# curtischong/arreau

Measured on AMD Instinct MI355X. Metric: denoising steps/sec (crystal-steps, whole node), higher is better.
Workload: dtype f32

## Files before the change

arreau_amd/_hip.py:

```python
import ctypes
import os
from ctypes import c_char_p, c_double, c_float, c_int32, c_int64, c_size_t, c_void_p, POINTER, Structure

import torch

_HERE = os.path.dirname(os.path.abspath(__file__))
LIB_PATH = os.environ.get("ARREAU_HIP_LIB") or os.path.join(_HERE, "csrc", "libarreau_hip.so")

EXPORTS = [
    "arreau_last_error", "arreau_version", "arreau_model_create", "arreau_model_destroy",
    "arreau_model_config", "arreau_workspace_bytes", "arreau_lattice_from_params", "arreau_frac_to_cart",
    "arreau_radius_graph_pbc", "arreau_compact_edges", "arreau_edges_to_slots", "arreau_predict_scores",
    "arreau_reverse_step", "arreau_profile_edge_kernel", "arreau_edge_kernel_time_ms", "arreau_conv_kernel_time_ms",
    "arreau_model_status", "arreau_model_set_variant", "arreau_ponita_forward",
    "arreau_diffusion_noise", "arreau_diffusion_losses", "arreau_sample_loop", "arreau_philox_fill",
    "arreau_train_forward", "arreau_train_backward", "arreau_train_conv_stats", "arreau_model_update_train_weights",
    "arreau_debug_sgemm", "arreau_optimizer_create", "arreau_optimizer_step", "arreau_optimizer_destroy",
    "arreau_model_train_weight_pointers", "arreau_model_refresh_derived_train_weights",
    "arreau_model_set_formats", "arreau_debug_set_pollution", "arreau_debug_leftover_fraction",
    "arreau_sample_loop_conditioned", "arreau_condition_initial_state",
    "arreau_sample_loop_scheduled", "arreau_reverse_step_to",
    "arreau_sample_loop_corrected", "arreau_corrector_step", "arreau_philox_fill_word",
    "arreau_sample_loop_resampled", "arreau_resample_jump", "arreau_optimizer_step_ema",
    "arreau_sample_loop_tied", "arreau_reverse_step_tied", "arreau_resample_jump_tied",
    "arreau_sample_loop_sym", "arreau_reverse_step_sym", "arreau_crystal_screen",
    "arreau_crystal_fingerprint", "arreau_fingerprint_match",
]

STATUS_NONFINITE, STATUS_BAD_TIMESTEP, STATUS_BAD_TYPE, STATUS_BAD_TIE, STATUS_BAD_SYMMETRY = 1, 2, 4, 8, 16
EDGE_KERNELS = {0: "fp32-mfma", 1: "fp32-mfma", 2: "fp32-mfma", 3: "bf16x6", 4: "fp16x3", 5: "general-fp32-gemm"}
MLP_KERNELS = {0: "fp32-mfma", 1: "bf16x6", 2: "fp16x3-32x32x16", 3: "fp16x3-16x16x32",
               5: "general-fp32-gemm"}
VARIANT_GENERAL = 5


class ArreauHipError(RuntimeError):
    pass


OPT_MAX_GROUPS = 4


class AdamArgs(Structure):
    _fields_ = [("step", c_int64), ("lr", c_double * OPT_MAX_GROUPS), ("weight_decay", c_double * OPT_MAX_GROUPS),
                ("beta1", c_double), ("beta2", c_double), ("eps", c_double), ("max_norm", c_double)]


class SampleConditionC(Structure):
    _fields_ = [("x0", c_void_p), ("pos_mask", c_void_p), ("a0", c_void_p), ("type_mask", c_void_p), ("l0", c_void_p),
                ("len_mask", c_void_p)]


class SampleScheduleC(Structure):
    _fields_ = [("d_next", c_void_p), ("lattice_clipmax", ctypes.c_float)]


class CorrectorC(Structure):
    _fields_ = [("steps", c_int32), ("snr", ctypes.c_float)]


class ResamplingC(Structure):
    _fields_ = [("passes", c_int32), ("jump_length", c_int32), ("timesteps", POINTER(c_int32)), ("n_timesteps", c_int32)]


class SymmetryC(Structure):
    _fields_ = [(name, c_void_p) for name in ("leader", "op", "orbit", "orbit_ptr", "orbit_atoms", "stab_ptr", "stab_ops", "rot",
                                                "rot_inv", "trans")] + [(name, c_int32) for name in ("n_orbits", "n_orbit_atoms",
                                                                                                     "n_stab_ops", "n_ops")]


class ScreenCriteriaC(Structure):
    _fields_ = [("min_distance", c_float), ("min_volume", c_float), ("search_radius", c_float), ("mask_type", c_int32),
                ("max_shells", c_int32)]


class ScreenResultC(Structure):
    _fields_ = [(name, c_void_p) for name in ("min_distance", "pair", "n_close", "volume", "number_density", "flags")]


class FingerprintParamsC(Structure):
    _fields_ = [("r_max", c_float), ("sigma", c_float), ("n_bins", c_int32), ("max_shells", c_int32)]


class FingerprintResultC(Structure):
    _fields_ = [(name, c_void_p) for name in ("fingerprint", "species", "counts", "flags")]


class MatchResultC(Structure):
    _fields_ = [(name, c_void_p) for name in ("duplicate_of", "distance", "nearest", "nearest_distance")]


class Config(Structure):
    _fields_ = [
        ("num_atomic_states", c_int32), ("hidden_dim", c_int32), ("basis_dim", c_int32),
        ("num_layers", c_int32), ("num_ori", c_int32), ("widening_factor", c_int32), ("degree", c_int32),
        ("max_neighbors", c_int32), ("num_timesteps", c_int32), ("radius", c_float),
        ("has_layer_scale", c_int32),
    ]


class Status(Structure):
    _fields_ = [("flags", c_int32), ("edge_kernel", c_int32), ("mlp_kernel", c_int32), ("conv_kernel", c_int32),
                ("basis_row_bytes", c_int32), ("conv_cross_fp8", c_int32), ("edge_activation_bound", c_float), ("node_activation_bound", c_float),
                ("basis_fp8_share", c_float), ("cross_fp8_share", c_float), ("readout_kernel", c_int32)]


_SD_FIELDS = [
    "basis_w1", "basis_b1", "basis_w2", "basis_b2", "fiber_w1", "fiber_b1", "fiber_w2", "fiber_b2",
    "x_embedder_w", "conv_kernel_w", "conv_fiber_w", "conv_bias", "norm_w", "norm_b", "linear1_w",
    "linear1_b", "linear2_w", "linear2_b", "layer_scale", "readout_w", "readout_b", "ori_grid", "t_emb_w",
    "ve_sigmas", "vp_alpha_bars", "vp_betas", "q_one_step_transposed", "q_mats",
]


class StateDict(Structure):
    _fields_ = [(name, c_void_p) for name in _SD_FIELDS]


def _prototypes():
    vp, i32, i64, u32, u64, f32, f64 = c_void_p, c_int32, c_int64, ctypes.c_uint32, ctypes.c_uint64, c_float, c_double
    cond, sched, corr, res, sym = (POINTER(t) for t in (SampleConditionC, SampleScheduleC, CorrectorC, ResamplingC, SymmetryC))
    loop = [vp] * 6 + [i32] * 4 + [u64] + [vp] * 4 + [c_size_t, i32]
    step_to = [vp] * 8 + [i32, i32] + [vp] * 7 + [f32]
    jump = [vp] * 8 + [i32, i32] + [vp] * 5 + [cond, vp]
    adam = [vp] * 4 + [POINTER(AdamArgs), vp]
    return {
        "arreau_last_error": [], "arreau_version": [],
        "arreau_model_create": [POINTER(Config), POINTER(StateDict), vp, POINTER(vp)],
        "arreau_model_destroy": [vp],
        "arreau_model_config": [vp, POINTER(Config)],
        "arreau_workspace_bytes": [POINTER(Config), i64, i64],
        "arreau_lattice_from_params": [vp, vp, i32, vp, vp],
        "arreau_frac_to_cart": [vp, vp, vp, i32, i32, vp, vp],
        "arreau_radius_graph_pbc": [vp, vp, vp, i32, i32, f32, i32] + [vp] * 6,
        "arreau_compact_edges": [vp] * 5 + [i32, i32] + [vp] * 6,
        "arreau_edges_to_slots": [vp, vp, vp, i64, i32, i32] + [vp] * 6,
        "arreau_predict_scores": [vp] * 7 + [i32, i32, i32] + [vp] * 7 + [vp, c_size_t, vp],
        "arreau_reverse_step": [vp] * 7 + [i32, i32] + [vp] * 8,
        "arreau_model_status": [vp, POINTER(Status), i32, vp],
        "arreau_model_set_variant": [vp, i32, i32],
        "arreau_model_set_formats": [vp, i32, i32],
        "arreau_ponita_forward": [vp] * 5 + [i32, i32] + [vp] * 7 + [vp, c_size_t, vp],
        "arreau_diffusion_noise": [vp] * 6 + [i32, i32] + [vp] * 11,
        "arreau_diffusion_losses": [vp] * 10 + [i32, i32] + [vp] * 6,
        "arreau_sample_loop": loop + [vp],
        "arreau_sample_loop_conditioned": loop + [cond, vp],
        "arreau_sample_loop_scheduled": loop + [cond, sched, vp],
        "arreau_sample_loop_corrected": loop + [cond, sched, corr, vp],
        "arreau_sample_loop_resampled": loop + [cond, sched, corr, res, vp],
        "arreau_sample_loop_tied": loop + [cond, sched, corr, res, vp, vp],
        "arreau_sample_loop_sym": loop + [cond, sched, corr, res, vp, sym, vp],
        "arreau_condition_initial_state": [vp] * 4 + [i32, i32, i32, u64, cond, vp],
        "arreau_reverse_step_to": step_to + [vp],
        "arreau_reverse_step_tied": step_to + [vp, vp],
        "arreau_reverse_step_sym": step_to + [vp, sym, vp],
        "arreau_corrector_step": [vp] * 4 + [i32, i32, vp, vp, f32, cond, vp],
        "arreau_resample_jump": jump + [vp],
        "arreau_resample_jump_tied": jump + [vp, vp],
        "arreau_philox_fill": [u64, i32, i32, i64, vp, vp, vp],
        "arreau_philox_fill_word": [u64, i32, i32, u32, i64, vp, vp, vp],
        "arreau_crystal_screen": [vp] * 4 + [i32, i32, POINTER(ScreenCriteriaC), POINTER(ScreenResultC), vp],
        "arreau_crystal_fingerprint": [vp] * 4 + [i32, i32, POINTER(FingerprintParamsC), POINTER(FingerprintResultC), vp],
        "arreau_fingerprint_match": [POINTER(FingerprintResultC), i32, POINTER(FingerprintResultC), i32, f32, POINTER(MatchResultC), vp],
        "arreau_train_forward": [vp] * 7 + [i32, i32] + [vp] * 4,
        "arreau_train_backward": [vp] * 4 + [POINTER(StateDict), vp],
        "arreau_train_conv_stats": [vp, vp, vp],
        "arreau_debug_sgemm": [i32, i32, i32, i32, vp, i64, i64, vp, i64, i64, vp, i32, f32, f32, vp],
        "arreau_model_update_train_weights": [vp, POINTER(StateDict), vp],
        "arreau_model_train_weight_pointers": [vp, POINTER(StateDict)],
        "arreau_model_refresh_derived_train_weights": [vp, vp, vp, vp],
        "arreau_optimizer_create": [i32, POINTER(vp), POINTER(vp), POINTER(i64), POINTER(i64), POINTER(i32), i32, i64, POINTER(vp)],
        "arreau_optimizer_step": adam + [vp],
        "arreau_optimizer_step_ema": adam + [f64, vp, vp],
        "arreau_optimizer_destroy": [vp],
        "arreau_debug_set_pollution": [u32],
        "arreau_debug_leftover_fraction": [u32, POINTER(f64), POINTER(f64), vp],
        "arreau_profile_edge_kernel": [i32],
        "arreau_edge_kernel_time_ms": [POINTER(f64), POINTER(i64)],
        "arreau_conv_kernel_time_ms": [POINTER(f64), POINTER(i64)],
    }


_RESTYPES = {"arreau_last_error": c_char_p, "arreau_version": c_char_p, "arreau_model_destroy": None,
             "arreau_workspace_bytes": c_size_t, "arreau_optimizer_destroy": None}

_lib = None


def lib():
    global _lib
    if _lib is not None:
        return _lib
    if not os.path.exists(LIB_PATH):
        raise ArreauHipError(
            f"{LIB_PATH} not found: build it with `python -m arreau_amd.build` (hipcc, gfx950). "
            "arreau_amd has no CPU fallback.")
    L = ctypes.CDLL(LIB_PATH)
    prototypes = _prototypes()
    for name in EXPORTS:
        if os.environ.get("ARREAU_HIP_LIB") and not hasattr(L, name):
            continue
        fn = getattr(L, name)
        fn.argtypes = prototypes[name]
        fn.restype = _RESTYPES.get(name, c_int32)
    _lib = L
    return L


def check(rc, what):
    if rc != 0:
        msg = lib().arreau_last_error().decode(errors="replace")
        raise ArreauHipError(f"{what} failed (code {rc}): {msg}")


def ptr(t):
    if t is None:
        return None
    assert t.is_contiguous(), "arreau_amd passes contiguous tensors only"
    return c_void_p(t.data_ptr())


def stream_ptr(device=None):
    return c_void_p(torch.cuda.current_stream(device).cuda_stream)


def require_gpu():
    if not torch.cuda.is_available():
        raise ArreauHipError("arreau_amd needs an AMD GPU (gfx950); there is no CPU fallback.")
```

arreau_amd/csrc/f16x3.h:

```cpp
#pragma once
#include <hip/hip_fp16.h>

#include "internal.h"

typedef _Float16 f16x8 __attribute__((ext_vector_type(8)));
typedef _Float16 f16x2 __attribute__((ext_vector_type(2)));
typedef unsigned int u32x4 __attribute__((ext_vector_type(4)));

#define F16X3_SCALE 2048.0f
#define F16X3_INV_SCALE (1.0f / 2048.0f)

#ifdef ARREAU_F32_PACKED
typedef float f32x2 __attribute__((ext_vector_type(2)));
__device__ __forceinline__ f32x2 fma2(f32x2 a, f32x2 b, f32x2 c) { return __builtin_elementwise_fma(a, b, c); }
__device__ __forceinline__ f16x2 cvt_f16x2(f32x2 v) { return __builtin_convertvector(v, f16x2); }
__device__ __forceinline__ f32x2 cvt_f32x2(f16x2 h) { return __builtin_convertvector(h, f32x2); }
#else
struct f32x2 { float x, y; };
__device__ __forceinline__ f32x2 operator*(f32x2 a, f32x2 b) { return f32x2{a.x * b.x, a.y * b.y}; }
__device__ __forceinline__ f32x2 operator-(f32x2 a, f32x2 b) { return f32x2{a.x - b.x, a.y - b.y}; }
__device__ __forceinline__ f32x2 operator+(f32x2 a, f32x2 b) { return f32x2{a.x + b.x, a.y + b.y}; }
__device__ __forceinline__ f32x2 fma2(f32x2 a, f32x2 b, f32x2 c) { return f32x2{fmaf(a.x, b.x, c.x), fmaf(a.y, b.y, c.y)}; }
__device__ __forceinline__ f16x2 cvt_f16x2(f32x2 v) {
    typedef float vf2 __attribute__((ext_vector_type(2)));
    return __builtin_convertvector(vf2{v.x, v.y}, f16x2);
}
__device__ __forceinline__ f32x2 cvt_f32x2(f16x2 h) { return f32x2{(float)h[0], (float)h[1]}; }
#endif
__device__ __forceinline__ f32x2 splat2(float v) { return f32x2{v, v}; }
#define F16X3_PAIR(v, i) (f32x2{(v)[2 * (i)], (v)[2 * (i) + 1]})

__device__ __forceinline__ f32x2 gelu_fast2(f32x2 x) {
    const float ax = fabsf(x.x), ay = fabsf(x.y);
    const f32x2 a = f32x2{__builtin_amdgcn_fmed3f(ax, -INFINITY, 12.0f), __builtin_amdgcn_fmed3f(ay, -INFINITY, 12.0f)};
    f32x2 q = fma2(splat2(3.3092788558903113e-05f), a, splat2(-7.6921945996487589e-04f));
    q = fma2(q, a, splat2(8.0807156986535972e-03f));
    q = fma2(q, a, splat2(-5.3412102790454205e-02f));
    q = fma2(q, a, splat2(-4.5877097453124149e-01f));
    q = fma2(q, a, splat2(-1.1512017015627947e+00f));
    q = fma2(q, a, splat2(-9.9999306107072172e-01f));
    f32x2 r;
    r.x = fmaf(-ax, __builtin_amdgcn_exp2f(q.x), __builtin_amdgcn_fmed3f(x.x, 0.0f, INFINITY));
    r.y = fmaf(-ay, __builtin_amdgcn_exp2f(q.y), __builtin_amdgcn_fmed3f(x.y, 0.0f, INFINITY));
    return r;
}
__device__ __forceinline__ float gelu_fast(float x) { return gelu_fast2(splat2(x)).x; }

struct Planes2 { u32x4 p[2][2]; };

template <bool CLAMP = true>
__device__ __forceinline__ void split_pair2(f32x2 v, unsigned& hi, unsigned& lo) {
    hi = __builtin_bit_cast(unsigned, cvt_f16x2(v));
    const f32x2 sc = v * splat2(F16X3_SCALE);
    const float neg_scale = -F16X3_SCALE;
    asm("v_fma_mixlo_f16 %0, %1, %2, %3 op_sel_hi:[1,0,0]" : "=v"(lo) : "v"(hi), "s"(neg_scale), "v"(sc.x));
    asm("v_fma_mixhi_f16 %0, %1, %2, %3 op_sel:[1,0,0] op_sel_hi:[1,0,0]" : "+v"(lo) : "v"(hi), "s"(neg_scale), "v"(sc.y));
}
template <bool OWNED = false>
__device__ __forceinline__ void split_pair_act(f32x2 v, unsigned& hi, unsigned& lo) {
    hi = __builtin_bit_cast(unsigned, cvt_f16x2(v));
    const float neg_one = -1.0f;
    if constexpr (OWNED) {
        lo = hi;
        asm("v_fma_mixlo_f16 %0, %1, %2, %3 op_sel_hi:[1,0,0]" : "+v"(lo) : "v"(hi), "s"(neg_one), "v"(v.x));
    } else
    asm("v_fma_mixlo_f16 %0, %1, %2, %3 op_sel_hi:[1,0,0]" : "=v"(lo) : "v"(hi), "s"(neg_one), "v"(v.x));
    asm("v_fma_mixhi_f16 %0, %1, %2, %3 op_sel:[1,0,0] op_sel_hi:[1,0,0]" : "+v"(lo) : "v"(hi), "s"(neg_one), "v"(v.y));
}
template <bool WORD>
__device__ __forceinline__ void split_pair_fp8(f32x2 v, unsigned& hi, unsigned& lo8) {
    typedef short s16x2 __attribute__((ext_vector_type(2)));
    hi = __builtin_bit_cast(unsigned, cvt_f16x2(v));
    float r0, r1;
    const float neg_one = -1.0f;
    asm("v_fma_mix_f32 %0, %1, %2, %3 op_sel_hi:[1,0,0]" : "=v"(r0) : "v"(hi), "s"(neg_one), "v"(v.x));
    asm("v_fma_mix_f32 %0, %1, %2, %3 op_sel:[1,0,0] op_sel_hi:[1,0,0]" : "=v"(r1) : "v"(hi), "s"(neg_one), "v"(v.y));
    lo8 = __builtin_bit_cast(unsigned, __builtin_amdgcn_cvt_scalef32_pk_fp8_f32(__builtin_bit_cast(s16x2, lo8), r0, r1, F16X3_INV_SCALE, WORD));
}
template <bool WORD>
__device__ __forceinline__ unsigned widen_lo8(unsigned lo8) {
    return __builtin_bit_cast(unsigned, __builtin_amdgcn_cvt_scalef32_pk_f16_fp8(lo8, 1.0f, WORD));
}

__device__ __forceinline__ Planes2 split_tile2(const f32x16& x) {
    Planes2 r;
#pragma unroll
    for (int s = 0; s < 2; ++s)
#pragma unroll
        for (int pp = 0; pp < 4; ++pp) {
            unsigned hi, lo;
            split_pair_act(F16X3_PAIR(x, 4 * s + pp), hi, lo);
            r.p[0][s][pp] = hi;
            r.p[1][s][pp] = lo;
        }
    return r;
}
__device__ __forceinline__ Planes2 gelu_split_folded2(const f32x16& v, float scale) {
    Planes2 r;
#pragma unroll
    for (int s = 0; s < 2; ++s)
#pragma unroll
        for (int pp = 0; pp < 4; ++pp) {
            unsigned hi, lo;
            split_pair_act(gelu_fast2(F16X3_PAIR(v, 4 * s + pp)) * splat2(scale), hi, lo);
            r.p[0][s][pp] = hi;
            r.p[1][s][pp] = lo;
        }
    return r;
}
__device__ __forceinline__ f32x16 fold_cross(const f32x16& mainacc, const f32x16& cross);
__device__ __forceinline__ Planes2 gelu_split_tile2(const f32x16& mainacc, const f32x16& cross, float scale) {
    return gelu_split_folded2(fold_cross(mainacc, cross), scale);
}

__device__ __forceinline__ f32x16 mfma_f16(const u32x4& a, const u32x4& b, const f32x16& c) {
    return __builtin_amdgcn_mfma_f32_32x32x16_f16(__builtin_bit_cast(f16x8, a), __builtin_bit_cast(f16x8, b), c, 0, 0, 0);
}

template <int NIN, int KS0, int KS1, int PF = 1>
__device__ __forceinline__ void mma_range2(f32x16& mainacc, f32x16& cross, const u32x4* __restrict__ buf,
                                           const Planes2 (&b)[NIN], int lane) {
    const u32x4* f = buf + lane;
    u32x4 c1[PF + 1], c2[PF + 1];
#pragma unroll
    for (int i = 0; i < PF; ++i)
        if (KS0 + i < KS1) {
            c1[i] = f[(size_t)(KS0 + i) * 128];
            c2[i] = f[(size_t)(KS0 + i) * 128 + 64];
        }
#pragma unroll
    for (int ks = KS0; ks < KS1; ++ks) {
        const int slot = (ks - KS0) % (PF + 1), nslot = (ks - KS0 + PF) % (PF + 1);
        if (ks + PF < KS1) {
            c1[nslot] = f[(size_t)(ks + PF) * 128];
            c2[nslot] = f[(size_t)(ks + PF) * 128 + 64];
        }
        const int t = ks >> 1, s = ks & 1;
        mainacc = mfma_f16(c1[slot], b[t].p[0][s], mainacc);
        cross = mfma_f16(c2[slot], b[t].p[0][s], cross);
        mainacc = mfma_f16(c1[slot], b[t].p[1][s], mainacc);
    }
    __builtin_amdgcn_sched_group_barrier(0x100, 2 * (PF < KS1 - KS0 ? PF : KS1 - KS0), 0);
#pragma unroll
    for (int ks = KS0; ks < KS1; ++ks) {
        if (ks + PF < KS1) __builtin_amdgcn_sched_group_barrier(0x100, 2, 0);
        __builtin_amdgcn_sched_group_barrier(0x008, 3, 0);
    }
}

template <int NIN, int NKS>
struct MmaStream2 {
    const u32x4* f;
    u32x4 c1[2], c2[2];
    __device__ __forceinline__ void start(const u32x4* __restrict__ buf, int lane) {
        f = buf + lane;
        c1[0] = f[0];
        c2[0] = f[64];
        __builtin_amdgcn_sched_group_barrier(0x100, 2, 0);
    }
    template <int KS0, int KS1>
    __device__ __forceinline__ void run(f32x16& mainacc, f32x16& cross, const Planes2 (&b)[NIN]) {
#pragma unroll
        for (int ks = KS0; ks < KS1; ++ks) {
            const int slot = ks & 1, nslot = slot ^ 1;
            if (ks + 1 < NKS) {
                c1[nslot] = f[(size_t)(ks + 1) * 128];
                c2[nslot] = f[(size_t)(ks + 1) * 128 + 64];
            }
            const int t = ks >> 1, s = ks & 1;
            mainacc = mfma_f16(c1[slot], b[t].p[0][s], mainacc);
            cross = mfma_f16(c2[slot], b[t].p[0][s], cross);
            mainacc = mfma_f16(c1[slot], b[t].p[1][s], mainacc);
        }
#pragma unroll
        for (int ks = KS0; ks < KS1; ++ks) {
            if (ks + 1 < NKS) __builtin_amdgcn_sched_group_barrier(0x100, 2, 0);
            __builtin_amdgcn_sched_group_barrier(0x008, 3, 0);
        }
    }
};

typedef float f32x4v __attribute__((ext_vector_type(4)));
__device__ __forceinline__ f32x4v mfma16_f16(const u32x4& a, const u32x4& b, const f32x4v& c) {
    return __builtin_amdgcn_mfma_f32_16x16x32_f16(__builtin_bit_cast(f16x8, a), __builtin_bit_cast(f16x8, b), c, 0, 0, 0);
}
struct Acc16 { f32x4v m[2][2], x[2][2]; };

template <int NKB, bool ACT = false >
struct MmaStream16 {
    const u32x4* f;
    u32x4 a1[2], a2[2];
    __device__ __forceinline__ void start(const u32x4* __restrict__ buf, int lane) {
        f = buf + lane;
        a1[0] = f[0];
        a2[0] = f[64];
        __builtin_amdgcn_sched_group_barrier(0x100, 2, 0);
    }
    template <int ST0, int ST1>
    __device__ __forceinline__ void run(Acc16& acc, const u32x4 (&b)[2][NKB][2]) {
        run<ST0, ST1>(acc.m, acc.x, b);
    }
    template <int ST0, int ST1>
    __device__ __forceinline__ void run(f32x4v (&am)[2][2], f32x4v (&ax)[2][2], const u32x4 (&b)[2][NKB][2]) {
#pragma unroll
        for (int st = ST0; st < ST1; ++st) {
            const int slot = st & 1, nslot = slot ^ 1;
            if (st + 1 < 2 * NKB) {
                a1[nslot] = f[(size_t)(st + 1) * 128];
                a2[nslot] = f[(size_t)(st + 1) * 128 + 64];
            }
            const int kb = st >> 1, mt = st & 1;
#pragma unroll
            for (int nb = 0; nb < 2; ++nb) {
                am[mt][nb] = mfma16_f16(a1[slot], b[nb][kb][0], am[mt][nb]);
                if constexpr (ACT) {
                    ax[mt][nb] = mfma16_f16(a2[slot], b[nb][kb][0], ax[mt][nb]);
                    am[mt][nb] = mfma16_f16(a1[slot], b[nb][kb][1], am[mt][nb]);
                } else {
                    ax[mt][nb] = mfma16_f16(a1[slot], b[nb][kb][1], ax[mt][nb]);
                    ax[mt][nb] = mfma16_f16(a2[slot], b[nb][kb][0], ax[mt][nb]);
                }
            }
        }
#pragma unroll
        for (int st = ST0; st < ST1; ++st) {
            if (st + 1 < 2 * NKB) __builtin_amdgcn_sched_group_barrier(0x100, 2, 0);
            __builtin_amdgcn_sched_group_barrier(0x008, 6, 0);
        }
    }
};

template <int NKB, int ST0, int ST1, int NB = 2>
__device__ __forceinline__ void mma16_range(f32x4v (&am)[2][NB], f32x4v (&ax)[2][NB], const u32x4* __restrict__ buf,
                                            const u32x4 (&b)[NB][NKB][2], int lane) {
    const u32x4* f = buf + lane;
    u32x4 a1[2], a2[2];
    auto frag = [&](u32x4& d, const u32x4& src) { d = src; };
    frag(a1[ST0 & 1], f[(size_t)ST0 * 128]);
    frag(a2[ST0 & 1], f[(size_t)ST0 * 128 + 64]);
#pragma unroll
    for (int st = ST0; st < ST1; ++st) {
        const int slot = st & 1, nslot = slot ^ 1;
        if (st + 1 < ST1) {
            frag(a1[nslot], f[(size_t)(st + 1) * 128]);
            frag(a2[nslot], f[(size_t)(st + 1) * 128 + 64]);
        }
        const int kb = st >> 1, mt = st & 1;
#pragma unroll
        for (int nb = 0; nb < NB; ++nb) {
            am[mt][nb] = mfma16_f16(a1[slot], b[nb][kb][0], am[mt][nb]);
            ax[mt][nb] = mfma16_f16(a2[slot], b[nb][kb][0], ax[mt][nb]);
            am[mt][nb] = mfma16_f16(a1[slot], b[nb][kb][1], am[mt][nb]);
        }
    }
    __builtin_amdgcn_sched_group_barrier(0x100, 2, 0);
#pragma unroll
    for (int st = ST0; st < ST1; ++st) {
        if (st + 1 < ST1) __builtin_amdgcn_sched_group_barrier(0x100, 2, 0);
        __builtin_amdgcn_sched_group_barrier(0x008, 3 * NB, 0);
    }
}

__device__ __forceinline__ f32x16 fold_cross(const f32x16& mainacc, const f32x16& cross) {
    f32x16 r;
#pragma unroll
    for (int i = 0; i < 8; ++i) {
        const f32x2 v = fma2(F16X3_PAIR(cross, i), splat2(F16X3_INV_SCALE), F16X3_PAIR(mainacc, i));
        r[2 * i] = v.x;
        r[2 * i + 1] = v.y;
    }
    return r;
}

__device__ __forceinline__ void glds16(const u32x4* gsrc, unsigned lds_dst) {
    unsigned keep;
    asm volatile("s_mov_b32 %0, m0\n\ts_mov_b32 m0, %2\n\ts_nop 0\n\tglobal_load_lds_dwordx4 %1, off\n\ts_mov_b32 m0, %0"
                 : "=&s"(keep) : "v"(gsrc), "s"(lds_dst) : "memory");
}
template <int NF, int NW>
__device__ __forceinline__ void dma_chunk(const u32x4* __restrict__ chunk, u32x4* slot, int wave, int lane) {
    constexpr int PER = (NF + NW - 1) / NW;
    const unsigned base = __builtin_amdgcn_readfirstlane((unsigned)(size_t)slot);
#pragma unroll
    for (int i = 0; i < PER; ++i) {
        int f = NW * i + wave;
        if (NF % NW != 0 && f >= NF) f -= NF % NW;
        glds16(chunk + (size_t)f * 64 + lane, base + (unsigned)f * 1024u);
    }
}
template <int NF, int NW>
__device__ __forceinline__ void dma_chunk_lean(const void* chunk_uniform, unsigned lane16, int wave,
                                               unsigned slot_plus_wave ) {
    static_assert(NF % NW == 0, "dma_chunk_lean: whole fragments per wave");
    const char* base = static_cast<const char*>(chunk_uniform) + 1024 * wave;
#pragma unroll
    for (int i = 0; i < NF / NW; ++i)
        asm volatile("s_add_u32 m0, %2, %3\n\ts_nop 0\n\tglobal_load_lds_dwordx4 %0, %1"
                     :
                     : "v"(lane16), "s"(base + 1024 * NW * i), "s"(slot_plus_wave), "n"(1024 * NW * i)
                     : "memory", "scc", "m0");
}
__device__ __forceinline__ void dma_wait() { asm volatile("s_waitcnt vmcnt(0)" ::: "memory"); }
template <int N>
__device__ __forceinline__ void dma_wait_but() {
#ifdef ARREAU_DEBUG_WAIT_ALL
    asm volatile("s_waitcnt vmcnt(0)" ::: "memory");
#else
    asm volatile("s_waitcnt vmcnt(%0)" ::"n"(N) : "memory");
#endif
}
```

arreau_amd/csrc/internal.h:

```cpp
#pragma once
#include <hip/hip_runtime.h>
#include <stdint.h>
#include <stdio.h>
#include <string>
#include <tuple>

#include "../../include/arreau_hip.h"

#define ARREAU_NUM_ATTR 6
#define ARREAU_NUM_MONO 83
#define ARREAU_MONO_PAD 96
#define ARREAU_POLY_COLS 258
#define ARREAU_ORI 16

struct arreau_train_ctx;
typedef float f32x16 __attribute__((ext_vector_type(16)));
typedef float f32x4 __attribute__((ext_vector_type(4)));

void arreau_set_error(const std::string& msg);

#define ARREAU_CHECK_HIP(expr)                                                              \
    do {                                                                                    \
        hipError_t _e = (expr);                                                             \
        if (_e != hipSuccess) {                                                             \
            arreau_set_error(std::string(#expr) + ": " + hipGetErrorString(_e));           \
            return ARREAU_EHIP;                                                             \
        }                                                                                   \
    } while (0)

#define ARREAU_REQUIRE(cond, msg)                                                           \
    do {                                                                                    \
        if (!(cond)) {                                                                      \
            arreau_set_error(std::string(msg));                                            \
            return ARREAU_EINVAL;                                                           \
        }                                                                                   \
    } while (0)

struct SampleConditionDev {
    const float* x0;
    const uint8_t* pos_mask;
    const int32_t* a0;
    const uint8_t* type_mask;
    const float* l0;
    const uint8_t* len_mask;
};

struct SampleState {
    float* frac;
    int32_t* types;
    float* lengths;
    const float* angles;
    const int32_t* offsets;
    int B, N;
    const int32_t* const_types;
    const float* fixed_lengths;
    float* lattice;
    bool operator==(const SampleState&) const = default;
};

inline bool operator==(const SampleConditionDev& a, const SampleConditionDev& b) {
    auto members = [](const SampleConditionDev& c) {
        const auto& [x0, pos_mask, a0, type_mask, l0, len_mask] = c;
        return std::tie(x0, pos_mask, a0, type_mask, l0, len_mask);
    };
    return members(a) == members(b);
}
inline bool operator==(const arreau_symmetry& a, const arreau_symmetry& b) {
    auto members = [](const arreau_symmetry& y) {
        const auto& [leader, op, orbit, orbit_ptr, orbit_atoms, stab_ptr, stab_ops, rot, rot_inv, trans, n_orbits, n_orbit_atoms,
                     n_stab_ops, n_ops] = y;
        return std::tie(leader, op, orbit, orbit_ptr, orbit_atoms, stab_ptr, stab_ops, rot, rot_inv, trans, n_orbits, n_orbit_atoms,
                        n_stab_ops, n_ops);
    };
    return members(a) == members(b);
}

struct SampleGraphKey {
    SampleState state;
    const void* workspace;
    uint64_t seed;
    SampleConditionDev cond;
    const int32_t* sched_next;
    const int32_t* length_tie;
    arreau_symmetry sym;
    int32_t edge_variant, mlp_variant, conv_variant, no_prep, basis_form, basis_fp8, cross_fp8, small_layer_fusion;
    int32_t scheduled;
    uint32_t clip_bits;
    int32_t corrector_steps;
    uint32_t snr_bits;
    int32_t resample_passes, resample_jump;
    bool operator==(const SampleGraphKey&) const = default;
};

struct arreau_model {
    arreau_config cfg;
    int S, C, D, L, O, W, H, k, T;
    float* blob;
    size_t blob_floats;
    const float* ori;
    const float* w1p;
    const float* b1;
    const float* w2p;
    const float* b2;
    const float* wkp;
    const float* edge_bf16;
    const float* edge_f16;
    int f16_ok;
    const float* conv_x8;
    int x8_ok;
    int x8_weights_ok;
    int fp8_ok;
    float calib_fp8, calib_x8;
    int train_full_range;
    int calibrating;
    float edge_act_bound, node_act_bound;
    int edge_variant, mlp_variant, conv_variant, readout_variant;
    mutable int ran_edge, ran_mlp, ran_conv, ran_x8, ran_readout;
    const float *t_w1f, *t_w2, *t_wk, *t_lin1, *t_lin2, *t_ro_w;
    struct arreau_train_ctx* train;
    int fused;
    int packed_stale;
    void* loop_stream;
    void* loop_event;
    SampleGraphKey graph_key;
    void* retired_graph;
    void* retired_stream;
    int32_t* status;
    float* fk;
    const float* conv_bias;
    const float* ln_w;
    const float* ln_b;
    const float* mlp;
    const float* mlp_bf16;
    const float* mlp_f16;
    const float* mlp_f16m;
    const float* mb1;
    const float* mb2;
    const float* ls;
    const float* embT;
    const float* ro_wT;
    const float* ro_b;
    const float* ro_pack;
    const float* ro_wv;
    float ro_bv_host[16];
    const float* t_emb_w;
    const float* ve_sigmas;
    const float* vp_alpha_bars;
    const float* vp_betas;
    const float* q1t;
    const float* qmats;
    int qmats_absorbing;
    const float* fiber_w1;
    const float* fiber_b1;
    const float* fiber_w2;
    const float* fiber_b2;
    const float* fiber_wk;
};

#define ARREAU_PACK_TILE_FLOATS 1024

__device__ __forceinline__ f32x16 arreau_mfma(float a, float b, f32x16 c) {
    return __builtin_amdgcn_mfma_f32_32x32x2f32(a, b, c, 0, 0, 0);
}

#define ARREAU_PF 8

template <int G, int NIN, int NCB>
__device__ __forceinline__ void arreau_stream_tile(f32x16 (&acc)[NCB], f32x4 (&ring)[ARREAU_PF],
                                                   const float* __restrict__ region, const int f0,
                                                   const f32x16 (&b)[NIN][NCB]) {
#pragma unroll
    for (int g = 0; g < G; ++g) {
        const int f = f0 + g;
        const f32x4 a = ring[f % ARREAU_PF];
        ring[f % ARREAU_PF] = *reinterpret_cast<const f32x4*>(region + (size_t)(f + ARREAU_PF) * 256);
#pragma unroll
        for (int m = 0; m < 4; ++m) {
#pragma unroll
            for (int cb = 0; cb < NCB; ++cb) acc[cb] = arreau_mfma(a[m], b[g >> 2][cb][4 * (g & 3) + m], acc[cb]);
        }
    }
#pragma unroll
    for (int g = 0; g < G; ++g) {
        __builtin_amdgcn_sched_group_barrier(0x020, 1, 0);
        __builtin_amdgcn_sched_group_barrier(0x008, 4 * NCB, 0);
    }
}

__device__ __forceinline__ f32x16 arreau_bias_tile(const float* __restrict__ bias, int u, int h) {
    f32x16 r;
#pragma unroll
    for (int q = 0; q < 4; ++q) {
        const f32x4 v = *reinterpret_cast<const f32x4*>(bias + 32 * u + 8 * q + 4 * h);
        r[4 * q] = v[0]; r[4 * q + 1] = v[1]; r[4 * q + 2] = v[2]; r[4 * q + 3] = v[3];
    }
    return r;
}

__device__ __forceinline__ float arreau_erf(float a) {
    const float t = fabsf(a);
    const float s = a * a;
    float r = fmaf(-1.72853470e-5f, t, 3.83197126e-4f);
    const float u = fmaf(-3.88396438e-3f, t, 2.42546219e-2f);
    r = fmaf(r, s, u);
    r = fmaf(r, t, -1.06777877e-1f);
    r = fmaf(r, t, -6.34846687e-1f);
    r = fmaf(r, t, -1.28717512e-1f);
    r = fmaf(r, t, -t);
    r = 1.0f - __builtin_amdgcn_exp2f(r * 1.44269504088896341f);
    r = copysignf(r, a);
    float p = -5.96761703e-4f;
    p = fmaf(p, s, 4.99119423e-3f);
    p = fmaf(p, s, -2.67681349e-2f);
    p = fmaf(p, s, 1.12819925e-1f);
    p = fmaf(p, s, -3.76125336e-1f);
    p = fmaf(p, s, 1.28379166e-1f);
    p = fmaf(p, a, a);
    return t > 0.927734375f ? r : p;
}

__device__ __forceinline__ float arreau_gelu(float x) {
    return 0.5f * x * (1.0f + arreau_erf(x * 0.70710678118654752440f));
}

struct StepNoiseSrc {
    const float* z_lattice;
    const float* z_frac;
    const float* u_types;
    uint64_t seed;
};

inline bool arreau_condition_empty(const SampleConditionDev* c) {
    return !c || !((c->x0 && c->pos_mask) || (c->a0 && c->type_mask) || (c->l0 && c->len_mask));
}
int arreau_condition_to_dev(const arreau_sample_condition* c, SampleConditionDev* out);
int arreau_symmetry_check(const arreau_symmetry* y, const char* who);

struct StepScheduleDev {
    const int32_t* next;
    const int32_t* s_of;
    float clipmax;
};

int arreau_corrector_check(int32_t steps, float snr, const char* who);
struct CorrectorDev {
    int steps;
    float snr;
};

struct StepOptions {
    const SampleConditionDev* cond = nullptr;
    const StepScheduleDev* sched = nullptr;
    CorrectorDev corr{};
    const int32_t* pass = nullptr;
    const int32_t* length_tie = nullptr;
    const arreau_symmetry* sym = nullptr;
};

int arreau_launch_corrector(const arreau_model* m, const SampleState& st, const int32_t* d_t, const float* d_eps, const float* d_z_frac,
                            uint64_t seed, uint32_t iter, const StepOptions& opt, hipStream_t s);

int arreau_resampling_check(int32_t passes, int32_t jump_length, const char* who);
struct JumpLoopDev {
    float* lattice_ws;
    float* cvec;
    int32_t* t_next;
    int32_t* t_cur;
    int32_t* pass;
};
int arreau_launch_resample_jump(const arreau_model* m, const SampleState& st, const int32_t* d_s, const int32_t* d_t, int s, int t,
                                const int32_t* d_batch, const StepNoiseSrc& noise , uint32_t pass,
                                const SampleConditionDev* cond, const JumpLoopDev* loop,
                                const int32_t* d_length_tie ,
                                hipStream_t stream);

void arreau_train_ctx_destroy(struct arreau_train_ctx* t);
#define ARREAU_VARIANT_GENERAL 5
inline bool arreau_general_path(const arreau_model* m) { return !m->fused || m->edge_variant == ARREAU_VARIANT_GENERAL; }
struct arreau_graph_view {
    const int32_t *batch, *deg, *src;
    const float *lattice, *dir, *dist;
};
int arreau_general_network(arreau_model* m, const arreau_graph_view& g, const int32_t* d_off, int B, int N, float* d_eps,
                           float* d_logits, float* d_len0, hipStream_t s);
float* arreau_general_x0(arreau_model* m, int N, int B, hipStream_t s);
void arreau_model_retire_graph(arreau_model* m, void* exec, void* stream);

inline int arreau_cu_count() {
    static const int n_cu = [] {
        int dev = 0;
        hipDeviceProp_t prop;
        if (hipGetDevice(&dev) == hipSuccess && hipGetDeviceProperties(&prop, dev) == hipSuccess && prop.multiProcessorCount > 0)
            return (int)prop.multiProcessorCount;
        return 256;
    }();
    return n_cu;
}

extern unsigned arreau_debug_pollution;
int arreau_debug_pollute(hipStream_t s);
#define ARREAU_LAUNCH(kernel, grid, block, smem, stream, ...)                      \
    do {                                                                           \
        if (arreau_debug_pollution) (void)arreau_debug_pollute(stream);            \
        hipLaunchKernelGGL(kernel, grid, block, smem, stream, __VA_ARGS__);        \
    } while (0)

int arreau_launch_fiber_precompute(arreau_model* m, hipStream_t s);
int arreau_launch_neighbor(const float* cart, const float* lattice, const int32_t* offsets, const int32_t* batch, int B, int N,
                           float radius, int k, int32_t* deg, int32_t* src, int32_t* cell, float* dir, float* dist,
                           hipStream_t s);
int arreau_launch_neighbor_embed(const arreau_model* m, const float* cart, const float* lattice, const int32_t* offsets,
                                 const int32_t* batch, int B, int N, int32_t* deg, int32_t* src, int32_t* cell, float* dir,
                                 float* dist, const float* frac, const int32_t* types, const float* cvec, float* x0, hipStream_t s,
                                 int32_t* tick = nullptr ,
                                 const int32_t* next_t = nullptr ,
                                 bool advance = true );
int arreau_launch_prep(const arreau_model* m, const float* frac, const float* lengths, const float* angles,
                       const int32_t* t, const int32_t* offsets, int B, int N, float* lattice, float* cart,
                       int32_t* batch, float* cvec, hipStream_t s, int32_t* t_next = nullptr, int32_t* t_cur = nullptr,
                       int t_offset = 0, const int32_t* next_t = nullptr );
struct ReverseInputs {
    const int32_t* t;
    const float *eps, *logits, *len0;
    StepNoiseSrc noise;
    const float* gs_atoms = nullptr;
    const int32_t* batch = nullptr;
    float* lattice_ws = nullptr;
    float* cvec_next = nullptr;
};
int arreau_launch_reverse(const arreau_model* m, const SampleState& st, const ReverseInputs& in, const StepOptions& opt, hipStream_t s);
int arreau_launch_edge(const arreau_model* m, const float* dir, const float* dist, const int32_t* deg,
                       const int32_t* batch, const float* lattice, int N, float* kbuf, hipStream_t s);
int arreau_launch_edge_bf16x6(const arreau_model* m, const float* dir, const float* dist, const int32_t* deg,
                              const int32_t* batch, const float* lattice, int N, float* kbuf, hipStream_t s);
int arreau_launch_edge_f16x3(const arreau_model* m, const float* dir, const float* dist, const int32_t* deg,
                             const int32_t* batch, const float* lattice, int N, float* kbuf, hipStream_t s);
int arreau_launch_embed(const arreau_model* m, const float* frac, const int32_t* types, const float* lattice,
                        const int32_t* batch, const float* cvec, int N, float* x0, hipStream_t s);
int arreau_launch_embed_general(const arreau_model* m, const float* x, const float* vec, int N, float* x0, hipStream_t s);
int arreau_launch_batch_index(const int32_t* offsets, int B, int N, int32_t* batch, hipStream_t s);
int arreau_launch_node_layer(const arreau_model* m, int layer, const float* kbuf, const int32_t* deg,
                             const int32_t* src, const float* x_in, float* x_conv, float* x_out, float* xbar,
                             float* vsum, int N, hipStream_t s);
typedef unsigned int u32x3_k __attribute__((ext_vector_type(3)));
__device__ __forceinline__ u32x3_k arreau_pack_k3(float v0, float v1, float v2, float v3) {
    const unsigned r0 = __float_as_uint(v0) + 0x80u, r1 = __float_as_uint(v1) + 0x80u;
    const unsigned r2 = __float_as_uint(v2) + 0x80u, r3 = __float_as_uint(v3) + 0x80u;
    u32x3_k d;
    d[0] = __builtin_amdgcn_perm(r1, r0, 0x05030201u);
    d[1] = __builtin_amdgcn_perm(r2, r1, 0x06050302u);
    d[2] = __builtin_amdgcn_perm(r3, r2, 0x07060503u);
    return d;
}
__device__ __forceinline__ void arreau_unpack_k3(unsigned d0, unsigned d1, unsigned d2, float (&v)[4]) {
    v[0] = __uint_as_float(d0 << 8);
    v[1] = __uint_as_float(__builtin_amdgcn_perm(d1, d0, 0x0504030cu));
    v[2] = __uint_as_float(__builtin_amdgcn_perm(d2, d1, 0x0403020cu));
    v[3] = __uint_as_float(d2 & 0xffffff00u);
}
bool arreau_k3(const arreau_model* m);
bool arreau_basis_form(const arreau_model* m, int receivers);
bool arreau_basis_fp8(const arreau_model* m);
bool arreau_cross_fp8(const arreau_model* m);
void arreau_prof_conv(int end, hipStream_t s);
int arreau_launch_conv_proj(const arreau_model* m, int layer, const float* basis, const int32_t* deg, const int32_t* src,
                            const float* x_in, float* x_conv, int N, hipStream_t s);

int arreau_launch_mlp_bf16x6(const arreau_model* m, int layer, const float* x_conv, const float* x_in, float* x_out,
                             float* xbar, float* vsum, int N, hipStream_t s);
bool arreau_mlp_train_forward_available(const arreau_model* m);
int arreau_launch_mlp_train_forward(const arreau_model* m, int layer, const float* x_conv, const float* x_in, float* x_out, float* xhat,
                                    float* rstd, float* xn, float* hpre, float* h, float* out, int N, hipStream_t s,
                                    const float* kl = nullptr, int kl_pitch = 0, const int32_t* deg = nullptr, const int32_t* src = nullptr,
                                    const float* fk = nullptr, float* x1 = nullptr);
int arreau_repack_mlp_f16x3_m16(arreau_model* m, hipStream_t s);
int arreau_launch_mlp_f16x3_m16(const arreau_model* m, int layer, const float* x_conv, const float* x_in, float* x_out,
                                float* xbar, float* vsum, int N, hipStream_t s);
bool arreau_small_layer_fusable(const arreau_model* m, int N);
int arreau_launch_small_layer(const arreau_model* m, int layer, const float* kbuf, const int32_t* deg, const int32_t* src,
                              const float* x_in, float* x_out, float* xbar, float* vsum, int Ntot, hipStream_t s);
int arreau_launch_mlp_f16x3_m16_split(const arreau_model* m, int layer, const float* x_conv, const float* x_in, float* x_out,
                                      float* xbar, float* vsum, int N, hipStream_t s);
int arreau_launch_readout(const arreau_model* m, const float* xbar, const float* vsum, const int32_t* offsets,
                          int B, int N, float* gs, float* eps, float* logits, float* len0, hipStream_t s);
```

arreau_amd/csrc/model.hip:

```cpp
#include <math.h>
#include <stdlib.h>
#include <string.h>

#include <algorithm>
#include <vector>

#include "internal.h"

static thread_local std::string g_last_error;
void arreau_set_error(const std::string& msg) { g_last_error = msg; }
extern "C" const char* arreau_last_error(void) { return g_last_error.c_str(); }
extern "C" const char* arreau_version(void) { return "arreau_hip 0.1 (gfx950)"; }

static void pack_linear(const float* W, int out_dim, int in_dim, int in_stride, int out_pad, int in_pad,
                        float* P) {
    const int U = out_pad / 32, Tn = in_pad / 32;
    for (int u = 0; u < U; ++u)
        for (int t = 0; t < Tn; ++t)
            for (int q = 0; q < 4; ++q)
                for (int lane = 0; lane < 64; ++lane)
                    for (int m = 0; m < 4; ++m) {
                        int out = 32 * u + (lane & 31);
                        int in = 32 * t + 8 * q + 4 * (lane >> 5) + m;
                        float v = (out < out_dim && in < in_dim) ? W[(size_t)out * in_stride + in] : 0.0f;
                        P[((((size_t)u * Tn + t) * 4 + q) * 64 + lane) * 4 + m] = v;
                    }
}

static inline uint16_t bf16_trunc_bits(float x) {
    uint32_t u;
    memcpy(&u, &x, 4);
    return (uint16_t)(u >> 16);
}
static inline float bf16_bits_to_float(uint16_t b) {
    uint32_t u = (uint32_t)b << 16;
    float x;
    memcpy(&x, &u, 4);
    return x;
}

static void pack_linear_bf16x3(const float* W, int out_dim, int in_dim, int in_stride, int out_pad, int in_pad,
                               uint16_t* Q) {
    const int U = out_pad / 32, Tn = in_pad / 32;
    for (int u = 0; u < U; ++u)
        for (int t = 0; t < Tn; ++t)
            for (int s = 0; s < 2; ++s)
                for (int lane = 0; lane < 64; ++lane)
                    for (int jj = 0; jj < 8; ++jj) {
                        const int out = 32 * u + (lane & 31);
                        const int in = 32 * t + 16 * s + 8 * (jj >> 2) + 4 * (lane >> 5) + (jj & 3);
                        const float w = (out < out_dim && in < in_dim) ? W[(size_t)out * in_stride + in] : 0.0f;
                        const uint16_t b1 = bf16_trunc_bits(w);
                        const float r1 = w - bf16_bits_to_float(b1);
                        const uint16_t b2 = bf16_trunc_bits(r1);
                        const float r2 = r1 - bf16_bits_to_float(b2);
                        const uint16_t b3 = bf16_trunc_bits(r2);
                        const uint16_t pl[3] = {b1, b2, b3};
                        for (int p = 0; p < 3; ++p)
                            Q[((((((size_t)u * Tn + t) * 2 + s) * 3 + p) * 64) + lane) * 8 + jj] = pl[p];
                    }
}

static inline uint16_t f32_to_f16_rne(float x) {
    uint32_t u;
    memcpy(&u, &x, 4);
    const uint32_t sign = (u >> 16) & 0x8000u;
    const int32_t exp = (int32_t)((u >> 23) & 0xff) - 127 + 15;
    uint32_t man = u & 0x7fffffu;
    if (((u >> 23) & 0xff) == 0xff) return (uint16_t)(sign | 0x7c00u | (man ? 0x200u : 0));
    if (exp >= 31) return (uint16_t)(sign | 0x7c00u);
    if (exp <= 0) {
        if (exp < -10) return (uint16_t)sign;
        man |= 0x800000u;
        const int shift = 14 - exp;
        uint32_t half = man >> shift;
        const uint32_t rem = man & ((1u << shift) - 1), mid = 1u << (shift - 1);
        if (rem > mid || (rem == mid && (half & 1))) ++half;
        return (uint16_t)(sign | half);
    }
    uint32_t half = ((uint32_t)exp << 10) | (man >> 13);
    const uint32_t rem = man & 0x1fffu;
    if (rem > 0x1000u || (rem == 0x1000u && (half & 1))) ++half;
    return (uint16_t)(sign | half);
}
static inline float f16_to_f32(uint16_t hbits) {
    const uint32_t sign = (uint32_t)(hbits & 0x8000u) << 16;
    const uint32_t exp = (hbits >> 10) & 0x1f, man = hbits & 0x3ffu;
    uint32_t u;
    if (exp == 0) {
        if (man == 0) u = sign;
        else {
            int e = -1;
            uint32_t m = man;
            do { ++e; m <<= 1; } while (!(m & 0x400u));
            u = sign | ((uint32_t)(127 - 15 - e) << 23) | ((m & 0x3ffu) << 13);
        }
    } else if (exp == 31) u = sign | 0x7f800000u | (man << 13);
    else u = sign | ((exp - 15 + 127) << 23) | (man << 13);
    float x;
    memcpy(&x, &u, 4);
    return x;
}

static float pack_linear_f16x3(const float* W, int out_dim, int in_dim, int in_stride, int out_pad, int in_pad,
                               uint16_t* Q) {
    const int U = out_pad / 32, Tn = in_pad / 32;
    float wmax = 0.f;
    for (int u = 0; u < U; ++u)
        for (int t = 0; t < Tn; ++t)
            for (int s = 0; s < 2; ++s)
                for (int lane = 0; lane < 64; ++lane)
                    for (int jj = 0; jj < 8; ++jj) {
                        const int out = 32 * u + (lane & 31);
                        const int in = 32 * t + 16 * s + 8 * (jj >> 2) + 4 * (lane >> 5) + (jj & 3);
                        const float w = (out < out_dim && in < in_dim) ? W[(size_t)out * in_stride + in] : 0.0f;
                        wmax = fabsf(w) > wmax ? fabsf(w) : wmax;
                        const uint16_t h1 = f32_to_f16_rne(w);
                        const uint16_t h2 = f32_to_f16_rne((w - f16_to_f32(h1)) * 2048.0f);
                        const size_t base = ((((size_t)u * Tn + t) * 2 + s) * 2) * 512 + (size_t)lane * 8 + jj;
                        Q[base] = h1;
                        Q[base + 512] = h2;
                    }
    return wmax;
}

static float pack_linear_f16x3_m16(const float* W, int out_dim, int in_dim, int in_stride, uint16_t* Q, bool native = false) {
    const int U = out_dim / 32, KB = in_dim / 32;
    float wmax = 0.f;
    for (int u = 0; u < U; ++u)
        for (int kb = 0; kb < KB; ++kb)
            for (int mt = 0; mt < 2; ++mt)
                for (int lane = 0; lane < 64; ++lane)
                    for (int e = 0; e < 8; ++e) {
                        const int g = lane >> 4;
                        const int out = 32 * u + 16 * mt + (lane & 15);
                        const int in = native ? 32 * kb + 16 * (e >> 2) + 4 * g + (e & 3)
                                              : 32 * kb + 16 * (g & 1) + 8 * (e >> 2) + 4 * (g >> 1) + (e & 3);
                        const float w = W[(size_t)out * in_stride + in];
                        wmax = fabsf(w) > wmax ? fabsf(w) : wmax;
                        const uint16_t h1 = f32_to_f16_rne(w);
                        const uint16_t h2 = f32_to_f16_rne((w - f16_to_f32(h1)) * 2048.0f);
                        const size_t base = (((size_t)u * KB + kb) * 2 + mt) * 2 * 512 + (size_t)lane * 8 + e;
                        Q[base] = h1;
                        Q[base + 512] = h2;
                    }
    return wmax;
}

static inline uint8_t f32_to_e4m3_rne_sat(float x) {
    const uint8_t sign = signbit(x) ? 0x80 : 0;
    const float a = fabsf(x);
    if (!(a == a)) return 0x7f;
    if (a >= 448.0f) return sign | 0x7e;
    int e;
    const float f = frexpf(a, &e);
    const int E = e - 1;
    if (a == 0.0f) return sign;
    if (E < -6) return sign | (uint8_t)nearbyintf(ldexpf(a, 9));
    int mant = (int)nearbyintf((2.0f * f - 1.0f) * 8.0f), ex = E + 7;
    if (mant == 8) { mant = 0; ++ex; }
    const int code = (ex << 3) | mant;
    return sign | (uint8_t)(code > 0x7e ? 0x7e : code);
}

static float pack_conv_cross_fp8(const float* W , int C, int D, uint8_t* Q) {
    float amax = 0.f;
    for (int T = 0; T < C / 16; ++T)
        for (int kp = 0; kp < D / 64; ++kp)
            for (int h = 0; h < 2; ++h)
                for (int lane = 0; lane < 64; ++lane)
                    for (int e = 0; e < 8; ++e) {
                        const int g = lane >> 4, kb = 2 * kp + h;
                        const int out = 16 * T + (lane & 15);
                        const int in = 32 * kb + 16 * (e >> 2) + 4 * g + (e & 3);
                        const float w = W[(size_t)out * D + in];
                        const float a1 = f16_to_f32(f32_to_f16_rne(w));
                        const float a2 = f16_to_f32(f32_to_f16_rne((w - a1) * 2048.0f));
                        amax = fmaxf(amax, fabsf(64.0f * a1));
                        const size_t plane0 = ((((size_t)T * (D / 64) + kp) * 2 + 0) * 64 + lane) * 16, plane1 = plane0 + 64 * 16;
                        Q[plane0 + 8 * h + e] = f32_to_e4m3_rne_sat(64.0f * a1);
                        Q[plane1 + 8 * h + e] = f32_to_e4m3_rne_sat(64.0f * a2);
                    }
    return amax;
}

struct Mono { int n; int idx[3]; };
static std::vector<Mono> monomials() {
    std::vector<Mono> v;
    for (int i = 0; i < 6; ++i) v.push_back({1, {i, 0, 0}});
    for (int i = 0; i < 6; ++i)
        for (int j = i; j < 6; ++j) v.push_back({2, {i, j, 0}});
    for (int i = 0; i < 6; ++i)
        for (int j = i; j < 6; ++j)
            for (int k = j; k < 6; ++k) v.push_back({3, {i, j, k}});
    return v;
}

static void fold_poly_weight(const float* W, int C, std::vector<float>& Wf ) {
    auto mons = monomials();
    Wf.assign((size_t)C * ARREAU_MONO_PAD, 0.0f);
    for (int c = 0; c < C; ++c) {
        const float* row = W + (size_t)c * ARREAU_POLY_COLS;
        for (size_t mi = 0; mi < mons.size(); ++mi) {
            const Mono& mo = mons[mi];
            double acc = 0.0;
            if (mo.n == 1) {
                acc = row[mo.idx[0]];
            } else if (mo.n == 2) {
                int i = mo.idx[0], j = mo.idx[1];
                acc = row[6 + 6 * i + j];
                if (i != j) acc += row[6 + 6 * j + i];
            } else {
                int a[3] = {mo.idx[0], mo.idx[1], mo.idx[2]};
                int perms[6][3] = {{0, 1, 2}, {0, 2, 1}, {1, 0, 2}, {1, 2, 0}, {2, 0, 1}, {2, 1, 0}};
                int seen[6][3];
                int ns = 0;
                for (auto& p : perms) {
                    int t3[3] = {a[p[0]], a[p[1]], a[p[2]]};
                    bool dup = false;
                    for (int s = 0; s < ns; ++s)
                        if (seen[s][0] == t3[0] && seen[s][1] == t3[1] && seen[s][2] == t3[2]) dup = true;
                    if (dup) continue;
                    seen[ns][0] = t3[0]; seen[ns][1] = t3[1]; seen[ns][2] = t3[2];
                    ++ns;
                    acc += row[42 + 36 * t3[0] + 6 * t3[1] + t3[2]];
                }
            }
            Wf[(size_t)c * ARREAU_MONO_PAD + mi] = (float)acc;
        }
    }
}

struct BlobBuilder {
    std::vector<float> data;
    size_t reserve(size_t n) {
        size_t off = (data.size() + 63) / 64 * 64;
        data.resize(off + n, 0.0f);
        return off;
    }
    size_t put(const float* src, size_t n) {
        size_t off = reserve(n);
        memcpy(data.data() + off, src, n * sizeof(float));
        return off;
    }
};

#define ARREAU_CALIB_SHARE 0.1f
static int calibrate_message_formats(arreau_model* m, hipStream_t s) {
    const char* off = getenv("ARREAU_CALIBRATE");
    if ((off && atoi(off) == 0) || !m->fused || !m->f16_ok || m->edge_variant != 4 || m->conv_variant != 2 || m->k != 8 || m->L < 2 ||
        (m->mlp_variant != 3 && m->mlp_variant != 4))
        return ARREAU_OK;
    const int B = 16, n = 20, N = B * n, S = m->S;
    uint64_t rng = 0x9e3779b97f4a7c15ull;
    auto uni = [&]() {
        rng ^= rng >> 12; rng ^= rng << 25; rng ^= rng >> 27;
        return (float)((double)((rng * 0x2545f4914f6cdd1dull) >> 11) / 9007199254740992.0);
    };
    std::vector<float> frac((size_t)N * 3), lengths((size_t)B * 3), angles((size_t)B * 3);
    std::vector<int32_t> types(N), tt(B, m->T / 2), offs(B + 1);
    for (auto& v : frac) v = uni();
    for (auto& v : lengths) v = 4.0f + 4.0f * uni();
    for (auto& v : angles) v = (70.0f + 40.0f * uni()) * 0.017453292519943295f;
    for (int i = 0; i < N; ++i) types[i] = i % 3 == 0 ? S - 1 : (int)(uni() * (float)S) % S;
    for (int b = 0; b <= B; ++b) offs[b] = b * n;
    const size_t ws_bytes = arreau_workspace_bytes(&m->cfg, N, B);
    const size_t f_in = (size_t)N * 3 + 6 * (size_t)B, out1 = (size_t)N * 3 + (size_t)N * S + 3 * (size_t)B;
    const size_t i_in = (size_t)N + 2 * (size_t)B + 1;
    char* dev = nullptr;
    const size_t bytes = ws_bytes + (f_in + 3 * out1 + i_in) * 4 + 4096;
    if (hipMalloc((void**)&dev, bytes) != hipSuccess) { (void)hipGetLastError(); return ARREAU_OK; }
    float* d_frac = (float*)dev; float* d_len = d_frac + (size_t)N * 3; float* d_ang = d_len + 3 * B;
    float* d_out = d_ang + 3 * B;
    int32_t* d_types = (int32_t*)(d_out + 3 * out1); int32_t* d_t = d_types + N; int32_t* d_off = d_t + B;
    char* d_ws = (char*)(((uintptr_t)(d_off + B + 1) + 255) & ~(uintptr_t)255);
    hipError_t e = hipMemcpyAsync(d_frac, frac.data(), frac.size() * 4, hipMemcpyHostToDevice, s);
    if (e == hipSuccess) e = hipMemcpyAsync(d_len, lengths.data(), lengths.size() * 4, hipMemcpyHostToDevice, s);
    if (e == hipSuccess) e = hipMemcpyAsync(d_ang, angles.data(), angles.size() * 4, hipMemcpyHostToDevice, s);
    if (e == hipSuccess) e = hipMemcpyAsync(d_types, types.data(), types.size() * 4, hipMemcpyHostToDevice, s);
    if (e == hipSuccess) e = hipMemcpyAsync(d_t, tt.data(), tt.size() * 4, hipMemcpyHostToDevice, s);
    if (e == hipSuccess) e = hipMemcpyAsync(d_off, offs.data(), offs.size() * 4, hipMemcpyHostToDevice, s);
    int rc = e == hipSuccess ? ARREAU_OK : ARREAU_EHIP;
    const int x8_weights = m->x8_ok;
    m->calibrating = 1;
    const int modes[3][2] = {{0, 0}, {1, 0}, {1, 1}};
    for (int v = 0; v < 3 && rc == ARREAU_OK; ++v) {
        if (modes[v][1] && !x8_weights) break;
        m->fp8_ok = modes[v][0]; m->x8_ok = modes[v][1];
        float* o = d_out + (size_t)v * out1;
        rc = arreau_predict_scores(m, d_frac, d_types, d_len, d_ang, d_t, d_off, B, N, 0, nullptr, nullptr, nullptr, nullptr, o,
                                   o + (size_t)N * 3, o + (size_t)N * 3 + (size_t)N * S, d_ws, ws_bytes, (void*)s);
    }
    m->calibrating = 0;
    m->fp8_ok = 1; m->x8_ok = x8_weights;
    std::vector<float> h(3 * out1);
    int32_t flags = 0;
    if (rc == ARREAU_OK) {
        e = hipMemcpyAsync(h.data(), d_out, h.size() * 4, hipMemcpyDeviceToHost, s);
        if (e == hipSuccess) e = hipMemcpyAsync(&flags, m->status, 4, hipMemcpyDeviceToHost, s);
        if (e == hipSuccess) e = hipMemsetAsync(m->status, 0, 4, s);
        if (e == hipSuccess) e = hipStreamSynchronize(s);
        if (e != hipSuccess) rc = ARREAU_EHIP;
    }
    (void)hipStreamSynchronize(s);
    (void)hipFree(dev);
    m->ran_edge = m->ran_mlp = m->ran_conv = m->ran_readout = -1;
    m->ran_x8 = 0;
    if (rc != ARREAU_OK) { arreau_set_error(std::string("format calibration: ") + arreau_last_error()); return rc; }
    (void)flags;
    auto finite = [&](int v) {
        const float* q = h.data() + (size_t)v * out1;
        for (size_t i = 0; i < (size_t)N * 3 + (size_t)N * S; ++i)
            if (!(fabsf(q[i]) < INFINITY)) return false;
        return true;
    };
    if (!finite(0)) return ARREAU_OK;
    auto share = [&](int v) {
        if (!finite(v)) return 1e9;
        const float* r = h.data();
        const float* q = h.data() + (size_t)v * out1;
        double me = 0.0, ml = 0.0, de = 0.0, dl = 0.0;
        for (size_t i = 0; i < (size_t)N * 3; ++i) { me = fmax(me, fabs((double)r[i])); de = fmax(de, fabs((double)q[i] - r[i])); }
        for (size_t i = (size_t)N * 3; i < (size_t)N * 3 + (size_t)N * S; ++i) { ml = fmax(ml, fabs((double)r[i])); dl = fmax(dl, fabs((double)q[i] - r[i])); }
        return fmax(de / (1e-5 * fmax(1.0, me)), dl / (1e-5 * fmax(1.0, ml / 8.0)));
    };
    m->calib_fp8 = (float)fmin(share(1), 1e9);
    m->fp8_ok = m->calib_fp8 <= ARREAU_CALIB_SHARE ? 1 : 0;
    if (x8_weights) {
        m->calib_x8 = (float)fmin(share(2), 1e9);
        m->x8_ok = m->fp8_ok && m->calib_x8 <= ARREAU_CALIB_SHARE ? 1 : 0;
    }
    if (getenv("ARREAU_VERBOSE_CALIBRATION"))
        fprintf(stderr, "[arreau_hip] message-path formats: share of the parity bounds used up on the calibration batch -- fp8 residual plane %.3f, "
                "+ fp8 cross products %.3f (limit %.2f): basis fp8 %d, fp8 cross %d\n", m->calib_fp8, m->calib_x8, ARREAU_CALIB_SHARE, m->fp8_ok, m->x8_ok);
    return ARREAU_OK;
}

extern "C" int arreau_model_create(const arreau_config* cfg, const arreau_state_dict* sd, void* stream,
                                   arreau_model** out_model) {
    ARREAU_REQUIRE(cfg && sd && out_model, "arreau_model_create: null argument");
    const int S = cfg->num_atomic_states, C = cfg->hidden_dim, D = cfg->basis_dim, L = cfg->num_layers;
    const int O = cfg->num_ori, W = cfg->widening_factor, T = cfg->num_timesteps, k = cfg->max_neighbors;
    const int H = W * C;
    ARREAU_REQUIRE(O == ARREAU_ORI, "unsupported num_ori (this build handles num_ori = 16)");
    ARREAU_REQUIRE(cfg->degree == 3, "unsupported polynomial degree (this build handles degree = 3)");
    ARREAU_REQUIRE(C >= 4 && C % 4 == 0 && C <= 1024, "hidden_dim must be a multiple of 4 in 4..1024");
    ARREAU_REQUIRE(D >= 4 && D % 4 == 0 && D <= 1024, "basis_dim must be a multiple of 4 in 4..1024");
    ARREAU_REQUIRE(W >= 1 && H <= 1024, "widening_factor * hidden_dim must be at most 1024");
    const bool fused = C == 128 && D == 256 && W == 4;
    ARREAU_REQUIRE(k >= 1 && k <= ARREAU_MAX_K, "max_neighbors must be in 1..8");
    ARREAU_REQUIRE(S >= 2 && S <= 124, "num_atomic_states must be in 2..124");
    ARREAU_REQUIRE(L >= 1 && L <= 8 && T >= 2, "bad num_layers (1..8) / num_timesteps");
    const float* need[] = {sd->basis_w1, sd->basis_b1, sd->basis_w2, sd->basis_b2, sd->fiber_w1, sd->fiber_b1,
                           sd->fiber_w2, sd->fiber_b2, sd->x_embedder_w, sd->conv_kernel_w, sd->conv_fiber_w,
                           sd->conv_bias, sd->norm_w, sd->norm_b, sd->linear1_w, sd->linear1_b, sd->linear2_w,
                           sd->linear2_b, sd->readout_w, sd->readout_b, sd->ori_grid, sd->t_emb_w, sd->ve_sigmas,
                           sd->vp_alpha_bars, sd->vp_betas, sd->q_one_step_transposed, sd->q_mats};
    for (const float* p : need) ARREAU_REQUIRE(p != nullptr, "arreau_model_create: missing state_dict entry");

    float edge_bound = 0.f, node_bound = 0.f;
    {
        std::vector<float> w1f_b;
        fold_poly_weight(sd->basis_w1, C, w1f_b);
        auto mons = monomials();
        const double R = cfg->radius > 1.0f ? cfg->radius : 1.0f;
        double mono_max = 0.0, h1_max = 0.0, basis_max = 0.0;
        std::vector<double> mb(mons.size());
        for (size_t mi = 0; mi < mons.size(); ++mi) {
            double b = 1.0;
            for (int q = 0; q < mons[mi].n; ++q) b *= mons[mi].idx[q] == 2 ? R : 1.0;
            mb[mi] = b;
            mono_max = std::max(mono_max, b);
        }
        for (int j = 0; j < C; ++j) {
            double a = fabs((double)sd->basis_b1[j]);
            for (size_t mi = 0; mi < mons.size(); ++mi) a += fabs((double)w1f_b[(size_t)j * ARREAU_MONO_PAD + mi]) * mb[mi];
            h1_max = std::max(h1_max, a);
        }
        for (int j = 0; j < D; ++j) {
            double a = fabs((double)sd->basis_b2[j]);
            for (int i = 0; i < C; ++i) a += fabs((double)sd->basis_w2[(size_t)j * C + i]) * h1_max;
            basis_max = std::max(basis_max, a);
        }
        edge_bound = (float)std::max(mono_max, std::max(h1_max, basis_max));
        double nb = 0.0;
        for (int l = 0; l < L; ++l) {
            const float* g = sd->norm_w + (size_t)l * C;
            const float* be = sd->norm_b + (size_t)l * C;
            for (int i = 0; i < C; ++i) nb = std::max(nb, sqrt((double)C - 1.0) * fabs((double)g[i]) + fabs((double)be[i]));
            for (int j = 0; j < H; ++j) {
                const float* w = sd->linear1_w + ((size_t)l * H + j) * C;
                double n2 = 0.0, dot = 0.0;
                for (int i = 0; i < C; ++i) { n2 += (double)w[i] * g[i] * (double)w[i] * g[i]; dot += (double)w[i] * be[i]; }
                nb = std::max(nb, sqrt((double)C) * sqrt(n2) + fabs(dot) + fabs((double)sd->linear1_b[(size_t)l * H + j]));
            }
        }
        node_bound = (float)nb;
    }

    BlobBuilder bb;
    std::vector<float> tmp;
    const size_t off_ori = bb.put(sd->ori_grid, (size_t)O * 3);

    std::vector<float> w1f;
    fold_poly_weight(sd->basis_w1, C, w1f);
    const size_t n_w1 = (size_t)(C / 32) * (ARREAU_MONO_PAD / 32) * ARREAU_PACK_TILE_FLOATS;
    const size_t n_w2 = (size_t)(D / 32) * (C / 32) * ARREAU_PACK_TILE_FLOATS;
    const size_t wk_tile = (size_t)(C / 32) * (D / 32) * ARREAU_PACK_TILE_FLOATS;
    const size_t stream_pad = 16 * 256;
    const size_t off_w1p = bb.reserve(fused ? n_w1 + n_w2 + wk_tile * L + stream_pad : 0);
    const size_t off_w2p = off_w1p + n_w1;
    const size_t off_wkp = off_w2p + n_w2;
    if (fused) {
        pack_linear(w1f.data(), C, ARREAU_MONO_PAD, ARREAU_MONO_PAD, C, ARREAU_MONO_PAD, bb.data.data() + off_w1p);
        pack_linear(sd->basis_w2, D, C, C, D, C, bb.data.data() + off_w2p);
        for (int l = 0; l < L; ++l)
            pack_linear(sd->conv_kernel_w + (size_t)l * C * D, C, D, D, C, D, bb.data.data() + off_wkp + l * wk_tile);
    }
    const size_t off_b1 = bb.put(sd->basis_b1, C);
    const size_t off_b2 = bb.put(sd->basis_b2, D);
    const size_t h_w1 = (size_t)(C / 32) * (ARREAU_MONO_PAD / 32) * 6 * 512;
    const size_t h_w2 = (size_t)(D / 32) * (C / 32) * 6 * 512;
    const size_t h_wk = (size_t)(C / 32) * (D / 32) * 6 * 512;
    const size_t off_es16 = bb.reserve(fused ? (h_w1 + h_w2 + h_wk * L) / 2 + 64 : 0);
    if (fused) {
        uint16_t* q = reinterpret_cast<uint16_t*>(bb.data.data() + off_es16);
        pack_linear_bf16x3(w1f.data(), C, ARREAU_MONO_PAD, ARREAU_MONO_PAD, C, ARREAU_MONO_PAD, q);
        pack_linear_bf16x3(sd->basis_w2, D, C, C, D, C, q + h_w1);
        for (int l = 0; l < L; ++l)
            pack_linear_bf16x3(sd->conv_kernel_w + (size_t)l * C * D, C, D, D, C, D, q + h_w1 + h_w2 + l * h_wk);
    }

    const size_t f_w1 = (size_t)(C / 32) * (ARREAU_MONO_PAD / 32) * 4 * 512;
    const size_t f_w2 = (size_t)(D / 32) * (C / 32) * 4 * 512;
    const size_t f_wk = (size_t)(C / 32) * (D / 32) * 4 * 512;
    const size_t off_ef16 = bb.reserve(fused ? (f_w1 + f_w2 + f_wk * L) / 2 + 64 : 0);
    float wmax16 = 0.f;
    if (fused) {
        uint16_t* q = reinterpret_cast<uint16_t*>(bb.data.data() + off_ef16);
        wmax16 = fmaxf(wmax16, pack_linear_f16x3(w1f.data(), C, ARREAU_MONO_PAD, ARREAU_MONO_PAD, C, ARREAU_MONO_PAD, q));
        wmax16 = fmaxf(wmax16, pack_linear_f16x3_m16(sd->basis_w2, D, C, C, q + f_w1));
        for (int l = 0; l < L; ++l)
            wmax16 = fmaxf(wmax16, pack_linear_f16x3_m16(sd->conv_kernel_w + (size_t)l * C * D, C, D, D,
                                                         q + f_w1 + f_w2 + l * f_wk, true));
    }
    const size_t x8_layer_floats = (size_t)(C / 16) * (D / 64) * 2 * 64 * 16 / 4;
    const size_t off_x8 = bb.reserve(fused ? x8_layer_floats * L : 0);
    float x8_amax = 0.f;
    if (fused)
        for (int l = 0; l < L; ++l)
            x8_amax = fmaxf(x8_amax, pack_conv_cross_fp8(sd->conv_kernel_w + (size_t)l * C * D, C, D,
                                                         reinterpret_cast<uint8_t*>(bb.data.data() + off_x8 + l * x8_layer_floats)));
    const size_t off_fk = bb.reserve((size_t)L * O * O * C);
    const size_t off_conv_bias = bb.put(sd->conv_bias, (size_t)L * C);
    const size_t off_ln_w = bb.put(sd->norm_w, (size_t)L * C);
    const size_t off_ln_b = bb.put(sd->norm_b, (size_t)L * C);

    const int HQ = H / 4;
    const size_t q1 = (size_t)(HQ / 32) * (C / 32) * ARREAU_PACK_TILE_FLOATS;
    const size_t q2 = (size_t)(C / 32) * (HQ / 32) * ARREAU_PACK_TILE_FLOATS;
    const size_t off_mlp = bb.reserve(fused ? (q1 + q2) * 4 * L + stream_pad : 0);
    for (int l = 0; l < L && fused; ++l)
        for (int w = 0; w < 4; ++w) {
            float* dst = bb.data.data() + off_mlp + ((size_t)l * 4 + w) * (q1 + q2);
            pack_linear(sd->linear1_w + ((size_t)l * H + (size_t)w * HQ) * C, HQ, C, C, HQ, C, dst);
            pack_linear(sd->linear2_w + (size_t)l * C * H + (size_t)w * HQ, C, HQ, H, C, HQ, dst + q1);
        }
    const size_t hq1 = (size_t)(HQ / 32) * (C / 32) * 6 * 512;
    const size_t hq2 = (size_t)(C / 32) * (HQ / 32) * 6 * 512;
    const size_t off_mlp16 = bb.reserve(fused ? (hq1 + hq2) * 4 * L / 2 + 64 : 0);
    for (int l = 0; l < L && fused; ++l)
        for (int w = 0; w < 4; ++w) {
            uint16_t* dst = reinterpret_cast<uint16_t*>(bb.data.data() + off_mlp16) + ((size_t)l * 4 + w) * (hq1 + hq2);
            pack_linear_bf16x3(sd->linear1_w + ((size_t)l * H + (size_t)w * HQ) * C, HQ, C, C, HQ, C, dst);
            pack_linear_bf16x3(sd->linear2_w + (size_t)l * C * H + (size_t)w * HQ, C, HQ, H, C, HQ, dst + hq1);
        }
    const size_t fq1 = (size_t)(HQ / 32) * (C / 32) * 4 * 512;
    const size_t fq2 = (size_t)(C / 32) * (HQ / 32) * 4 * 512;
    const size_t off_mlpf16 = bb.reserve(fused ? (fq1 + fq2) * 4 * L / 2 + 64 : 0);
    for (int l = 0; l < L && fused; ++l)
        for (int w = 0; w < 4; ++w) {
            uint16_t* dst = reinterpret_cast<uint16_t*>(bb.data.data() + off_mlpf16) + ((size_t)l * 4 + w) * (fq1 + fq2);
            wmax16 = fmaxf(wmax16, pack_linear_f16x3(sd->linear1_w + ((size_t)l * H + (size_t)w * HQ) * C, HQ, C, C, HQ, C, dst));
            wmax16 = fmaxf(wmax16, pack_linear_f16x3(sd->linear2_w + (size_t)l * C * H + (size_t)w * HQ, C, HQ, H, C, HQ, dst + fq1));
        }
    const size_t off_mlpf16m = bb.reserve(fused ? (fq1 + fq2) * 4 * L / 2 + 64 : 0);
    for (int l = 0; l < L && fused; ++l)
        for (int w = 0; w < 4; ++w) {
            uint16_t* dst = reinterpret_cast<uint16_t*>(bb.data.data() + off_mlpf16m) + ((size_t)l * 4 + w) * (fq1 + fq2);
            pack_linear_f16x3_m16(sd->linear1_w + ((size_t)l * H + (size_t)w * HQ) * C, HQ, C, C, dst, true);
            pack_linear_f16x3_m16(sd->linear2_w + (size_t)l * C * H + (size_t)w * HQ, C, HQ, H, dst + fq1, true);
        }
    const size_t off_mb1 = bb.put(sd->linear1_b, (size_t)L * H);
    const size_t off_mb2 = bb.put(sd->linear2_b, (size_t)L * C);

    tmp.assign((size_t)L * C, 1.0f);
    if (cfg->has_layer_scale && sd->layer_scale) memcpy(tmp.data(), sd->layer_scale, tmp.size() * sizeof(float));
    const size_t off_ls = bb.put(tmp.data(), tmp.size());

    const int IN = S + 78;
    tmp.assign((size_t)IN * C, 0.f);
    for (int c = 0; c < C; ++c)
        for (int i = 0; i < IN; ++i) tmp[(size_t)i * C + c] = sd->x_embedder_w[(size_t)c * IN + i];
    const size_t off_embT = bb.put(tmp.data(), tmp.size());

    const int RO = S + 4;
    tmp.assign((size_t)L * C * RO, 0.f);
    for (int l = 0; l < L; ++l)
        for (int s = 0; s < RO; ++s)
            for (int c = 0; c < C; ++c)
                tmp[((size_t)l * C + c) * RO + s] = sd->readout_w[((size_t)l * RO + s) * C + c];
    const size_t off_ro_wT = bb.put(tmp.data(), tmp.size());
    const size_t off_ro_b = bb.put(sd->readout_b, (size_t)L * RO);
    const int RO_PAD = RO <= 96 ? 96 : ((RO + 31) / 32) * 32;
    const size_t ro_layer = (size_t)(RO_PAD / 32) * (C / 32) * ARREAU_PACK_TILE_FLOATS;
    tmp.assign(fused ? (size_t)L * ro_layer + (size_t)ARREAU_PF * 256 : 0, 0.f);
    for (int l = 0; l < L && fused; ++l) pack_linear(sd->readout_w + (size_t)l * RO * C, RO, C, C, RO_PAD, C, tmp.data() + (size_t)l * ro_layer);
    const size_t off_ro_pack = bb.put(tmp.data(), tmp.size());
    tmp.assign((size_t)L * C, 0.f);
    for (int l = 0; l < L; ++l)
        for (int c = 0; c < C; ++c) tmp[(size_t)l * C + c] = sd->readout_w[((size_t)l * RO + S) * C + c];
    const size_t off_ro_wv = bb.put(tmp.data(), tmp.size());

    const size_t off_temb = bb.put(sd->t_emb_w, ARREAU_T_EMB_DIM / 2);
    const size_t off_ve = bb.put(sd->ve_sigmas, (size_t)T + 1);
    const size_t off_ab = bb.put(sd->vp_alpha_bars, (size_t)T + 1);
    const size_t off_be = bb.put(sd->vp_betas, (size_t)T + 1);
    const size_t off_q1t = bb.put(sd->q_one_step_transposed, (size_t)T * S * S);
    const size_t off_qm = bb.put(sd->q_mats, (size_t)T * S * S);

    const size_t off_fw1 = bb.put(sd->fiber_w1, (size_t)C * 3);
    const size_t off_fb1 = bb.put(sd->fiber_b1, C);
    const size_t off_fw2 = bb.put(sd->fiber_w2, (size_t)D * C);
    const size_t off_fb2 = bb.put(sd->fiber_b2, D);
    const size_t off_fwk = bb.put(sd->conv_fiber_w, (size_t)L * C * D);
    const size_t off_t_w1f = bb.put(w1f.data(), (size_t)C * ARREAU_MONO_PAD);
    const size_t off_t_w2 = bb.put(sd->basis_w2, (size_t)D * C);
    const size_t off_t_wk = bb.put(sd->conv_kernel_w, (size_t)L * C * D);
    const size_t off_t_lin1 = bb.put(sd->linear1_w, (size_t)L * H * C);
    const size_t off_t_lin2 = bb.put(sd->linear2_w, (size_t)L * C * H);
    const size_t off_t_ro_w = bb.reserve((size_t)L * RO * C + (size_t)4 * C);
    memcpy(bb.data.data() + off_t_ro_w, sd->readout_w, (size_t)L * RO * C * sizeof(float));
    const size_t off_status = bb.reserve(64);

    arreau_model* m = new arreau_model();
    memset(m, 0, sizeof(*m));
    m->cfg = *cfg;
    m->S = S; m->C = C; m->D = D; m->L = L; m->O = O; m->W = W; m->H = H; m->k = k; m->T = T;
    m->blob_floats = bb.data.size();
    hipError_t e = hipMalloc((void**)&m->blob, m->blob_floats * sizeof(float));
    if (e != hipSuccess) {
        delete m;
        arreau_set_error(std::string("hipMalloc(model blob): ") + hipGetErrorString(e));
        return ARREAU_EHIP;
    }
    hipStream_t s = (hipStream_t)stream;
    e = hipMemcpyAsync(m->blob, bb.data.data(), m->blob_floats * sizeof(float), hipMemcpyHostToDevice, s);
    if (e == hipSuccess) e = hipStreamSynchronize(s);
    if (e != hipSuccess) {
        (void)hipFree(m->blob);
        delete m;
        arreau_set_error(std::string("model upload: ") + hipGetErrorString(e));
        return ARREAU_EHIP;
    }
    float* b = m->blob;
    m->ori = b + off_ori; m->w1p = b + off_w1p; m->b1 = b + off_b1; m->w2p = b + off_w2p; m->b2 = b + off_b2;
    m->wkp = b + off_wkp; m->edge_bf16 = b + off_es16; m->edge_f16 = b + off_ef16; m->f16_ok = fused && wmax16 < 60000.0f ? 1 : 0; m->conv_x8 = b + off_x8; m->x8_ok = m->x8_weights_ok = fused && x8_amax <= 448.0f ? 1 : 0; m->fp8_ok = fused ? 1 : 0; m->calib_fp8 = m->calib_x8 = -1.0f; m->fk = b + off_fk; m->conv_bias = b + off_conv_bias; m->ln_w = b + off_ln_w;
    m->ln_b = b + off_ln_b; m->mlp = b + off_mlp; m->mlp_bf16 = b + off_mlp16; m->mlp_f16 = b + off_mlpf16; m->mlp_f16m = b + off_mlpf16m; m->mb1 = b + off_mb1; m->mb2 = b + off_mb2;
    m->ls = b + off_ls; m->embT = b + off_embT; m->ro_wT = b + off_ro_wT; m->ro_b = b + off_ro_b; m->ro_pack = b + off_ro_pack; m->ro_wv = b + off_ro_wv;
    for (int l = 0; l < L; ++l) m->ro_bv_host[l] = sd->readout_b[(size_t)l * RO + S];
    m->t_emb_w = b + off_temb; m->ve_sigmas = b + off_ve; m->vp_alpha_bars = b + off_ab; m->vp_betas = b + off_be;
    m->q1t = b + off_q1t; m->qmats = b + off_qm;
    {
        int absorbing = 1;
        const float* q = sd->q_mats;
        for (size_t t = 0; t < (size_t)T && absorbing; ++t)
            for (int c = 0; c < S && absorbing; ++c)
                for (int s2 = 0; s2 < S - 1; ++s2)
                    if (s2 != c && q[(t * S + c) * S + s2] != 0.0f) { absorbing = 0; break; }
        if (getenv("ARREAU_D3PM_DENSE")) absorbing = 0;
        m->qmats_absorbing = absorbing;
    }
    m->fiber_w1 = b + off_fw1; m->fiber_b1 = b + off_fb1; m->fiber_w2 = b + off_fw2; m->fiber_b2 = b + off_fb2;
    m->fiber_wk = b + off_fwk;
    m->status = reinterpret_cast<int32_t*>(b + off_status);
    m->t_w1f = b + off_t_w1f; m->t_w2 = b + off_t_w2; m->t_wk = b + off_t_wk; m->t_lin1 = b + off_t_lin1;
    m->t_lin2 = b + off_t_lin2; m->t_ro_w = b + off_t_ro_w;
    auto env_int = [](const char* name, int dflt) { const char* e = getenv(name); return e ? atoi(e) : dflt; };
    m->edge_act_bound = edge_bound;
    m->node_act_bound = node_bound;
    const float f16_slack = 64.0f * 65504.0f;
    m->edge_variant = env_int("ARREAU_EDGE_VARIANT", edge_bound <= f16_slack ? 4 : 3);
    m->mlp_variant = env_int("ARREAU_MLP_VARIANT", node_bound <= f16_slack ? 3 : 1);
    m->train_full_range = edge_bound > f16_slack || node_bound > f16_slack ? 1 : 0;
    m->conv_variant = env_int("ARREAU_CONV_VARIANT", 2);
    m->readout_variant = env_int("ARREAU_READOUT_VARIANT", 1);
    m->ran_edge = m->ran_mlp = m->ran_conv = m->ran_readout = -1;
    m->ran_x8 = 0;
    m->fused = fused ? 1 : 0;
    if (!fused || getenv("ARREAU_GENERAL_PATH")) m->edge_variant = ARREAU_VARIANT_GENERAL;

    int rc = arreau_launch_fiber_precompute(m, s);
    if (rc == ARREAU_OK) {
        e = hipStreamSynchronize(s);
        if (e != hipSuccess) {
            arreau_set_error(std::string("fiber precompute: ") + hipGetErrorString(e));
            rc = ARREAU_EHIP;
        }
    }
    if (rc == ARREAU_OK) rc = calibrate_message_formats(m, s);
    if (rc != ARREAU_OK) {
        if (m->train) arreau_train_ctx_destroy(m->train);
        (void)hipFree(m->blob);
        delete m;
        return rc;
    }
    *out_model = m;
    return ARREAU_OK;
}

void arreau_model_retire_graph(arreau_model* m, void* exec, void* stream) {
    if (m->retired_graph) {
        (void)hipStreamSynchronize((hipStream_t)m->retired_stream);
        (void)hipGraphExecDestroy((hipGraphExec_t)m->retired_graph);
    }
    m->retired_graph = exec;
    m->retired_stream = stream;
}

extern "C" void arreau_model_destroy(arreau_model* model) {
    if (!model) return;
    arreau_model_retire_graph(model, nullptr, nullptr);
    if (model->train) {
        (void)hipDeviceSynchronize();
        arreau_train_ctx_destroy(model->train);
    }
    if (model->loop_stream) {
        (void)hipStreamSynchronize((hipStream_t)model->loop_stream);
        (void)hipStreamDestroy((hipStream_t)model->loop_stream);
        (void)hipEventDestroy((hipEvent_t)model->loop_event);
    }
    if (model->blob) (void)hipFree(model->blob);
    delete model;
}

extern "C" int arreau_model_config(const arreau_model* model, arreau_config* out_cfg) {
    ARREAU_REQUIRE(model && out_cfg, "arreau_model_config: null argument");
    *out_cfg = model->cfg;
    return ARREAU_OK;
}

extern "C" int arreau_model_set_variant(arreau_model* model, int32_t edge_variant, int32_t mlp_variant) {
    ARREAU_REQUIRE(model, "arreau_model_set_variant: null model");
    ARREAU_REQUIRE(edge_variant >= -1 && edge_variant <= ARREAU_VARIANT_GENERAL && mlp_variant >= -1 && mlp_variant <= 4,
                   "arreau_model_set_variant: edge variant must be in 0..5, mlp variant in 0..4 (-1 keeps)");
    ARREAU_REQUIRE(model->fused || edge_variant < 0 || edge_variant == ARREAU_VARIANT_GENERAL,
                   "arreau_model_set_variant: this model's shape (hidden_dim, basis_dim, widening_factor) has no fused kernels; "
                   "only the general path (edge variant 5) is available");
    if (edge_variant >= 0) model->edge_variant = edge_variant;
    if (mlp_variant == 1) model->train_full_range = 1;
    else if (mlp_variant == 3) model->train_full_range = 0;
    if (mlp_variant >= 0) model->mlp_variant = mlp_variant;
    return ARREAU_OK;
}

extern "C" int arreau_model_set_formats(arreau_model* model, int32_t basis_fp8, int32_t cross_fp8) {
    ARREAU_REQUIRE(model, "arreau_model_set_formats: null model");
    if (basis_fp8 >= 0) model->fp8_ok = basis_fp8 != 0 && model->fused ? 1 : 0;
    if (cross_fp8 >= 0) model->x8_ok = cross_fp8 != 0 && model->x8_weights_ok ? 1 : 0;
    if (!model->fp8_ok) model->x8_ok = 0;
    return ARREAU_OK;
}

extern "C" int arreau_model_status(const arreau_model* model, arreau_status* out, int32_t reset, void* stream) {
    ARREAU_REQUIRE(model && out, "arreau_model_status: null argument");
    hipStream_t s = (hipStream_t)stream;
    int32_t flags = 0;
    ARREAU_CHECK_HIP(hipMemcpyAsync(&flags, model->status, sizeof(flags), hipMemcpyDeviceToHost, s));
    if (reset) ARREAU_CHECK_HIP(hipMemsetAsync(model->status, 0, sizeof(int32_t), s));
    ARREAU_CHECK_HIP(hipStreamSynchronize(s));
    out->flags = flags;
    out->edge_kernel = model->ran_edge;
    out->mlp_kernel = model->ran_mlp;
    out->conv_kernel = model->ran_conv;
    out->readout_kernel = model->ran_readout;
    out->basis_row_bytes = model->ran_conv == 2 ? (arreau_basis_fp8(model) ? 768 : 1024) : 0;
    out->conv_cross_fp8 = model->ran_conv == 2 ? model->ran_x8 : 0;
    out->edge_activation_bound = model->edge_act_bound;
    out->node_activation_bound = model->node_act_bound;
    out->basis_fp8_share = model->calib_fp8;
    out->cross_fp8_share = model->calib_x8;
    return ARREAU_OK;
}

__global__ void fiber_precompute_kernel(const float* __restrict__ ori, const float* __restrict__ w1,
                                        const float* __restrict__ b1, const float* __restrict__ w2,
                                        const float* __restrict__ b2, const float* __restrict__ wk,
                                        float* __restrict__ fk, int C, int D, int L, int O) {
    extern __shared__ float sm[];
    float* h1 = sm;
    float* basis = sm + C;
    const int o = blockIdx.x / O, p = blockIdx.x % O;
    const float a = ori[o * 3 + 0] * ori[p * 3 + 0] + ori[o * 3 + 1] * ori[p * 3 + 1] + ori[o * 3 + 2] * ori[p * 3 + 2];
    const float poly[3] = {a, a * a, (a * a) * a};
    for (int c = threadIdx.x; c < C; c += blockDim.x) {
        float v = b1[c];
        for (int i = 0; i < 3; ++i) v += w1[c * 3 + i] * poly[i];
        h1[c] = arreau_gelu(v);
    }
    __syncthreads();
    for (int d = threadIdx.x; d < D; d += blockDim.x) {
        float v = b2[d];
        for (int c = 0; c < C; ++c) v += w2[(size_t)d * C + c] * h1[c];
        basis[d] = arreau_gelu(v);
    }
    __syncthreads();
    for (int idx = threadIdx.x; idx < L * C; idx += blockDim.x) {
        const int l = idx / C, c = idx % C;
        const float* wrow = wk + ((size_t)l * C + c) * D;
        float v = 0.f;
        for (int d = 0; d < D; ++d) v += wrow[d] * basis[d];
        fk[(((size_t)l * O + o) * O + p) * C + c] = v / (float)O;
    }
}

int arreau_launch_fiber_precompute(arreau_model* m, hipStream_t s) {
    const size_t smem = (size_t)(m->C + m->D) * sizeof(float);
    hipLaunchKernelGGL(fiber_precompute_kernel, dim3(m->O * m->O), dim3(256), smem, s, m->ori, m->fiber_w1,
                       m->fiber_b1, m->fiber_w2, m->fiber_b2, m->fiber_wk, m->fk, m->C, m->D, m->L, m->O);
    ARREAU_CHECK_HIP(hipGetLastError());
    return ARREAU_OK;
}
```

arreau_amd/csrc/node_f16m.hip:

```cpp
#include <stdlib.h>
#include <utility>

#include "f16x3.h"
#include "internal.h"

namespace {
__device__ __forceinline__ float row16_sum_m(float v) {
    auto dpp = [](float x, auto ctrl) {
        return __builtin_bit_cast(float, __builtin_amdgcn_update_dpp(0, __builtin_bit_cast(int, x), decltype(ctrl)::value, 0xf, 0xf, false));
    };
    v += dpp(v, std::integral_constant<int, 0xB1>{});
    v += dpp(v, std::integral_constant<int, 0x4E>{});
    v += dpp(v, std::integral_constant<int, 0x141>{});
    v += dpp(v, std::integral_constant<int, 0x140>{});
    return v;
}
__device__ __forceinline__ float group4_sum(float v) {
    v += __shfl_xor(v, 16, 64);
    v += __shfl_xor(v, 32, 64);
    return v;
}
template <bool CLAMP, bool OWNED = false>
__device__ __forceinline__ void split8(const float (&v)[8], u32x4& hi, u32x4& lo) {
#pragma unroll
    for (int pp = 0; pp < 4; ++pp) {
        unsigned a, b;
        split_pair_act<OWNED>(f32x2{v[2 * pp], v[2 * pp + 1]}, a, b);
        hi[pp] = a;
        lo[pp] = b;
    }
}
}

template <int C, int H, int NW, int NB, int NSLOT>
__global__ __launch_bounds__(64 * NW, 2) void mlp_kernel_f16x3_m16(
    const float* __restrict__ x_conv,
    const float* __restrict__ x_in, float* __restrict__ x_out,
    const float* __restrict__ ln_w, const float* __restrict__ ln_b,
    const u32x4* __restrict__ stream,
    const float* __restrict__ mb1, const float* __restrict__ mb2, const float* __restrict__ ls,
    const float* __restrict__ wv,
    float bv, int n0, int N , int first_layer,
    float* __restrict__ xbar,
    float* __restrict__ vsum)
{
    static_assert(C == 128 && H == 512, "chunking below assumes C = 128, H = 512");
    constexpr int KC = C / 32;
    constexpr int HQ = H / 4, KH = HQ / 32;
    constexpr int NF = KC * 4;
    static_assert(KH == KC, "W1 and W2 quarter chunks have the same size");
    static_assert(NSLOT == 3 || NSLOT == 4, "ring depth");
    constexpr int P = NSLOT - 1;
    constexpr int PER = NF / NW;
    __shared__ u32x4 lds[NSLOT][NF * 64];
    __shared__ __attribute__((aligned(16))) float bias_s[H];
    __shared__ __attribute__((aligned(16))) float ep_s[3][C];

    const int wave = __builtin_amdgcn_readfirstlane(threadIdx.x >> 6), lane = threadIdx.x & 63;
    const int cp = lane & 15, gp = lane >> 4;
    const int tile = (int)blockIdx.x * NW + wave;
    const bool active = n0 + NB * tile < N;
    int nrow[NB];
    bool valid[NB];
#pragma unroll
    for (int nb = 0; nb < NB; ++nb) {
        const int n_i = n0 + NB * tile + nb;
        valid[nb] = n_i < N;
        nrow[nb] = valid[nb] ? n_i : N - 1;
    }

    const u32x4* dma_src = stream;
    dma_chunk<NF, NW>(dma_src, lds[0], wave, lane);
    dma_src += (size_t)NF * 64;
    dma_chunk<NF, NW>(dma_src, lds[1], wave, lane);
    dma_src += (size_t)NF * 64;
    if constexpr (P == 3) {
        dma_chunk<NF, NW>(dma_src, lds[2], wave, lane);
        dma_src += (size_t)NF * 64;
    }
    for (int i = threadIdx.x; i < H; i += 64 * NW) bias_s[i] = mb1[i];
    for (int i = threadIdx.x; i < C; i += 64 * NW) {
        ep_s[0][i] = mb2[i];
        ep_s[1][i] = ls[i];
        ep_s[2][i] = wv[i];
    }

    u32x4 xn[NB][KC][2];
#pragma unroll
    for (int nb = 0; nb < NB; ++nb) {
        const float* rowp = x_conv + ((size_t)nrow[nb] * 16 + cp) * C + 4 * gp;
        float x[KC][8];
        float sum = 0.f;
#pragma unroll
        for (int kb = 0; kb < KC; ++kb)
#pragma unroll
            for (int hf = 0; hf < 2; ++hf) {
                const f32x4 v = *reinterpret_cast<const f32x4*>(rowp + 32 * kb + 16 * hf);
#pragma unroll
                for (int r = 0; r < 4; ++r) x[kb][4 * hf + r] = v[r];
                sum += (v[0] + v[1]) + (v[2] + v[3]);
            }
        const float mean = group4_sum(sum) * (1.0f / C);
        float sq = 0.f;
#pragma unroll
        for (int kb = 0; kb < KC; ++kb)
#pragma unroll
            for (int e = 0; e < 8; ++e) {
                const float dlt = x[kb][e] - mean;
                x[kb][e] = dlt;
                sq += dlt * dlt;
            }
        const float rstd = 1.0f / sqrtf(group4_sum(sq) * (1.0f / C) + 1e-5f);
#pragma unroll
        for (int kb = 0; kb < KC; ++kb) {
#pragma unroll
            for (int hf = 0; hf < 2; ++hf) {
                const f32x4 gw = *reinterpret_cast<const f32x4*>(ln_w + 32 * kb + 16 * hf + 4 * gp);
                const f32x4 gb = *reinterpret_cast<const f32x4*>(ln_b + 32 * kb + 16 * hf + 4 * gp);
#pragma unroll
                for (int r = 0; r < 4; ++r) x[kb][4 * hf + r] = x[kb][4 * hf + r] * rstd * gw[r] + gb[r];
            }
            split8<true>(x[kb], xn[nb][kb][0], xn[nb][kb][1]);
        }
    }
    dma_wait();
    __syncthreads();

    f32x4v acc_o[KC][2][NB];
#pragma unroll
    for (int u = 0; u < KC; ++u)
#pragma unroll
        for (int mt = 0; mt < 2; ++mt)
#pragma unroll
            for (int nb = 0; nb < NB; ++nb) acc_o[u][mt][nb] = f32x4v{0.f, 0.f, 0.f, 0.f};

    int sl = 0;
    const unsigned lane16 = 16u * lane;
    const unsigned lds0 = __builtin_amdgcn_readfirstlane((unsigned)(size_t)&lds[0][0]) + 1024u * wave;
    int q = 0;
    constexpr int NCHUNK = 8 * 4;
    auto sync = [&]() {
        const int younger = min(max(NCHUNK - 2 - q, 0), P - 2);
        if (P == 3 && younger == 1) dma_wait_but<PER>();
        else dma_wait();
        __syncthreads();
        if (q + P < NCHUNK) dma_chunk_lean<NF, NW>(dma_src, lane16, wave, lds0 + (unsigned)(sl == 0 ? NSLOT - 1 : sl - 1) * (NF * 1024u));
        dma_src += (size_t)NF * 64;
        ++q;
    };
    constexpr int ST = KC;
#pragma unroll 1
    for (int w = 0; w < 4; ++w) {
        u32x4 hid[NB][KH][2];
#pragma unroll
        for (int u = 0; u < KH; ++u) {
            struct { f32x4v m[2][NB], x[2][NB]; } acc;
#pragma unroll
            for (int mt = 0; mt < 2; ++mt) {
                const f32x4 b = *reinterpret_cast<const f32x4*>(bias_s + w * HQ + 32 * u + 16 * mt + 4 * gp);
#pragma unroll
                for (int nb = 0; nb < NB; ++nb) {
                    acc.m[mt][nb] = f32x4v{b[0], b[1], b[2], b[3]};
                    acc.x[mt][nb] = f32x4v{0.f, 0.f, 0.f, 0.f};
                }
            }
            if (active) mma16_range<KC, 0, ST, NB>(acc.m, acc.x, lds[sl], xn, lane);
            sync();
            if (active) {
                mma16_range<KC, ST, 2 * KC, NB>(acc.m, acc.x, lds[sl], xn, lane);
#pragma unroll
                for (int nb = 0; nb < NB; ++nb) {
                    float v[8];
#pragma unroll
                    for (int mt = 0; mt < 2; ++mt)
#pragma unroll
                        for (int pr = 0; pr < 2; ++pr) {
                            const f32x2 pre = fma2(f32x2{acc.x[mt][nb][2 * pr], acc.x[mt][nb][2 * pr + 1]}, splat2(F16X3_INV_SCALE),
                                                   f32x2{acc.m[mt][nb][2 * pr], acc.m[mt][nb][2 * pr + 1]});
                            const f32x2 act = gelu_fast2(pre);
                            v[4 * mt + 2 * pr] = act.x;
                            v[4 * mt + 2 * pr + 1] = act.y;
                        }
                    split8<false>(v, hid[nb][u][0], hid[nb][u][1]);
                }
            }
            sl = sl == NSLOT - 1 ? 0 : sl + 1;
        }
#pragma unroll
        for (int u = 0; u < KC; ++u) {
            f32x4v cross[2][NB];
#pragma unroll
            for (int mt = 0; mt < 2; ++mt)
#pragma unroll
                for (int nb = 0; nb < NB; ++nb) cross[mt][nb] = f32x4v{0.f, 0.f, 0.f, 0.f};
            if (active) mma16_range<KH, 0, ST, NB>(acc_o[u], cross, lds[sl], hid, lane);
            sync();
            if (active) {
                mma16_range<KH, ST, 2 * KH, NB>(acc_o[u], cross, lds[sl], hid, lane);
#pragma unroll
                for (int mt = 0; mt < 2; ++mt)
#pragma unroll
                    for (int nb = 0; nb < NB; ++nb)
#pragma unroll
                        for (int r = 0; r < 4; ++r) acc_o[u][mt][nb][r] = fmaf(cross[mt][nb][r], F16X3_INV_SCALE, acc_o[u][mt][nb][r]);
            }
            sl = sl == NSLOT - 1 ? 0 : sl + 1;
        }
    }
    dma_wait();
    if (!active) return;

    int lane_e = lane;
    asm volatile("" : "+v"(lane_e));
    const int c = lane_e & 15, g = lane_e >> 4;
    const float inv16 = 1.0f / 16.0f;
    float vdot[NB];
#pragma unroll
    for (int nb = 0; nb < NB; ++nb) vdot[nb] = 0.f;
#pragma unroll
    for (int u = 0; u < KC; ++u)
#pragma unroll
        for (int mt = 0; mt < 2; ++mt) {
            const int c0 = 32 * u + 16 * mt + 4 * g;
            const f32x4 b2v = *reinterpret_cast<const f32x4*>(&ep_s[0][c0]);
            const f32x4 lsv = *reinterpret_cast<const f32x4*>(&ep_s[1][c0]);
            const f32x4 wvv = *reinterpret_cast<const f32x4*>(&ep_s[2][c0]);
#pragma unroll
            for (int nb = 0; nb < NB; ++nb) {
                const size_t off = ((size_t)nrow[nb] * 16 + c) * C + c0;
                const f32x4 xi = *reinterpret_cast<const f32x4*>(x_in + off);
                f32x4 xo;
#pragma unroll
                for (int r = 0; r < 4; ++r) xo[r] = (acc_o[u][mt][nb][r] + b2v[r]) * lsv[r] + xi[r];
                if (valid[nb]) *reinterpret_cast<f32x4*>(x_out + off) = xo;
#pragma unroll
                for (int r = 0; r < 4; ++r) vdot[nb] += xo[r] * wvv[r];
                f32x4 sum;
#pragma unroll
                for (int r = 0; r < 4; ++r) sum[r] = row16_sum_m(xo[r]);
                if (valid[nb] && c == 0) {
                    const f32x4 mean = {sum[0] * inv16, sum[1] * inv16, sum[2] * inv16, sum[3] * inv16};
                    *reinterpret_cast<f32x4*>(xbar + (size_t)nrow[nb] * C + c0) = mean;
                }
            }
        }
#pragma unroll
    for (int nb = 0; nb < NB; ++nb) {
        const float tot = group4_sum(vdot[nb]);
        if (valid[nb] && g == 0) {
            const size_t o = (size_t)nrow[nb] * 16 + c;
            vsum[o] = (first_layer ? 0.0f : vsum[o]) + (tot + bv);
        }
    }
}

namespace {
template <int NST>
__device__ __forceinline__ void load_steps(u32x4 (&w)[2 * NST], const u32x4* __restrict__ chunk, int st0, int lane) {
#pragma unroll
    for (int i = 0; i < NST; ++i) {
        w[2 * i] = chunk[(size_t)(st0 + i) * 128 + lane];
        w[2 * i + 1] = chunk[(size_t)(st0 + i) * 128 + 64 + lane];
    }
}
}

struct MlpTrainSave {
    float *xhat, *rstd, *xn, *hpre, *h, *out;
    float* x1 = nullptr;
    int kl_pitch = 0;
};
template <int C, int H, bool FUSE = false, bool TRAIN = false>
__global__ __launch_bounds__(512) void mlp_kernel_f16x3_m16_split(
    const float* __restrict__ x_conv, const float* __restrict__ x_in, float* __restrict__ x_out,
    const float* __restrict__ ln_w, const float* __restrict__ ln_b, const u32x4* __restrict__ stream,
    const float* __restrict__ mb1, const float* __restrict__ mb2, const float* __restrict__ ls,
    const float* __restrict__ wv, float bv, int n0, int first_layer, float* __restrict__ xbar, float* __restrict__ vsum,
    const float* __restrict__ kl , const int32_t* __restrict__ deg,
    const int32_t* __restrict__ src, const float* __restrict__ fk , const float* __restrict__ conv_bias,
    MlpTrainSave save) {
    static_assert(C == 128 && H == 512, "chunking below assumes C = 128, H = 512");
    constexpr int KC = C / 32, HQ = H / 4;
    constexpr int TS = 132;
    __shared__ u32x4 hidx[16][2][64];
    __shared__ f32x4 xo_s[8][64];
    __shared__ __attribute__((aligned(16))) float ctile[FUSE ? 16 * TS : 4];
    __shared__ __attribute__((aligned(16))) float xc_s[FUSE ? 16 * TS : 4];

    const int wave = __builtin_amdgcn_readfirstlane(threadIdx.x >> 6), lane = threadIdx.x & 63;
    const int q = wave >> 1, e = wave & 1;
    const int cp = lane & 15, gp = lane >> 4;
    const int n = n0 + blockIdx.x;
    const u32x4* qs = stream + (size_t)q * 8 * 1024;

    u32x4 wa[16], wb[16];
    load_steps<8>(wa, qs + (size_t)(2 * e) * 1024, 0, lane);
    load_steps<8>(wb, qs + (size_t)(2 * e + 1) * 1024, 0, lane);
    const int ou = wave >> 1, omt = wave & 1;
    const int ep_c0 = 32 * ou + 16 * omt + 4 * gp;
    const size_t ep_off = ((size_t)n * 16 + cp) * C + ep_c0;
    const f32x4 ep_b2 = *reinterpret_cast<const f32x4*>(mb2 + ep_c0);
    const f32x4 ep_ls = *reinterpret_cast<const f32x4*>(ls + ep_c0);
    const f32x4 ep_xi = *reinterpret_cast<const f32x4*>(x_in + ep_off);

    if constexpr (FUSE) {
        const int tid = threadIdx.x;
        const int c = tid & 127, pq = tid >> 7;
        const int c4 = tid & 31, o_row = tid >> 5;
        constexpr int K = 8;
        const int nd = min(deg[n], K);
        const int32_t* srow = src + (size_t)n * K;
        const size_t kp = TRAIN ? (size_t)save.kl_pitch : (size_t)C;
        const size_t kbase = ((size_t)n * K * 16 + o_row) * kp + 4 * c4;
        f32x4 kv[K], xv[K];
#pragma unroll
        for (int s_ = 0; s_ < K; ++s_) {
            const int sn = max(srow[s_], 0);
            kv[s_] = *reinterpret_cast<const f32x4*>(kl + kbase + (size_t)s_ * 16 * kp);
            xv[s_] = *reinterpret_cast<const f32x4*>(x_in + ((size_t)sn * 16 + o_row) * C + 4 * c4);
        }
        float fkr[16][4];
#pragma unroll
        for (int o = 0; o < 16; ++o)
#pragma unroll
            for (int p = 0; p < 4; ++p) fkr[o][p] = fk[((size_t)o * 16 + (4 * pq + p)) * C + c];
        const float cbias = conv_bias[c];
        f32x4 acc = {0.f, 0.f, 0.f, 0.f};
#pragma unroll
        for (int s_ = 0; s_ < K; ++s_) {
            const bool on = s_ < nd;
            acc[0] = on ? __fadd_rn(acc[0], __fmul_rn(kv[s_][0], xv[s_][0])) : acc[0];
            acc[1] = on ? __fadd_rn(acc[1], __fmul_rn(kv[s_][1], xv[s_][1])) : acc[1];
            acc[2] = on ? __fadd_rn(acc[2], __fmul_rn(kv[s_][2], xv[s_][2])) : acc[2];
            acc[3] = on ? __fadd_rn(acc[3], __fmul_rn(kv[s_][3], xv[s_][3])) : acc[3];
        }
        *reinterpret_cast<f32x4*>(&ctile[o_row * TS + 4 * c4]) = acc;
        if constexpr (TRAIN) *reinterpret_cast<f32x4*>(save.x1 + ((size_t)n * 16 + o_row) * C + 4 * c4) = acc;
        __syncthreads();
        float out[4] = {0.f, 0.f, 0.f, 0.f};
#pragma unroll
        for (int o = 0; o < 16; ++o) {
            const float xo = ctile[o * TS + c];
#pragma unroll
            for (int p = 0; p < 4; ++p) out[p] += xo * fkr[o][p];
        }
#pragma unroll
        for (int p = 0; p < 4; ++p) xc_s[(4 * pq + p) * TS + c] = TRAIN ? out[p] * (1.0f / 16.0f) + cbias : out[p] + cbias;
        __syncthreads();
    }

    u32x4 xn[KC][2];
    {
        const float* rowp = FUSE ? xc_s + cp * TS + 4 * gp : x_conv + ((size_t)n * 16 + cp) * C + 4 * gp;
        float x[KC][8];
        float sum = 0.f;
#pragma unroll
        for (int kb = 0; kb < KC; ++kb)
#pragma unroll
            for (int hf = 0; hf < 2; ++hf) {
                const f32x4 v = *reinterpret_cast<const f32x4*>(rowp + 32 * kb + 16 * hf);
#pragma unroll
                for (int r = 0; r < 4; ++r) x[kb][4 * hf + r] = v[r];
                sum += (v[0] + v[1]) + (v[2] + v[3]);
            }
        const float mean = group4_sum(sum) * (1.0f / C);
        float sq = 0.f;
#pragma unroll
        for (int kb = 0; kb < KC; ++kb)
#pragma unroll
            for (int i = 0; i < 8; ++i) {
                const float dlt = x[kb][i] - mean;
                x[kb][i] = dlt;
                sq += dlt * dlt;
            }
        const float rstd = 1.0f / sqrtf(group4_sum(sq) * (1.0f / C) + 1e-5f);
        if constexpr (TRAIN) {
            if (wave == 0 && gp == 0) save.rstd[(size_t)n * 16 + cp] = rstd;
        }
#pragma unroll
        for (int kb = 0; kb < KC; ++kb) {
#pragma unroll
            for (int hf = 0; hf < 2; ++hf) {
                const f32x4 gw = *reinterpret_cast<const f32x4*>(ln_w + 32 * kb + 16 * hf + 4 * gp);
                const f32x4 gb = *reinterpret_cast<const f32x4*>(ln_b + 32 * kb + 16 * hf + 4 * gp);
                if constexpr (TRAIN) {
                    if (wave == 0) {
                        const size_t o = ((size_t)n * 16 + cp) * C + 32 * kb + 16 * hf + 4 * gp;
                        f32x4 xh, xo;
#pragma unroll
                        for (int r = 0; r < 4; ++r) {
                            xh[r] = x[kb][4 * hf + r] * rstd;
                            xo[r] = x[kb][4 * hf + r] * rstd * gw[r] + gb[r];
                        }
                        *reinterpret_cast<f32x4*>(save.xhat + o) = xh;
                        *reinterpret_cast<f32x4*>(save.xn + o) = xo;
                    }
                }
#pragma unroll
                for (int r = 0; r < 4; ++r) x[kb][4 * hf + r] = x[kb][4 * hf + r] * rstd * gw[r] + gb[r];
            }
            split8<true, FUSE && TRAIN>(x[kb], xn[kb][0], xn[kb][1]);
        }
    }

    auto hidden_chunk = [&](const u32x4 (&w)[16], int j) {
        const int u = 2 * e + j;
        f32x4v am[2], ax[2];
#pragma unroll
        for (int mt = 0; mt < 2; ++mt) {
            const f32x4 b = *reinterpret_cast<const f32x4*>(mb1 + q * HQ + 32 * u + 16 * mt + 4 * gp);
            am[mt] = f32x4v{b[0], b[1], b[2], b[3]};
            ax[mt] = f32x4v{0.f, 0.f, 0.f, 0.f};
        }
#pragma unroll
        for (int st = 0; st < 2 * KC; ++st) {
            const int kb = st >> 1, mt = st & 1;
            am[mt] = mfma16_f16(w[2 * st], xn[kb][0], am[mt]);
            ax[mt] = mfma16_f16(w[2 * st + 1], xn[kb][0], ax[mt]);
            am[mt] = mfma16_f16(w[2 * st], xn[kb][1], am[mt]);
        }
        float v[8];
#pragma unroll
        for (int mt = 0; mt < 2; ++mt)
#pragma unroll
            for (int pr = 0; pr < 2; ++pr) {
                const f32x2 pre = fma2(f32x2{ax[mt][2 * pr], ax[mt][2 * pr + 1]}, splat2(F16X3_INV_SCALE),
                                       f32x2{am[mt][2 * pr], am[mt][2 * pr + 1]});
                const f32x2 act = gelu_fast2(pre);
                v[4 * mt + 2 * pr] = act.x;
                v[4 * mt + 2 * pr + 1] = act.y;
                if constexpr (TRAIN) {
                    const size_t o = ((size_t)n * 16 + cp) * H + q * HQ + 32 * u + 16 * mt + 4 * gp + 2 * pr;
                    typedef float f2v __attribute__((ext_vector_type(2)));
                    *reinterpret_cast<f2v*>(save.hpre + o) = f2v{pre.x, pre.y};
                    *reinterpret_cast<f2v*>(save.h + o) = f2v{act.x, act.y};
                }
            }
        u32x4 hi, lo;
        split8<false, FUSE && TRAIN>(v, hi, lo);
        hidx[4 * q + u][0][lane] = hi;
        hidx[4 * q + u][1][lane] = lo;
    };
    auto load_out = [&](u32x4 (&w)[16], int w0, int w2) {
        const u32x4* chunk = stream + ((size_t)w2 * 8 + 4 + ou) * 1024 + lane;
#pragma unroll
        for (int kb = 0; kb < 4; ++kb) {
            w[w0 + 2 * kb] = chunk[(size_t)(2 * kb + omt) * 128];
            w[w0 + 2 * kb + 1] = chunk[(size_t)(2 * kb + omt) * 128 + 64];
        }
    };
    hidden_chunk(wa, 0);
    load_out(wa, 0, 0);
    load_out(wa, 8, 1);
    hidden_chunk(wb, 1);
    load_out(wb, 0, 2);
    load_out(wb, 8, 3);
    __syncthreads();

    f32x4v acc = f32x4v{0.f, 0.f, 0.f, 0.f};
    auto quarter = [&](const u32x4 (&w)[16], auto w0c, int w2) {
        constexpr int w0 = decltype(w0c)::value;
        f32x4v cross = f32x4v{0.f, 0.f, 0.f, 0.f};
#pragma unroll
        for (int kb = 0; kb < 4; ++kb) {
            const u32x4 bh = hidx[4 * w2 + kb][0][lane], bl = hidx[4 * w2 + kb][1][lane];
            acc = mfma16_f16(w[w0 + 2 * kb], bh, acc);
            cross = mfma16_f16(w[w0 + 2 * kb + 1], bh, cross);
            acc = mfma16_f16(w[w0 + 2 * kb], bl, acc);
        }
#pragma unroll
        for (int r = 0; r < 4; ++r) acc[r] = fmaf(cross[r], F16X3_INV_SCALE, acc[r]);
    };
    quarter(wa, std::integral_constant<int, 0>{}, 0);
    quarter(wa, std::integral_constant<int, 8>{}, 1);
    quarter(wb, std::integral_constant<int, 0>{}, 2);
    quarter(wb, std::integral_constant<int, 8>{}, 3);

    {
        f32x4 xo;
#pragma unroll
        for (int r = 0; r < 4; ++r) xo[r] = (acc[r] + ep_b2[r]) * ep_ls[r] + ep_xi[r];
        *reinterpret_cast<f32x4*>(x_out + ep_off) = xo;
        if constexpr (TRAIN) {
            *reinterpret_cast<f32x4*>(save.out + ep_off) = f32x4{acc[0] + ep_b2[0], acc[1] + ep_b2[1], acc[2] + ep_b2[2], acc[3] + ep_b2[3]};
            return;
        }
        f32x4 sum;
#pragma unroll
        for (int r = 0; r < 4; ++r) sum[r] = row16_sum_m(xo[r]);
        if (cp == 0) {
            const float inv16 = 1.0f / 16.0f;
            const f32x4 mean = {sum[0] * inv16, sum[1] * inv16, sum[2] * inv16, sum[3] * inv16};
            *reinterpret_cast<f32x4*>(xbar + (size_t)n * C + ep_c0) = mean;
        }
        xo_s[wave][lane] = xo;
    }
    __syncthreads();
    if (wave != 0) return;
    float vdot = 0.f;
#pragma unroll
    for (int u = 0; u < KC; ++u)
#pragma unroll
        for (int mt = 0; mt < 2; ++mt) {
            const f32x4 xo = xo_s[2 * u + mt][lane];
            const f32x4 wvv = *reinterpret_cast<const f32x4*>(wv + 32 * u + 16 * mt + 4 * gp);
#pragma unroll
            for (int r = 0; r < 4; ++r) vdot += xo[r] * wvv[r];
        }
    const float tot = group4_sum(vdot);
    if (gp == 0) {
        const size_t o = (size_t)n * 16 + cp;
        vsum[o] = (first_layer ? 0.0f : vsum[o]) + (tot + bv);
    }
}

#define ARREAU_MLP_SPLIT_MAX_NODES 512
int arreau_launch_mlp_f16x3_m16_split(const arreau_model* m, int layer, const float* x_conv, const float* x_in, float* x_out,
                                      float* xbar, float* vsum, int N, hipStream_t s) {
    if (N <= 0) return ARREAU_OK;
    const int C = m->C, H = m->H;
    if (!(C == 128 && H == 512)) {
        arreau_set_error("mlp kernel (fp16x3, hidden split): unsupported (hidden_dim, widening_factor)");
        return ARREAU_EINVAL;
    }
    const size_t layer_u32x4 = (size_t)2 * H * C * 2 * 2 / 16;
    const u32x4* stream = reinterpret_cast<const u32x4*>(m->mlp_f16m) + (size_t)layer * layer_u32x4;
    ARREAU_LAUNCH((mlp_kernel_f16x3_m16_split<128, 512>), dim3((unsigned)N), dim3(512), 0, s, x_conv, x_in, x_out,
                       m->ln_w + (size_t)layer * C, m->ln_b + (size_t)layer * C, stream, m->mb1 + (size_t)layer * H,
                       m->mb2 + (size_t)layer * C, m->ls + (size_t)layer * C, m->ro_wv + (size_t)layer * C, m->ro_bv_host[layer],
                       0, layer == 0 ? 1 : 0, xbar + (size_t)layer * N * C, vsum, (const float*)nullptr, (const int32_t*)nullptr,
                       (const int32_t*)nullptr, (const float*)nullptr, (const float*)nullptr, MlpTrainSave{});
    ARREAU_CHECK_HIP(hipGetLastError());
    return ARREAU_OK;
}

bool arreau_small_layer_fusable(const arreau_model* m, int N) {
    const char* e = getenv("ARREAU_FUSE_SMALL");
    static const int split_env = [] { const char* v = getenv("ARREAU_MLP_SPLIT"); return v ? atoi(v) : -1; }();
    return (e == nullptr || atoi(e) != 0) && split_env < 0 && N <= ARREAU_MLP_SPLIT_MAX_NODES && m->mlp_variant == 3 &&
           m->f16_ok && m->k == 8 && m->C == 128 && m->H == 512 && (m->conv_variant == 1 || m->conv_variant == 2) && !arreau_k3(m) &&
           !arreau_basis_form(m, N);
}
int arreau_launch_small_layer(const arreau_model* m, int layer, const float* kbuf, const int32_t* deg, const int32_t* src,
                              const float* x_in, float* x_out, float* xbar, float* vsum, int Ntot, hipStream_t s) {
    if (Ntot <= 0) return ARREAU_OK;
    const int C = m->C, H = m->H;
    const size_t layer_u32x4 = (size_t)2 * H * C * 2 * 2 / 16;
    const u32x4* stream = reinterpret_cast<const u32x4*>(m->mlp_f16m) + (size_t)layer * layer_u32x4;
    const size_t layer_stride = (size_t)Ntot * m->k * 16 * C;
    ARREAU_LAUNCH((mlp_kernel_f16x3_m16_split<128, 512, true>), dim3((unsigned)Ntot), dim3(512), 0, s, (const float*)nullptr, x_in, x_out,
                       m->ln_w + (size_t)layer * C, m->ln_b + (size_t)layer * C, stream, m->mb1 + (size_t)layer * H,
                       m->mb2 + (size_t)layer * C, m->ls + (size_t)layer * C, m->ro_wv + (size_t)layer * C, m->ro_bv_host[layer],
                       0, layer == 0 ? 1 : 0, xbar + (size_t)layer * Ntot * C, vsum, kbuf + layer_stride * layer, deg, src,
                       m->fk + (size_t)layer * 16 * 16 * C, m->conv_bias + (size_t)layer * C, MlpTrainSave{});
    ARREAU_CHECK_HIP(hipGetLastError());
    return ARREAU_OK;
}

bool arreau_mlp_train_forward_available(const arreau_model* m) {
    const char* e = getenv("ARREAU_TRAIN_FUSED_MLP");
    return (!e || atoi(e) != 0) && m->C == 128 && m->H == 512 && m->mlp_f16m != nullptr;
}
int arreau_launch_mlp_train_forward(const arreau_model* m, int layer, const float* x_conv, const float* x_in, float* x_out, float* xhat,
                                    float* rstd, float* xn, float* hpre, float* h, float* out, int N, hipStream_t s,
                                    const float* kl, int kl_pitch, const int32_t* deg, const int32_t* src, const float* fk, float* x1) {
    if (N <= 0) return ARREAU_OK;
    const int C = m->C, H = m->H;
    const size_t layer_u32x4 = (size_t)2 * H * C * 2 * 2 / 16;
    const u32x4* stream = reinterpret_cast<const u32x4*>(m->mlp_f16m) + (size_t)layer * layer_u32x4;
    if (kl != nullptr) {
        ARREAU_REQUIRE(m->k == 8 && kl_pitch % 4 == 0 && deg && src && fk && x1, "fused training conv: k = 8 and 16-byte kernel rows");
        MlpTrainSave sv{xhat, rstd, xn, hpre, h, out};
        sv.x1 = x1; sv.kl_pitch = kl_pitch;
        ARREAU_LAUNCH((mlp_kernel_f16x3_m16_split<128, 512, true, true>), dim3((unsigned)N), dim3(512), 0, s, (const float*)nullptr, x_in, x_out,
                      m->ln_w + (size_t)layer * C, m->ln_b + (size_t)layer * C, stream, m->mb1 + (size_t)layer * H, m->mb2 + (size_t)layer * C,
                      m->ls + (size_t)layer * C, (const float*)nullptr, 0.0f, 0, 0, (float*)nullptr, (float*)nullptr, kl, deg, src, fk,
                      m->conv_bias + (size_t)layer * C, sv);
        ARREAU_CHECK_HIP(hipGetLastError());
        return ARREAU_OK;
    }
    ARREAU_LAUNCH((mlp_kernel_f16x3_m16_split<128, 512, false, true>), dim3((unsigned)N), dim3(512), 0, s, x_conv, x_in, x_out,
                  m->ln_w + (size_t)layer * C, m->ln_b + (size_t)layer * C, stream, m->mb1 + (size_t)layer * H, m->mb2 + (size_t)layer * C,
                  m->ls + (size_t)layer * C, (const float*)nullptr, 0.0f, 0, 0, (float*)nullptr, (float*)nullptr, (const float*)nullptr,
                  (const int32_t*)nullptr, (const int32_t*)nullptr, (const float*)nullptr, (const float*)nullptr,
                  MlpTrainSave{xhat, rstd, xn, hpre, h, out});
    ARREAU_CHECK_HIP(hipGetLastError());
    return ARREAU_OK;
}

namespace {
__global__ __launch_bounds__(256) void repack_mlp_f16x3_m16_kernel(const float* __restrict__ lin1 , const float* __restrict__ lin2 ,
                                                                    int L, unsigned short* __restrict__ q) {
    constexpr int C = 128, H = 512, HQ = 128;
    const long i = (long)blockIdx.x * 256 + threadIdx.x;
    const long per_mat = 4L * 4 * 2 * 64 * 8;
    if (i >= (long)L * 4 * 2 * per_mat) return;
    const int e = (int)(i & 7), lane = (int)((i >> 3) & 63), mt = (int)((i >> 9) & 1), kb = (int)((i >> 10) & 3), u = (int)((i >> 12) & 3);
    const int mat = (int)((i >> 14) & 1), w = (int)((i >> 15) & 3), l = (int)(i >> 17);
    const int g = lane >> 4;
    const int o = 32 * u + 16 * mt + (lane & 15);
    const int k = 32 * kb + 16 * (e >> 2) + 4 * g + (e & 3);
    const float v = mat == 0 ? lin1[((size_t)l * H + (size_t)w * HQ + o) * C + k] : lin2[((size_t)l * C + o) * H + (size_t)w * HQ + k];
    const _Float16 h1 = (_Float16)v;
    const _Float16 h2 = (_Float16)((v - (float)h1) * 2048.0f);
    const size_t base = (((size_t)l * 4 + w) * 2 + mat) * (size_t)(2 * per_mat) + (((size_t)u * 4 + kb) * 2 + mt) * 2 * 512 + (size_t)lane * 8 + e;
    q[base] = __builtin_bit_cast(unsigned short, h1);
    q[base + 512] = __builtin_bit_cast(unsigned short, h2);
}
}
int arreau_repack_mlp_f16x3_m16(arreau_model* m, hipStream_t s) {
    if (!(m->C == 128 && m->H == 512 && m->mlp_f16m)) return ARREAU_OK;
    const long n = (long)m->L * 4 * 2 * 16384;
    ARREAU_LAUNCH(repack_mlp_f16x3_m16_kernel, dim3((unsigned)((n + 255) / 256)), dim3(256), 0, s, m->t_lin1, m->t_lin2, m->L,
                  reinterpret_cast<unsigned short*>(const_cast<float*>(m->mlp_f16m)));
    ARREAU_CHECK_HIP(hipGetLastError());
    return ARREAU_OK;
}

int arreau_launch_mlp_f16x3_m16(const arreau_model* m, int layer, const float* x_conv, const float* x_in, float* x_out,
                                float* xbar, float* vsum, int N, hipStream_t s) {
    if (N <= 0) return ARREAU_OK;
    const int C = m->C, H = m->H;
    if (!(C == 128 && H == 512)) {
        arreau_set_error("mlp kernel (fp16x3, 16x16x32): unsupported (hidden_dim, widening_factor)");
        return ARREAU_EINVAL;
    }
    constexpr int NW = 4;
    const size_t layer_u32x4 = (size_t)2 * H * C * 2 * 2 / 16;
    static const int split_env = [] { const char* e = getenv("ARREAU_MLP_SPLIT"); return e ? atoi(e) : -1; }();
    if (split_env >= 0 ? split_env != 0 : N <= ARREAU_MLP_SPLIT_MAX_NODES)
        return arreau_launch_mlp_f16x3_m16_split(m, layer, x_conv, x_in, x_out, xbar, vsum, N, s);
    static const int nb_env = [] { const char* e = getenv("ARREAU_MLP_NB"); return e ? atoi(e) : 0; }();
    const int wave_slots = 8 * arreau_cu_count();
    const long long rounds1 = ((long long)N + wave_slots - 1) / wave_slots;
    const long long rounds2 = (((long long)N + 1) / 2 + wave_slots - 1) / wave_slots;
    const int nb = nb_env == 1 || nb_env == 2 ? nb_env : (6 * rounds1 < 10 * rounds2 ? 1 : 2);
    const long long tiles = ((long long)N + nb - 1) / nb;
    const dim3 grid((unsigned)((tiles + NW - 1) / NW)), block(64 * NW);
    const float* lnw = m->ln_w + (size_t)layer * C;
    const float* lnb = m->ln_b + (size_t)layer * C;
    const u32x4* stream = reinterpret_cast<const u32x4*>(m->mlp_f16m) + (size_t)layer * layer_u32x4;
    static const int slots = [] { const char* e = getenv("ARREAU_MLP_SLOTS"); return e && atoi(e) == 4 ? 4 : 3; }();
    auto launch = [&](auto kernel) {
        ARREAU_LAUNCH(kernel, grid, block, 0, s, x_conv, x_in, x_out, lnw, lnb, stream, m->mb1 + (size_t)layer * H,
                           m->mb2 + (size_t)layer * C, m->ls + (size_t)layer * C, m->ro_wv + (size_t)layer * C,
                           m->ro_bv_host[layer], 0, N, layer == 0 ? 1 : 0, xbar + (size_t)layer * N * C, vsum);
    };
    if (nb == 1 && slots == 4) launch(mlp_kernel_f16x3_m16<128, 512, NW, 1, 4>);
    else if (nb == 1) launch(mlp_kernel_f16x3_m16<128, 512, NW, 1, 3>);
    else if (slots == 4) launch(mlp_kernel_f16x3_m16<128, 512, NW, 2, 4>);
    else launch(mlp_kernel_f16x3_m16<128, 512, NW, 2, 3>);
    ARREAU_CHECK_HIP(hipGetLastError());
    return ARREAU_OK;
}
```

arreau_amd/engine.py:

```python
import ctypes
import math
import os

import torch

from . import _hip


def _f32(t):
    return t.detach().to("cpu", torch.float32).contiguous()


def _byref(struct):
    return ctypes.byref(struct) if struct is not None else None


def screen(frac, lattice, offsets, types=None, criteria=None):
    from .diffusion import screening
    return screening.screen(frac, lattice, offsets, types, criteria)


def pack_state(module):
    net = module.model
    sd = module.state_dict()
    L = net.num_layers
    S = module.num_atomic_states
    cfg = _hip.Config(
        num_atomic_states=S, hidden_dim=net.hidden_dim, basis_dim=net.basis_dim, num_layers=L,
        num_ori=net.num_ori, widening_factor=net.widening_factor, degree=net.degree,
        max_neighbors=int(module.diffusion_loss.max_neighbors), num_timesteps=int(module.diffusion_loss.T),
        radius=float(module.diffusion_loss.cutoff),
        has_layer_scale=int(f"model.interaction_layers.0.layer_scale" in sd and
                            sd["model.interaction_layers.0.layer_scale"] is not None))
    il = "model.interaction_layers.{}."
    stack = lambda fmt: torch.stack([_f32(sd[fmt.format(i)]) for i in range(L)], 0).contiguous()
    host = {
        "basis_w1": _f32(sd["model.basis_fn.1.weight"]), "basis_b1": _f32(sd["model.basis_fn.1.bias"]),
        "basis_w2": _f32(sd["model.basis_fn.3.weight"]), "basis_b2": _f32(sd["model.basis_fn.3.bias"]),
        "fiber_w1": _f32(sd["model.fiber_basis_fn.1.weight"]), "fiber_b1": _f32(sd["model.fiber_basis_fn.1.bias"]),
        "fiber_w2": _f32(sd["model.fiber_basis_fn.3.weight"]), "fiber_b2": _f32(sd["model.fiber_basis_fn.3.bias"]),
        "x_embedder_w": _f32(sd["model.x_embedder.weight"]),
        "conv_kernel_w": stack(il + "conv.kernel.weight"), "conv_fiber_w": stack(il + "conv.fiber_kernel.weight"),
        "conv_bias": stack(il + "conv.bias"), "norm_w": stack(il + "norm.weight"), "norm_b": stack(il + "norm.bias"),
        "linear1_w": stack(il + "linear_1.weight"), "linear1_b": stack(il + "linear_1.bias"),
        "linear2_w": stack(il + "linear_2.weight"), "linear2_b": stack(il + "linear_2.bias"),
        "readout_w": stack("model.read_out_layers.{}.weight"), "readout_b": stack("model.read_out_layers.{}.bias"),
        "ori_grid": _f32(net.ori_grid), "t_emb_w": _f32(sd["t_emb.gaussian_fourier_proj_w"]),
        "ve_sigmas": _f32(sd["diffusion_loss.pos_diffusion.sigmas"]),
        "vp_alpha_bars": _f32(sd["diffusion_loss.lattice_diffusion.alpha_bars"]),
        "vp_betas": _f32(sd["diffusion_loss.lattice_diffusion.betas"]),
        "q_one_step_transposed": _f32(sd["diffusion_loss.d3pm.q_one_step_transposed"]),
        "q_mats": _f32(sd["diffusion_loss.d3pm.q_mats"]),
    }
    if cfg.has_layer_scale:
        host["layer_scale"] = stack(il + "layer_scale")
    expect = {"basis_w1": (net.hidden_dim, 258), "x_embedder_w": (net.hidden_dim, S + 78),
              "readout_w": (L, S + 4, net.hidden_dim), "ori_grid": (net.num_ori, 3),
              "q_mats": (cfg.num_timesteps, S, S), "ve_sigmas": (cfg.num_timesteps + 1,)}
    for k, shp in expect.items():
        if tuple(host[k].shape) != shp:
            raise ValueError(f"state_dict entry for {k} has shape {tuple(host[k].shape)}, expected {shp}")
    csd = _hip.StateDict()
    for name in _hip._SD_FIELDS:
        t = host.get(name)
        setattr(csd, name, t.data_ptr() if t is not None else None)
    return cfg, host, csd, S, L


class HipEngine:
    def __init__(self, module, device):
        _hip.require_gpu()
        self.device = torch.device(device)
        cfg, host, csd, S, L = pack_state(module)
        self.cfg = cfg
        self._handle = ctypes.c_void_p()
        with torch.cuda.device(self.device):
            _hip.check(_hip.lib().arreau_model_create(ctypes.byref(cfg), ctypes.byref(csd),
                                                      _hip.stream_ptr(self.device), ctypes.byref(self._handle)),
                       "arreau_model_create")
        self._host_keepalive = host
        self._ws = None
        self._ws_cap = (0, 0)
        self.S, self.k = S, cfg.max_neighbors
        self.stale_for_sampling = False
        self.fused_shape = (cfg.hidden_dim, cfg.basis_dim, cfg.widening_factor) == (128, 256, 4)
        self._general = not self.fused_shape or bool(os.environ.get("ARREAU_GENERAL_PATH"))

    def close(self):
        if getattr(self, "_handle", None) is not None and self._handle.value:
            _hip.lib().arreau_model_destroy(self._handle)
            self._handle = ctypes.c_void_p()

    def __del__(self):
        try:
            self.close()
        except Exception:
            pass

    def status(self, reset=False):
        st = _hip.Status()
        _hip.check(_hip.lib().arreau_model_status(self._handle, ctypes.byref(st), int(bool(reset)),
                                                   _hip.stream_ptr(self.device)), "arreau_model_status")
        return {"flags": int(st.flags), "edge_kernel": _hip.EDGE_KERNELS.get(st.edge_kernel, "none"),
                "mlp_kernel": _hip.MLP_KERNELS.get(st.mlp_kernel, "none"), "edge_variant": int(st.edge_kernel),
                "mlp_variant": int(st.mlp_kernel), "conv_variant": int(st.conv_kernel),
                "basis_row_bytes": int(st.basis_row_bytes), "conv_cross_fp8": int(st.conv_cross_fp8), "edge_activation_bound": float(st.edge_activation_bound),
                "node_activation_bound": float(st.node_activation_bound),
                "basis_fp8_share": float(st.basis_fp8_share), "cross_fp8_share": float(st.cross_fp8_share),
                "readout_kernel": int(st.readout_kernel)}

    def check_status(self, reset=True):
        st = self.status(reset=reset)
        f = st["flags"]
        if f:
            why = []
            if f & _hip.STATUS_NONFINITE:
                why.append("a network output is inf/NaN (an activation left the fp16 range of the fp16x3 kernels, "
                           "or the inputs/weights are non-finite); ARREAU_EDGE_VARIANT=3 ARREAU_MLP_VARIANT=1 selects the "
                           "full-range bf16x6 kernels")
            if f & _hip.STATUS_BAD_TIMESTEP:
                why.append("a timestep index was outside the schedule")
            if f & _hip.STATUS_BAD_TYPE:
                why.append("an atom-type index was outside [0, num_atomic_states)")
            if f & _hip.STATUS_BAD_TIE:
                why.append("a lattice-system tie code was outside 0..2")
            if f & _hip.STATUS_BAD_SYMMETRY:
                why.append("a space-group symmetry table entry was out of range or inconsistent")
            raise _hip.ArreauHipError("arreau_hip status flags %d: %s" % (f, "; ".join(why)))
        return st

    def set_formats(self, basis_fp8=-1, cross_fp8=-1):
        _hip.check(_hip.lib().arreau_model_set_formats(self._handle, int(basis_fp8), int(cross_fp8)), "arreau_model_set_formats")

    def fp8_formats_in_use(self, st=None):
        st = self.status(reset=False) if st is None else st
        return st["conv_variant"] == 2 and (st["basis_row_bytes"] == 768 or st["conv_cross_fp8"] == 1)

    def checked(self, fn):
        out = fn()
        st = self.status(reset=False)
        if st["flags"] == _hip.STATUS_NONFINITE and self.fp8_formats_in_use(st):
            import warnings
            warnings.warn("arreau_amd: non-finite outputs with fp8 operand planes in use (a basis value beyond e4m3's range?); this "
                          "engine keeps two fp16 planes and three fp16 products from now on and the evaluation is repeated with them")
            self.set_formats(0, 0)
            self.status(reset=True)
            out = fn()
        self.check_status()
        return out

    def set_batch_layout(self, num_atoms, groups=0):
        if int(groups) > 1:
            raise ValueError(f"set_batch_layout: groups={int(groups)} is not supported; the library runs one stream over "
                             "the whole batch")

    def set_variant(self, edge=-1, mlp=-1):
        _hip.check(_hip.lib().arreau_model_set_variant(self._handle, int(edge), int(mlp)), "arreau_model_set_variant")
        if int(edge) >= 0:
            self._general = int(edge) == _hip.VARIANT_GENERAL

    def ponita_forward(self, x, vec, lattice, offsets, edges):
        dev = self.device
        N, B = x.shape[0], lattice.shape[0]
        if x.shape[1] != self.S + 74 or tuple(vec.shape) != (N, 4, 3):
            raise ValueError(f"x must be [N,{self.S + 74}] and vec [N,4,3]; got {tuple(x.shape)}, {tuple(vec.shape)}")
        logits = torch.empty((N, self.S), device=dev, dtype=torch.float32)
        vec_out = torch.empty((N, 1, 3), device=dev, dtype=torch.float32)
        gscalar = torch.empty((B, 3), device=dev, dtype=torch.float32)
        ws = self.workspace(N, B)
        deg, src, direction, dist = edges
        _hip.check(_hip.lib().arreau_ponita_forward(
            self._handle, _hip.ptr(x), _hip.ptr(vec), _hip.ptr(lattice), _hip.ptr(offsets), B, N, _hip.ptr(deg),
            _hip.ptr(src), _hip.ptr(direction), _hip.ptr(dist), _hip.ptr(logits), _hip.ptr(vec_out), _hip.ptr(gscalar),
            _hip.ptr(ws), ws.numel(), _hip.stream_ptr(dev)), "arreau_ponita_forward")
        return logits, vec_out, gscalar

    def sample_loop(self, frac, types, lengths, angles, offsets, t_start, n_steps, seed, const_types, lattice_out,
                    use_graph=False, fixed_lengths=None, condition=None, next_table=None, lattice_clipmax=0.999, corrector=None,
                    resampling=None, length_tie=None, symmetry=None):
        res = None
        if resampling is not None:
            from .diffusion.resampling import check_resampling
            passes, jump = check_resampling(*resampling[:2])
            ts = list(resampling[2]) if len(resampling) > 2 and resampling[2] is not None else None
            if passes > 1:
                if next_table is not None and ts is None:
                    raise ValueError("resampling on a respaced loop needs the host list of its timesteps")
                ts_arr = (ctypes.c_int32 * len(ts))(*ts) if ts else None
                res = _hip.ResamplingC(passes, jump, ctypes.cast(ts_arr, ctypes.POINTER(ctypes.c_int32)) if ts else None,
                                       len(ts) if ts else 0)
        if corrector is not None:
            from .diffusion.corrector import check_corrector
            corrector = check_corrector(*corrector)
        N, B = frac.shape[0], lengths.shape[0]
        ws = self.workspace(N, B)
        args = (self._handle, _hip.ptr(frac), _hip.ptr(types), _hip.ptr(lengths), _hip.ptr(angles), _hip.ptr(offsets), B, N,
                int(t_start), int(n_steps), int(seed) & (2 ** 64 - 1), _hip.ptr(const_types), _hip.ptr(fixed_lengths),
                _hip.ptr(lattice_out), _hip.ptr(ws), ws.numel(), int(bool(use_graph)))
        sched = None
        if next_table is not None:
            T = int(self.cfg.num_timesteps)
            if (tuple(next_table.shape) != (T + 1,) or next_table.dtype != torch.int32 or next_table.device != self.device
                    or not next_table.is_contiguous()):
                raise ValueError(f"next_table must be a contiguous int32 tensor of shape ({T + 1},) on {self.device}")
            sched = _hip.SampleScheduleC(_hip.ptr(next_table).value, float(lattice_clipmax))
        cond = self._condition_struct(condition, N, B) if condition is not None else None
        corr = _hip.CorrectorC(corrector[0], corrector[1]) if corrector is not None else None
        if length_tie is not None:
            self._check_tie(length_tie, B)
        opts = (_byref(cond), _byref(sched), _byref(corr), _byref(res))
        if symmetry is not None:
            name, opts = "arreau_sample_loop_sym", opts + (_hip.ptr(length_tie), _byref(self._symmetry_struct(symmetry, N)))
        elif length_tie is not None:
            name, opts = "arreau_sample_loop_tied", opts + (_hip.ptr(length_tie),)
        elif any(o is not None for o in opts):
            name = "arreau_sample_loop_resampled"
        else:
            name, opts = "arreau_sample_loop", ()
        _hip.check(getattr(_hip.lib(), name)(*args, *opts, _hip.stream_ptr(self.device)), name)

    def _check_tie(self, length_tie, B):
        if (tuple(length_tie.shape) != (B,) or length_tie.dtype != torch.int32 or length_tie.device != self.device
                or not length_tie.is_contiguous()):
            raise ValueError(f"length_tie must be a contiguous int32 tensor of shape ({B},) on {self.device}")

    def _symmetry_struct(self, tables, N):
        names = ("leader", "op", "orbit", "orbit_ptr", "orbit_atoms", "stab_ptr", "stab_ops", "rot", "rot_inv", "trans")
        missing = [n for n in names if tables.get(n) is None]
        if missing or set(tables) - set(names):
            raise ValueError(f"symmetry tables: expected exactly {names}")
        for n in names:
            t = tables[n]
            want = torch.float32 if n in ("rot", "rot_inv", "trans") else torch.int32
            if t.dtype != want or t.device != self.device or not t.is_contiguous() or t.numel() == 0:
                raise ValueError(f"symmetry tables: {n} must be a non-empty contiguous {want} tensor on {self.device}")
        for n in ("leader", "op", "orbit"):
            if tuple(tables[n].shape) != (N,):
                raise ValueError(f"symmetry tables: {n} must have shape ({N},)")
        n_orb = tables["orbit_ptr"].numel() - 1
        if tables["stab_ptr"].numel() != n_orb + 1 or n_orb < 1:
            raise ValueError("symmetry tables: orbit_ptr and stab_ptr must both hold n_orbits + 1 >= 2 entries")
        n_ops = tables["rot"].numel() // 9
        if tuple(tables["rot"].shape) != (n_ops, 9) or tuple(tables["rot_inv"].shape) != (n_ops, 9) or \
                tuple(tables["trans"].shape) != (n_ops, 3):
            raise ValueError("symmetry tables: rot / rot_inv must be [n_ops, 9] and trans [n_ops, 3]")
        return _hip.SymmetryC(*[_hip.ptr(tables[n]).value for n in names], n_orb, tables["orbit_atoms"].numel(),
                              tables["stab_ops"].numel(), n_ops)

    def condition_initial_state(self, frac, types, lengths, t_start, seed, condition):
        N, B = frac.shape[0], lengths.shape[0]
        cond = self._condition_struct(condition, N, B)
        _hip.check(_hip.lib().arreau_condition_initial_state(
            self._handle, _hip.ptr(frac), _hip.ptr(types), _hip.ptr(lengths), B, N, int(t_start), int(seed) & (2 ** 64 - 1),
            ctypes.byref(cond), _hip.stream_ptr(self.device)), "arreau_condition_initial_state")

    def _condition_struct(self, condition, N, B):
        spec = {"x0": ((N, 3), torch.float32), "pos_mask": ((N,), torch.uint8), "a0": ((N,), torch.int32),
                "type_mask": ((N,), torch.uint8), "l0": ((B, 3), torch.float32), "len_mask": ((B,), torch.uint8)}
        unknown = set(condition) - set(spec)
        if unknown:
            raise ValueError(f"condition: unknown entries {sorted(unknown)}")
        c = _hip.SampleConditionC()
        for name, (shape, dtype) in spec.items():
            t = condition.get(name)
            if t is None:
                continue
            if tuple(t.shape) != shape or t.dtype != dtype or t.device != self.device or not t.is_contiguous():
                raise ValueError(f"condition: {name} must be a contiguous {dtype} tensor of shape {shape} on {self.device}")
            setattr(c, name, _hip.ptr(t))
        return c

    def philox_fill(self, seed, timestep, kind, n, raw=False):
        out = torch.empty(n, device=self.device, dtype=torch.float32)
        words = torch.empty((n, 4), device=self.device, dtype=torch.int32) if raw else None
        _hip.check(_hip.lib().arreau_philox_fill(int(seed) & (2 ** 64 - 1), int(timestep), int(kind), int(n), _hip.ptr(out),
                                                 _hip.ptr(words), _hip.stream_ptr(self.device)), "arreau_philox_fill")
        return (out, words) if raw else out

    def philox_fill_word(self, seed, timestep, kind, word3, n, raw=False):
        out = torch.empty(n, device=self.device, dtype=torch.float32)
        words = torch.empty((n, 4), device=self.device, dtype=torch.int32) if raw else None
        _hip.check(_hip.lib().arreau_philox_fill_word(int(seed) & (2 ** 64 - 1), int(timestep), int(kind), int(word3) & (2 ** 32 - 1),
                                                      int(n), _hip.ptr(out), _hip.ptr(words), _hip.stream_ptr(self.device)),
                   "arreau_philox_fill_word")
        return (out, words) if raw else out

    def corrector_step(self, frac, t_crystal, offsets, eps, z_frac, snr, condition=None):
        from .diffusion.corrector import check_corrector
        _, snr = check_corrector(1, snr)
        N, B = frac.shape[0], t_crystal.shape[0]
        cond = self._condition_struct(condition, N, B) if condition is not None else None
        _hip.check(_hip.lib().arreau_corrector_step(
            self._handle, _hip.ptr(frac), _hip.ptr(t_crystal), _hip.ptr(offsets), B, N, _hip.ptr(eps), _hip.ptr(z_frac), snr,
            _byref(cond), _hip.stream_ptr(self.device)), "arreau_corrector_step")

    def diffusion_noise(self, frac0, types0, lattice0, t_crystal, offsets, z_frac, u_types, z_lengths):
        dev = self.device
        N, B = frac0.shape[0], lattice0.shape[0]
        f32 = dict(device=dev, dtype=torch.float32)
        out = dict(noisy_frac=torch.empty((N, 3), **f32), target_eps=torch.empty((N, 3), **f32),
                   noisy_types=torch.empty(N, device=dev, dtype=torch.int32), noisy_lengths=torch.empty((B, 3), **f32),
                   lengths=torch.empty((B, 3), **f32), angles=torch.empty((B, 3), **f32))
        inv = torch.empty((B, 3, 3), **f32)
        _hip.check(_hip.lib().arreau_diffusion_noise(
            self._handle, _hip.ptr(frac0), _hip.ptr(types0), _hip.ptr(lattice0), _hip.ptr(t_crystal), _hip.ptr(offsets),
            B, N, _hip.ptr(z_frac), _hip.ptr(u_types), _hip.ptr(z_lengths), _hip.ptr(out["noisy_frac"]),
            _hip.ptr(out["target_eps"]), _hip.ptr(out["noisy_types"]), _hip.ptr(out["noisy_lengths"]),
            _hip.ptr(out["lengths"]), _hip.ptr(out["angles"]), _hip.ptr(inv), _hip.stream_ptr(dev)),
            "arreau_diffusion_noise")
        return out

    def diffusion_losses(self, pred_eps, target_eps, logits, types0, noisy_types, t_crystal, pred_lengths, lengths,
                         offsets, with_grads=False):
        dev = self.device
        N, B = pred_eps.shape[0], pred_lengths.shape[0]
        f32 = dict(device=dev, dtype=torch.float32)
        terms = torch.empty((N, 3), **f32)
        losses = torch.empty(6, **f32)
        g = (torch.empty((N, 3), **f32), torch.empty((N, self.S), **f32), torch.empty((B, 3), **f32)) if with_grads \
            else (None, None, None)
        _hip.check(_hip.lib().arreau_diffusion_losses(
            self._handle, _hip.ptr(pred_eps), _hip.ptr(target_eps), _hip.ptr(logits), _hip.ptr(types0),
            _hip.ptr(noisy_types), _hip.ptr(t_crystal), _hip.ptr(pred_lengths), _hip.ptr(lengths), _hip.ptr(offsets), B, N,
            _hip.ptr(terms), _hip.ptr(losses), _hip.ptr(g[0]), _hip.ptr(g[1]), _hip.ptr(g[2]), _hip.stream_ptr(dev)),
            "arreau_diffusion_losses")
        return (losses, g) if with_grads else losses

    def train_forward(self, frac, types, lengths, angles, t_crystal, offsets):
        dev = self.device
        N, B = frac.shape[0], lengths.shape[0]
        eps = torch.empty((N, 3), device=dev, dtype=torch.float32)
        logits = torch.empty((N, self.S), device=dev, dtype=torch.float32)
        len0 = torch.empty((B, 3), device=dev, dtype=torch.float32)
        _hip.check(_hip.lib().arreau_train_forward(
            self._handle, _hip.ptr(frac), _hip.ptr(types), _hip.ptr(lengths), _hip.ptr(angles), _hip.ptr(t_crystal),
            _hip.ptr(offsets), B, N, _hip.ptr(eps), _hip.ptr(logits), _hip.ptr(len0), _hip.stream_ptr(dev)),
            "arreau_train_forward")
        return eps, logits, len0

    def train_backward(self, grad_eps, grad_logits, grad_len0):
        dev = self.device
        cfg = self.cfg
        S, C, D, L, W = self.S, cfg.hidden_dim, cfg.basis_dim, cfg.num_layers, cfg.widening_factor
        H = W * C
        shapes = {"basis_w1": (C, 258), "basis_b1": (C,), "basis_w2": (D, C), "basis_b2": (D,), "fiber_w1": (C, 3),
                  "fiber_b1": (C,), "fiber_w2": (D, C), "fiber_b2": (D,), "x_embedder_w": (C, S + 78),
                  "conv_kernel_w": (L, C, D), "conv_fiber_w": (L, C, D), "conv_bias": (L, C), "norm_w": (L, C),
                  "norm_b": (L, C), "linear1_w": (L, H, C), "linear1_b": (L, H), "linear2_w": (L, C, H),
                  "linear2_b": (L, C), "layer_scale": (L, C), "readout_w": (L, S + 4, C), "readout_b": (L, S + 4)}
        sizes = {k: -(-math.prod(v) // 4) * 4 for k, v in shapes.items()}
        flat = torch.zeros(sum(sizes.values()), device=dev, dtype=torch.float32)
        g, o = {}, 0
        for k, shp in shapes.items():
            g[k] = flat[o:o + math.prod(shp)].view(shp)
            o += sizes[k]
        csd = _hip.StateDict()
        for name in _hip._SD_FIELDS:
            t = g.get(name)
            setattr(csd, name, t.data_ptr() if t is not None else None)
        _hip.check(_hip.lib().arreau_train_backward(self._handle, _hip.ptr(grad_eps), _hip.ptr(grad_logits),
                                                    _hip.ptr(grad_len0), ctypes.byref(csd), _hip.stream_ptr(dev)),
                   "arreau_train_backward")
        self.last_grad_flat = flat
        return {name: (g[field] if l is None else g[field][l]) for name, field, l in self._state_names()}

    def _state_names(self):
        names = getattr(self, "_state_names_cache", None)
        if names is None:
            cfg = self.cfg
            names = [("model.basis_fn.1.weight", "basis_w1", None), ("model.basis_fn.1.bias", "basis_b1", None),
                     ("model.basis_fn.3.weight", "basis_w2", None), ("model.basis_fn.3.bias", "basis_b2", None),
                     ("model.fiber_basis_fn.1.weight", "fiber_w1", None), ("model.fiber_basis_fn.1.bias", "fiber_b1", None),
                     ("model.fiber_basis_fn.3.weight", "fiber_w2", None), ("model.fiber_basis_fn.3.bias", "fiber_b2", None),
                     ("model.x_embedder.weight", "x_embedder_w", None)]
            il = "model.interaction_layers.{}."
            per_layer = {"conv.kernel.weight": "conv_kernel_w", "conv.fiber_kernel.weight": "conv_fiber_w", "conv.bias": "conv_bias",
                         "norm.weight": "norm_w", "norm.bias": "norm_b", "linear_1.weight": "linear1_w",
                         "linear_1.bias": "linear1_b", "linear_2.weight": "linear2_w", "linear_2.bias": "linear2_b"}
            if cfg.has_layer_scale:
                per_layer["layer_scale"] = "layer_scale"
            for l in range(cfg.num_layers):
                for key, field in per_layer.items():
                    names.append((il.format(l) + key, field, l))
                names.append((f"model.read_out_layers.{l}.weight", "readout_w", l))
                names.append((f"model.read_out_layers.{l}.bias", "readout_b", l))
            self._state_names_cache = names
        return names

    def update_train_weights(self, module):
        dev = self.device
        plan = getattr(self, "_train_weight_plan", None)
        params = getattr(module, "_named_parameter_cache", None)
        if params is None:
            params = dict(module.named_parameters())
        if plan is None or plan["module"] is not module or any(p.data_ptr() != q for p, q in zip(plan["src"], plan["ptrs"])):
            L = self.cfg.num_layers
            bufs, dst, src = {}, [], []
            for name, field, l in self._state_names():
                p = params[name]
                if field not in bufs:
                    bufs[field] = torch.empty(((L,) if l is not None else ()) + tuple(p.shape), device=dev, dtype=torch.float32)
                dst.append(bufs[field] if l is None else bufs[field][l])
                src.append(p)
            csd = _hip.StateDict()
            for name in _hip._SD_FIELDS:
                t = bufs.get(name)
                setattr(csd, name, t.data_ptr() if t is not None else None)
            plan = {"module": module, "bufs": bufs, "dst": dst, "src": src, "ptrs": [p.data_ptr() for p in src], "csd": csd}
            self._train_weight_plan = plan
        with torch.no_grad():
            torch._foreach_copy_(plan["dst"], [p.detach() for p in plan["src"]])
        _hip.check(_hip.lib().arreau_model_update_train_weights(self._handle, ctypes.byref(plan["csd"]), _hip.stream_ptr(dev)),
                   "arreau_model_update_train_weights")
        self.stale_for_sampling = not self._general

    def train_weight_mirrors(self, module):
        cached = getattr(self, "_mirror_cache", None)
        params = getattr(module, "_named_parameter_cache", None)
        if params is None:
            params = dict(module.named_parameters())
        if cached is not None and cached[0] is module and all(p.data_ptr() == q for p, q in cached[2]):
            return cached[1]
        csd = _hip.StateDict()
        _hip.check(_hip.lib().arreau_model_train_weight_pointers(self._handle, ctypes.byref(csd)), "arreau_model_train_weight_pointers")
        mirrors = {}
        for name, field, l in self._state_names():
            base = getattr(csd, field)
            p = params[name]
            if base:
                mirrors[p] = int(base) + 4 * p.numel() * (l or 0)
        self._mirror_cache = (module, mirrors, [(p, p.data_ptr()) for p in mirrors])
        return mirrors

    def refresh_derived_train_weights(self, module):
        params = getattr(module, "_named_parameter_cache", None)
        if params is None:
            params = dict(module.named_parameters())
        _hip.check(_hip.lib().arreau_model_refresh_derived_train_weights(
            self._handle, _hip.ptr(params["model.basis_fn.1.weight"].detach()), _hip.ptr(params["model.x_embedder.weight"].detach()),
            _hip.stream_ptr(self.device)), "arreau_model_refresh_derived_train_weights")
        self.stale_for_sampling = not self._general

    def conv_stats(self):
        st = torch.empty((self.cfg.num_layers, 3), device=self.device, dtype=torch.float32)
        _hip.check(_hip.lib().arreau_train_conv_stats(self._handle, _hip.ptr(st), _hip.stream_ptr(self.device)),
                   "arreau_train_conv_stats")
        return st

    def workspace(self, N, B):
        if self._ws is None or N > self._ws_cap[0] or B > self._ws_cap[1]:
            capN, capB = max(N, self._ws_cap[0]), max(B, self._ws_cap[1])
            nbytes = _hip.lib().arreau_workspace_bytes(ctypes.byref(self.cfg), capN, capB)
            self._ws = None
            self._ws = torch.empty(nbytes, dtype=torch.uint8, device=self.device)
            self._ws_cap = (capN, capB)
        return self._ws

    def predict_scores(self, frac, types, lengths, angles, t_crystal, offsets, edges=None, return_edges=False):
        dev = self.device
        N, B = frac.shape[0], lengths.shape[0]
        eps = torch.empty((N, 3), device=dev, dtype=torch.float32)
        logits = torch.empty((N, self.S), device=dev, dtype=torch.float32)
        len0 = torch.empty((B, 3), device=dev, dtype=torch.float32)
        ws = self.workspace(N, B)
        if edges is not None:
            deg, src, direction, dist = edges
            given = 1
        elif return_edges:
            k = self.k
            deg = torch.empty(N, device=dev, dtype=torch.int32)
            src = torch.empty((N, k), device=dev, dtype=torch.int32)
            direction = torch.empty((N, k, 3), device=dev, dtype=torch.float32)
            dist = torch.empty((N, k), device=dev, dtype=torch.float32)
            given = 0
        else:
            deg = src = direction = dist = None
            given = 0
        _hip.check(_hip.lib().arreau_predict_scores(
            self._handle, _hip.ptr(frac), _hip.ptr(types), _hip.ptr(lengths), _hip.ptr(angles), _hip.ptr(t_crystal),
            _hip.ptr(offsets), B, N, given, _hip.ptr(deg), _hip.ptr(src), _hip.ptr(direction), _hip.ptr(dist),
            _hip.ptr(eps), _hip.ptr(logits), _hip.ptr(len0), _hip.ptr(ws), ws.numel(), _hip.stream_ptr(dev)),
            "arreau_predict_scores")
        if return_edges:
            return eps, logits, len0, (deg, src, direction, dist)
        return eps, logits, len0

    def reverse_step(self, frac, types, lengths, angles, t_crystal, offsets, eps, logits, len0, z_lattice, z_frac,
                     u_types, lattice_out):
        B, N = lengths.shape[0], frac.shape[0]
        _hip.check(_hip.lib().arreau_reverse_step(
            self._handle, _hip.ptr(frac), _hip.ptr(types), _hip.ptr(lengths), _hip.ptr(angles), _hip.ptr(t_crystal),
            _hip.ptr(offsets), B, N, _hip.ptr(eps), _hip.ptr(logits), _hip.ptr(len0), _hip.ptr(z_lattice),
            _hip.ptr(z_frac), _hip.ptr(u_types), _hip.ptr(lattice_out), _hip.stream_ptr(self.device)),
            "arreau_reverse_step")

    def _reverse_step_to(self, name, frac, types, lengths, angles, t_crystal, s_crystal, offsets, eps, logits, len0, z_lattice, z_frac,
                         u_types, lattice_out, lattice_clipmax, *options):
        B, N = lengths.shape[0], frac.shape[0]
        _hip.check(getattr(_hip.lib(), name)(
            self._handle, _hip.ptr(frac), _hip.ptr(types), _hip.ptr(lengths), _hip.ptr(angles), _hip.ptr(t_crystal),
            _hip.ptr(s_crystal), _hip.ptr(offsets), B, N, _hip.ptr(eps), _hip.ptr(logits), _hip.ptr(len0), _hip.ptr(z_lattice),
            _hip.ptr(z_frac), _hip.ptr(u_types), _hip.ptr(lattice_out), float(lattice_clipmax), *options,
            _hip.stream_ptr(self.device)), name)

    def reverse_step_to(self, frac, types, lengths, angles, t_crystal, s_crystal, offsets, eps, logits, len0, z_lattice, z_frac,
                        u_types, lattice_out, lattice_clipmax=0.999):
        self._reverse_step_to("arreau_reverse_step_to", frac, types, lengths, angles, t_crystal, s_crystal, offsets, eps, logits, len0,
                              z_lattice, z_frac, u_types, lattice_out, lattice_clipmax)

    def reverse_step_tied(self, frac, types, lengths, angles, t_crystal, s_crystal, offsets, eps, logits, len0, z_lattice, z_frac,
                          u_types, lattice_out, length_tie, lattice_clipmax=0.999):
        self._check_tie(length_tie, lengths.shape[0])
        self._reverse_step_to("arreau_reverse_step_tied", frac, types, lengths, angles, t_crystal, s_crystal, offsets, eps, logits, len0,
                              z_lattice, z_frac, u_types, lattice_out, lattice_clipmax, _hip.ptr(length_tie))

    def reverse_step_sym(self, frac, types, lengths, angles, t_crystal, s_crystal, offsets, eps, logits, len0, z_lattice, z_frac,
                         u_types, lattice_out, length_tie, symmetry, lattice_clipmax=0.999):
        if length_tie is not None:
            self._check_tie(length_tie, lengths.shape[0])
        sym = self._symmetry_struct(symmetry, frac.shape[0]) if symmetry is not None else None
        self._reverse_step_to("arreau_reverse_step_sym", frac, types, lengths, angles, t_crystal, s_crystal, offsets, eps, logits, len0,
                              z_lattice, z_frac, u_types, lattice_out, lattice_clipmax, _hip.ptr(length_tie), _byref(sym))

    def resample_jump(self, frac, types, lengths, angles, s_crystal, t_crystal, offsets, z_frac, z_lengths, u_types, lattice_out,
                      const_types=None, fixed_lengths=None, condition=None, length_tie=None):
        B, N = lengths.shape[0], frac.shape[0]
        cond = self._condition_struct(condition, N, B) if condition is not None else None
        name, tie = "arreau_resample_jump", ()
        if length_tie is not None:
            self._check_tie(length_tie, B)
            name, tie = "arreau_resample_jump_tied", (_hip.ptr(length_tie),)
        _hip.check(getattr(_hip.lib(), name)(
            self._handle, _hip.ptr(frac), _hip.ptr(types), _hip.ptr(lengths), _hip.ptr(angles), _hip.ptr(s_crystal),
            _hip.ptr(t_crystal), _hip.ptr(offsets), B, N, _hip.ptr(z_frac), _hip.ptr(z_lengths), _hip.ptr(u_types),
            _hip.ptr(const_types), _hip.ptr(fixed_lengths), _byref(cond), _hip.ptr(lattice_out), *tie,
            _hip.stream_ptr(self.device)), name)

    def screen(self, frac, lattice, offsets, types=None, criteria=None):
        from .diffusion import screening
        if frac.device != self.device:
            raise ValueError(f"screen: the state must be on {self.device}")
        return screening.screen(frac, lattice, offsets, types, criteria)

    def edges_to_slots(self, edge_index, dists, direction, N):
        dev, k = self.device, self.k
        ei = edge_index.to(device=dev, dtype=torch.int64).contiguous()
        E = ei.shape[1]
        d = dists.to(device=dev, dtype=torch.float32).contiguous()
        dr = direction.to(device=dev, dtype=torch.float32).contiguous()
        deg = torch.empty(N, device=dev, dtype=torch.int32)
        src = torch.empty((N, k), device=dev, dtype=torch.int32)
        sdir = torch.empty((N, k, 3), device=dev, dtype=torch.float32)
        sdist = torch.empty((N, k), device=dev, dtype=torch.float32)
        status = torch.zeros(1, device=dev, dtype=torch.int32)
        _hip.check(_hip.lib().arreau_edges_to_slots(_hip.ptr(ei), _hip.ptr(d), _hip.ptr(dr), E, N, k, _hip.ptr(deg),
                                                     _hip.ptr(src), _hip.ptr(sdir), _hip.ptr(sdist), _hip.ptr(status),
                                                     _hip.stream_ptr(dev)), "arreau_edges_to_slots")
        if int(status.item()) != 0:
            raise ValueError(f"edge list must be receiver-sorted with at most {k} in-edges per node")
        return deg, src, sdir, sdist
```

include/arreau_hip.h:

```cpp
#ifndef ARREAU_HIP_H
#define ARREAU_HIP_H

#include <stddef.h>
#include <stdint.h>

#ifdef __cplusplus
extern "C" {
#endif

#define ARREAU_OK 0
#define ARREAU_EINVAL (-1)
#define ARREAU_EHIP (-2)
#define ARREAU_ECAPACITY (-3)

typedef struct arreau_config {
    int32_t num_atomic_states;
    int32_t hidden_dim;
    int32_t basis_dim;
    int32_t num_layers;
    int32_t num_ori;
    int32_t widening_factor;
    int32_t degree;
    int32_t max_neighbors;
    int32_t num_timesteps;
    float radius;
    int32_t has_layer_scale;
} arreau_config;

#define ARREAU_MAX_K 8
#define ARREAU_T_EMB_DIM 64
#define ARREAU_N_CRYSTAL_FEATS 10

typedef struct arreau_state_dict {
    const float* basis_w1;
    const float* basis_b1;
    const float* basis_w2;
    const float* basis_b2;
    const float* fiber_w1;
    const float* fiber_b1;
    const float* fiber_w2;
    const float* fiber_b2;
    const float* x_embedder_w;
    const float* conv_kernel_w;
    const float* conv_fiber_w;
    const float* conv_bias;
    const float* norm_w;
    const float* norm_b;
    const float* linear1_w;
    const float* linear1_b;
    const float* linear2_w;
    const float* linear2_b;
    const float* layer_scale;
    const float* readout_w;
    const float* readout_b;
    const float* ori_grid;
    const float* t_emb_w;
    const float* ve_sigmas;
    const float* vp_alpha_bars;
    const float* vp_betas;
    const float* q_one_step_transposed;
    const float* q_mats;
} arreau_state_dict;

typedef struct arreau_model arreau_model;

const char* arreau_last_error(void);
const char* arreau_version(void);

int arreau_model_create(const arreau_config* cfg, const arreau_state_dict* h_sd, void* stream,
                        arreau_model** out_model);
void arreau_model_destroy(arreau_model* model);
int arreau_model_config(const arreau_model* model, arreau_config* out_cfg);

#define ARREAU_STATUS_NONFINITE 1
#define ARREAU_STATUS_BAD_TIMESTEP 2
#define ARREAU_STATUS_BAD_TYPE 4
#define ARREAU_STATUS_BAD_TIE 8
#define ARREAU_STATUS_BAD_SYMMETRY 16
typedef struct arreau_status {
    int32_t flags;
    int32_t edge_kernel;
    int32_t mlp_kernel;
    int32_t conv_kernel;
    int32_t basis_row_bytes;
    int32_t conv_cross_fp8;
    float edge_activation_bound;
    float node_activation_bound;
    float basis_fp8_share;
    float cross_fp8_share;
    int32_t readout_kernel;
} arreau_status;
int arreau_model_status(const arreau_model* model, arreau_status* out, int32_t reset, void* stream);
int arreau_model_set_formats(arreau_model* model, int32_t basis_fp8, int32_t cross_fp8);
int arreau_model_set_variant(arreau_model* model, int32_t edge_variant, int32_t mlp_variant);

size_t arreau_workspace_bytes(const arreau_config* cfg, int64_t max_atoms, int64_t max_crystals);


int arreau_lattice_from_params(const float* d_lengths, const float* d_angles, int32_t B,
                               float* d_lattice, void* stream);

int arreau_frac_to_cart(const float* d_frac, const float* d_lattice, const int32_t* d_crystal_offsets,
                        int32_t B, int32_t N, float* d_cart, void* stream);

int arreau_radius_graph_pbc(const float* d_cart, const float* d_lattice,
                            const int32_t* d_crystal_offsets, int32_t B, int32_t N,
                            float radius, int32_t k,
                            int32_t* d_deg, int32_t* d_src, int32_t* d_cell, float* d_dir,
                            float* d_dist, void* stream);

int arreau_compact_edges(const int32_t* d_deg, const int32_t* d_src, const int32_t* d_cell,
                         const float* d_dir, const float* d_dist, int32_t N, int32_t k,
                         int32_t* d_edge_offsets, int64_t* d_edge_index ,
                         float* d_cell_offsets , float* d_out_dist, float* d_out_dir,
                         void* stream);

int arreau_edges_to_slots(const int64_t* d_edge_index , const float* d_dist,
                          const float* d_dir, int64_t E, int32_t N, int32_t k,
                          int32_t* d_deg, int32_t* d_src, float* d_slot_dir, float* d_slot_dist,
                          int32_t* d_status, void* stream);

#define ARREAU_SCREEN_NONFINITE 1
#define ARREAU_SCREEN_CELL 2
#define ARREAU_SCREEN_CLOSE 4
#define ARREAU_SCREEN_MASKED 8
#define ARREAU_SCREEN_BEYOND 16
#define ARREAU_SCREEN_INVALID_MASK 15
#define ARREAU_SCREEN_MAX_SHELLS 8
typedef struct arreau_screen_criteria {
    float min_distance;
    float min_volume;
    float search_radius;
    int32_t mask_type;
    int32_t max_shells;
} arreau_screen_criteria;
typedef struct arreau_screen_result {
    float* min_distance;
    int32_t* pair;
    int32_t* n_close;
    float* volume;
    float* number_density;
    int32_t* flags;
} arreau_screen_result;
int arreau_crystal_screen(const float* d_frac, const int32_t* d_types , const float* d_lattice ,
                          const int32_t* d_crystal_offsets, int32_t B, int32_t N, const arreau_screen_criteria* crit,
                          arreau_screen_result* out , void* stream);

#define ARREAU_FP_NONFINITE 1
#define ARREAU_FP_CELL 2
#define ARREAU_FP_MANY_SPECIES 4
#define ARREAU_FP_EMPTY 8
#define ARREAU_FP_MAX_SPECIES 8
#define ARREAU_FP_BINS 64
#define ARREAU_FP_COMPONENTS 36
#define ARREAU_FP_ROW (ARREAU_FP_COMPONENTS * ARREAU_FP_BINS)
typedef struct arreau_fingerprint_params {
    float r_max;
    float sigma;
    int32_t n_bins;
    int32_t max_shells;
} arreau_fingerprint_params;
typedef struct arreau_fingerprint_result {
    float* fingerprint;
    int32_t* species;
    int32_t* counts;
    int32_t* flags;
} arreau_fingerprint_result;
typedef struct arreau_match_result {
    int32_t* duplicate_of;
    float* distance;
    int32_t* nearest;
    float* nearest_distance;
} arreau_match_result;
int arreau_crystal_fingerprint(const float* d_frac, const int32_t* d_types, const float* d_lattice, const int32_t* d_crystal_offsets,
                               int32_t B, int32_t N, const arreau_fingerprint_params* params, arreau_fingerprint_result* out,
                               void* stream);
int arreau_fingerprint_match(const arreau_fingerprint_result* x, int32_t Bx, const arreau_fingerprint_result* y, int32_t By,
                             float tolerance, arreau_match_result* out, void* stream);


int arreau_predict_scores(const arreau_model* model,
                          const float* d_frac, const int32_t* d_types, const float* d_lengths,
                          const float* d_angles, const int32_t* d_t,
                          const int32_t* d_crystal_offsets, int32_t B, int32_t N,
                          int32_t use_given_edges,
                          int32_t* d_deg, int32_t* d_src, float* d_dir, float* d_dist,
                          float* d_eps, float* d_logits, float* d_len0,
                          void* d_workspace, size_t workspace_bytes, void* stream);

int arreau_ponita_forward(const arreau_model* model, const float* d_x, const float* d_vec, const float* d_lattice,
                          const int32_t* d_crystal_offsets, int32_t B, int32_t N,
                          const int32_t* d_deg, const int32_t* d_src, const float* d_dir, const float* d_dist,
                          float* d_logits, float* d_vec_out, float* d_global_scalar,
                          void* d_workspace, size_t workspace_bytes, void* stream);

int arreau_reverse_step(const arreau_model* model,
                        float* d_frac, int32_t* d_types, float* d_lengths, const float* d_angles,
                        const int32_t* d_t, const int32_t* d_crystal_offsets, int32_t B, int32_t N,
                        const float* d_eps, const float* d_logits, const float* d_len0,
                        const float* d_z_lattice, const float* d_z_frac, const float* d_u_types,
                        float* d_lattice, void* stream);

int arreau_sample_loop(arreau_model* model, float* d_frac, int32_t* d_types, float* d_lengths, const float* d_angles,
                       const int32_t* d_crystal_offsets, int32_t B, int32_t N, int32_t t_start, int32_t n_steps,
                       uint64_t seed, const int32_t* d_const_types, const float* d_fixed_lengths, float* d_lattice,
                       void* d_workspace, size_t workspace_bytes, int32_t use_graph, void* stream);

typedef struct arreau_sample_condition {
    const float* x0;
    const uint8_t* pos_mask;
    const int32_t* a0;
    const uint8_t* type_mask;
    const float* l0;
    const uint8_t* len_mask;
} arreau_sample_condition;

int arreau_sample_loop_conditioned(arreau_model* model, float* d_frac, int32_t* d_types, float* d_lengths, const float* d_angles,
                                   const int32_t* d_crystal_offsets, int32_t B, int32_t N, int32_t t_start, int32_t n_steps,
                                   uint64_t seed, const int32_t* d_const_types, const float* d_fixed_lengths, float* d_lattice,
                                   void* d_workspace, size_t workspace_bytes, int32_t use_graph,
                                   const arreau_sample_condition* cond, void* stream);

int arreau_condition_initial_state(const arreau_model* model, float* d_frac, int32_t* d_types, float* d_lengths, int32_t B,
                                   int32_t N, int32_t t_start, uint64_t seed, const arreau_sample_condition* cond,
                                   void* stream);

typedef struct arreau_sample_schedule {
    const int32_t* d_next;
    float lattice_clipmax;
} arreau_sample_schedule;

int arreau_sample_loop_scheduled(arreau_model* model, float* d_frac, int32_t* d_types, float* d_lengths, const float* d_angles,
                                 const int32_t* d_crystal_offsets, int32_t B, int32_t N, int32_t t_start, int32_t n_steps,
                                 uint64_t seed, const int32_t* d_const_types, const float* d_fixed_lengths, float* d_lattice,
                                 void* d_workspace, size_t workspace_bytes, int32_t use_graph,
                                 const arreau_sample_condition* cond, const arreau_sample_schedule* schedule, void* stream);

int arreau_reverse_step_to(const arreau_model* model,
                           float* d_frac, int32_t* d_types, float* d_lengths, const float* d_angles,
                           const int32_t* d_t, const int32_t* d_s, const int32_t* d_crystal_offsets, int32_t B, int32_t N,
                           const float* d_eps, const float* d_logits, const float* d_len0,
                           const float* d_z_lattice, const float* d_z_frac, const float* d_u_types,
                           float* d_lattice, float lattice_clipmax, void* stream);

#define ARREAU_MAX_CORRECTOR_STEPS 16
typedef struct {
    int32_t steps;
    float snr;
} arreau_corrector;

int arreau_sample_loop_corrected(arreau_model* model, float* d_frac, int32_t* d_types, float* d_lengths, const float* d_angles,
                                 const int32_t* d_crystal_offsets, int32_t B, int32_t N, int32_t t_start, int32_t n_steps,
                                 uint64_t seed, const int32_t* d_const_types, const float* d_fixed_lengths, float* d_lattice,
                                 void* d_workspace, size_t workspace_bytes, int32_t use_graph,
                                 const arreau_sample_condition* cond, const arreau_sample_schedule* schedule,
                                 const arreau_corrector* corrector, void* stream);

int arreau_corrector_step(const arreau_model* model, float* d_frac, const int32_t* d_t, const int32_t* d_crystal_offsets,
                          int32_t B, int32_t N, const float* d_eps, const float* d_z_frac, float snr,
                          const arreau_sample_condition* condition, void* stream);

#define ARREAU_MAX_RESAMPLE_PASSES 64
typedef struct {
    int32_t passes;
    int32_t jump_length;
    const int32_t* timesteps;
    int32_t n_timesteps;
} arreau_resampling;

int arreau_sample_loop_resampled(arreau_model* model, float* d_frac, int32_t* d_types, float* d_lengths, const float* d_angles,
                                 const int32_t* d_crystal_offsets, int32_t B, int32_t N, int32_t t_start, int32_t n_steps,
                                 uint64_t seed, const int32_t* d_const_types, const float* d_fixed_lengths, float* d_lattice,
                                 void* d_workspace, size_t workspace_bytes, int32_t use_graph,
                                 const arreau_sample_condition* cond, const arreau_sample_schedule* schedule,
                                 const arreau_corrector* corrector, const arreau_resampling* resampling, void* stream);

int arreau_resample_jump(const arreau_model* model, float* d_frac, int32_t* d_types, float* d_lengths, const float* d_angles,
                         const int32_t* d_s, const int32_t* d_t, const int32_t* d_crystal_offsets, int32_t B, int32_t N,
                         const float* d_z_frac, const float* d_z_lengths, const float* d_u_types,
                         const int32_t* d_const_types, const float* d_fixed_lengths,
                         const arreau_sample_condition* cond, float* d_lattice, void* stream);


int arreau_sample_loop_tied(arreau_model* model, float* d_frac, int32_t* d_types, float* d_lengths, const float* d_angles,
                            const int32_t* d_crystal_offsets, int32_t B, int32_t N, int32_t t_start, int32_t n_steps,
                            uint64_t seed, const int32_t* d_const_types, const float* d_fixed_lengths, float* d_lattice,
                            void* d_workspace, size_t workspace_bytes, int32_t use_graph,
                            const arreau_sample_condition* cond, const arreau_sample_schedule* schedule,
                            const arreau_corrector* corrector, const arreau_resampling* resampling, const int32_t* d_length_tie,
                            void* stream);

int arreau_reverse_step_tied(const arreau_model* model,
                             float* d_frac, int32_t* d_types, float* d_lengths, const float* d_angles,
                             const int32_t* d_t, const int32_t* d_s, const int32_t* d_crystal_offsets, int32_t B, int32_t N,
                             const float* d_eps, const float* d_logits, const float* d_len0,
                             const float* d_z_lattice, const float* d_z_frac, const float* d_u_types,
                             float* d_lattice, float lattice_clipmax, const int32_t* d_length_tie, void* stream);

int arreau_resample_jump_tied(const arreau_model* model, float* d_frac, int32_t* d_types, float* d_lengths, const float* d_angles,
                              const int32_t* d_s, const int32_t* d_t, const int32_t* d_crystal_offsets, int32_t B, int32_t N,
                              const float* d_z_frac, const float* d_z_lengths, const float* d_u_types,
                              const int32_t* d_const_types, const float* d_fixed_lengths,
                              const arreau_sample_condition* cond, float* d_lattice, const int32_t* d_length_tie, void* stream);

typedef struct arreau_symmetry {
    const int32_t* leader;
    const int32_t* op;
    const int32_t* orbit;
    const int32_t* orbit_ptr;
    const int32_t* orbit_atoms;
    const int32_t* stab_ptr;
    const int32_t* stab_ops;
    const float* rot;
    const float* rot_inv;
    const float* trans;
    int32_t n_orbits, n_orbit_atoms, n_stab_ops, n_ops;
} arreau_symmetry;

int arreau_sample_loop_sym(arreau_model* model, float* d_frac, int32_t* d_types, float* d_lengths, const float* d_angles,
                           const int32_t* d_crystal_offsets, int32_t B, int32_t N, int32_t t_start, int32_t n_steps,
                           uint64_t seed, const int32_t* d_const_types, const float* d_fixed_lengths, float* d_lattice,
                           void* d_workspace, size_t workspace_bytes, int32_t use_graph,
                           const arreau_sample_condition* cond, const arreau_sample_schedule* schedule,
                           const arreau_corrector* corrector, const arreau_resampling* resampling, const int32_t* d_length_tie,
                           const arreau_symmetry* symmetry, void* stream);

int arreau_reverse_step_sym(const arreau_model* model,
                            float* d_frac, int32_t* d_types, float* d_lengths, const float* d_angles,
                            const int32_t* d_t, const int32_t* d_s, const int32_t* d_crystal_offsets, int32_t B, int32_t N,
                            const float* d_eps, const float* d_logits, const float* d_len0,
                            const float* d_z_lattice, const float* d_z_frac, const float* d_u_types,
                            float* d_lattice, float lattice_clipmax, const int32_t* d_length_tie, const arreau_symmetry* symmetry,
                            void* stream);

int arreau_philox_fill(uint64_t seed, int32_t timestep, int32_t kind, int64_t n, float* d_out, uint32_t* d_raw,
                       void* stream);
int arreau_philox_fill_word(uint64_t seed, int32_t timestep, int32_t kind, uint32_t word3, int64_t n, float* d_out,
                            uint32_t* d_raw, void* stream);


int arreau_diffusion_noise(const arreau_model* model, const float* d_frac0, const int32_t* d_types0,
                           const float* d_lattice0, const int32_t* d_t, const int32_t* d_crystal_offsets,
                           int32_t B, int32_t N, const float* d_z_frac, const float* d_u_types,
                           const float* d_z_lengths, float* d_noisy_frac, float* d_target_eps,
                           int32_t* d_noisy_types, float* d_noisy_lengths, float* d_lengths, float* d_angles,
                           float* d_inv_lattice, void* stream);

int arreau_diffusion_losses(const arreau_model* model, const float* d_pred_eps, const float* d_target_eps,
                            const float* d_logits, const int32_t* d_types0, const int32_t* d_noisy_types,
                            const int32_t* d_t, const float* d_pred_lengths, const float* d_lengths,
                            const int32_t* d_crystal_offsets, int32_t B, int32_t N, float* d_terms,
                            float* d_losses, float* d_grad_eps, float* d_grad_logits, float* d_grad_lengths,
                            void* stream);

int arreau_train_forward(arreau_model* model, const float* d_frac, const int32_t* d_types, const float* d_lengths,
                         const float* d_angles, const int32_t* d_t, const int32_t* d_crystal_offsets, int32_t B,
                         int32_t N, float* d_eps, float* d_logits, float* d_len0, void* stream);

int arreau_train_backward(arreau_model* model, const float* d_grad_eps, const float* d_grad_logits,
                          const float* d_grad_len0, const arreau_state_dict* d_grads, void* stream);

int arreau_model_update_train_weights(arreau_model* model, const arreau_state_dict* d_sd, void* stream);

int arreau_train_conv_stats(arreau_model* model, float* d_stats, void* stream);

#define ARREAU_OPT_MAX_GROUPS 4
typedef struct arreau_optimizer arreau_optimizer;
typedef struct {
    int64_t step;
    double lr[ARREAU_OPT_MAX_GROUPS];
    double weight_decay[ARREAU_OPT_MAX_GROUPS];
    double beta1, beta2, eps;
    double max_norm;
} arreau_adam_args;
int arreau_optimizer_create(int32_t n_tensors, void* const* d_params, void* const* d_mirrors, const int64_t* numel,
                            const int64_t* flat_offset, const int32_t* group, int32_t n_groups, int64_t flat_len,
                            arreau_optimizer** out);
int arreau_optimizer_step(arreau_optimizer* opt, const float* d_flat_grad, float* d_exp_avg, float* d_exp_avg_sq,
                          const arreau_adam_args* args, float* d_norm_out, void* stream);
int arreau_optimizer_step_ema(arreau_optimizer* opt, const float* d_flat_grad, float* d_exp_avg, float* d_exp_avg_sq,
                              const arreau_adam_args* args, float* d_ema, double decay, float* d_norm_out, void* stream);
void arreau_optimizer_destroy(arreau_optimizer* opt);
int arreau_model_train_weight_pointers(arreau_model* model, arreau_state_dict* out);
int arreau_model_refresh_derived_train_weights(arreau_model* model, const float* d_basis_w1, const float* d_x_embedder_w,
                                               void* stream);

int arreau_debug_sgemm(int32_t mode, int32_t M, int32_t N, int32_t K, const float* d_A, int64_t as0, int64_t as1, const float* d_B,
                       int64_t bs0, int64_t bs1, float* d_C, int32_t ldc, float alpha, float beta, void* stream);

int arreau_profile_edge_kernel(int32_t enable);
int arreau_edge_kernel_time_ms(double* mean_ms, int64_t* launches);
int arreau_conv_kernel_time_ms(double* mean_ms, int64_t* launches);

int arreau_debug_set_pollution(uint32_t pattern);
int arreau_debug_leftover_fraction(uint32_t pattern, double* lds_fraction, double* reg_fraction, void* stream);

#ifdef __cplusplus
}
#endif
#endif
```

Measured before the change: 189,900.

## Pre-scale MLP fp16x3 weight planes by power-of-two to drop cross-plane rescale

After: 188,000. -1.0%, worse.

```diff
diff --git a/arreau_amd/_hip.py b/arreau_amd/_hip.py
--- a/arreau_amd/_hip.py
+++ b/arreau_amd/_hip.py
@@ -12,7 +12,7 @@
     "arreau_model_config", "arreau_workspace_bytes", "arreau_lattice_from_params", "arreau_frac_to_cart",
     "arreau_radius_graph_pbc", "arreau_compact_edges", "arreau_edges_to_slots", "arreau_predict_scores",
     "arreau_reverse_step", "arreau_profile_edge_kernel", "arreau_edge_kernel_time_ms", "arreau_conv_kernel_time_ms",
-    "arreau_model_status", "arreau_model_set_variant", "arreau_ponita_forward",
+    "arreau_model_status", "arreau_model_set_variant", "arreau_ponita_forward", "arreau_model_read_mlp_planes",
     "arreau_diffusion_noise", "arreau_diffusion_losses", "arreau_sample_loop", "arreau_philox_fill",
     "arreau_train_forward", "arreau_train_backward", "arreau_train_conv_stats", "arreau_model_update_train_weights",
     "arreau_debug_sgemm", "arreau_optimizer_create", "arreau_optimizer_step", "arreau_optimizer_destroy",
@@ -102,7 +102,8 @@
 class Status(Structure):
     _fields_ = [("flags", c_int32), ("edge_kernel", c_int32), ("mlp_kernel", c_int32), ("conv_kernel", c_int32),
                 ("basis_row_bytes", c_int32), ("conv_cross_fp8", c_int32), ("edge_activation_bound", c_float), ("node_activation_bound", c_float),
-                ("basis_fp8_share", c_float), ("cross_fp8_share", c_float), ("readout_kernel", c_int32)]
+                ("basis_fp8_share", c_float), ("cross_fp8_share", c_float), ("readout_kernel", c_int32),
+                ("mlp_scale_linear1", c_int32 * 16), ("mlp_scale_linear2", c_int32 * 16), ("node_activation_bound_scaled", c_float)]
 
 
 _SD_FIELDS = [
@@ -139,6 +140,7 @@
         "arreau_reverse_step": [vp] * 7 + [i32, i32] + [vp] * 8,
         "arreau_model_status": [vp, POINTER(Status), i32, vp],
         "arreau_model_set_variant": [vp, i32, i32],
+        "arreau_model_read_mlp_planes": [vp, i32, vp, c_size_t, vp],
         "arreau_model_set_formats": [vp, i32, i32],
         "arreau_ponita_forward": [vp] * 5 + [i32, i32] + [vp] * 7 + [vp, c_size_t, vp],
         "arreau_diffusion_noise": [vp] * 6 + [i32, i32] + [vp] * 11,
diff --git a/arreau_amd/csrc/f16x3.h b/arreau_amd/csrc/f16x3.h
--- a/arreau_amd/csrc/f16x3.h
+++ b/arreau_amd/csrc/f16x3.h
@@ -45,6 +45,26 @@
     return r;
 }
 __device__ __forceinline__ float gelu_fast(float x) { return gelu_fast2(splat2(x)).x; }
+struct GeluScaled { float clamp, c[7]; };
+static inline GeluScaled gelu_scaled_make(int s) {
+    const float c[7] = {3.3092788558903113e-05f, -7.6921945996487589e-04f, 8.0807156986535972e-03f, -5.3412102790454205e-02f,
+                        -4.5877097453124149e-01f, -1.1512017015627947e+00f, -9.9999306107072172e-01f};
+    GeluScaled g;
+    g.clamp = ldexpf(12.0f, s);
+    for (int i = 0; i < 7; ++i) g.c[i] = ldexpf(c[i], -s * (6 - i));
+    return g;
+}
+__device__ __forceinline__ f32x2 gelu_fast2_scaled(f32x2 x, const GeluScaled& g) {
+    const float ax = fabsf(x.x), ay = fabsf(x.y);
+    const f32x2 a = f32x2{__builtin_amdgcn_fmed3f(ax, -INFINITY, g.clamp), __builtin_amdgcn_fmed3f(ay, -INFINITY, g.clamp)};
+    f32x2 q = fma2(splat2(g.c[0]), a, splat2(g.c[1]));
+#pragma unroll
+    for (int i = 2; i < 7; ++i) q = fma2(q, a, splat2(g.c[i]));
+    f32x2 r;
+    r.x = fmaf(-ax, __builtin_amdgcn_exp2f(q.x), __builtin_amdgcn_fmed3f(x.x, 0.0f, INFINITY));
+    r.y = fmaf(-ay, __builtin_amdgcn_exp2f(q.y), __builtin_amdgcn_fmed3f(x.y, 0.0f, INFINITY));
+    return r;
+}
 
 struct Planes2 { u32x4 p[2][2]; };
 
@@ -231,33 +251,39 @@
 };
 
 template <int NKB, int ST0, int ST1, int NB = 2>
-__device__ __forceinline__ void mma16_range(f32x4v (&am)[2][NB], f32x4v (&ax)[2][NB], const u32x4* __restrict__ buf,
+__device__ __forceinline__ void mma16_range(f32x4v (&acc)[2][NB], const u32x4* __restrict__ buf,
                                             const u32x4 (&b)[NB][NKB][2], int lane) {
+    constexpr int G = NB == 1 ? 2 : 1;
+    static_assert(ST0 % G == 0 && ST1 % G == 0, "mma16_range: whole groups of steps");
     const u32x4* f = buf + lane;
-    u32x4 a1[2], a2[2];
-    auto frag = [&](u32x4& d, const u32x4& src) { d = src; };
-    frag(a1[ST0 & 1], f[(size_t)ST0 * 128]);
-    frag(a2[ST0 & 1], f[(size_t)ST0 * 128 + 64]);
-#pragma unroll
-    for (int st = ST0; st < ST1; ++st) {
-        const int slot = st & 1, nslot = slot ^ 1;
-        if (st + 1 < ST1) {
-            frag(a1[nslot], f[(size_t)(st + 1) * 128]);
-            frag(a2[nslot], f[(size_t)(st + 1) * 128 + 64]);
-        }
-        const int kb = st >> 1, mt = st & 1;
-#pragma unroll
-        for (int nb = 0; nb < NB; ++nb) {
-            am[mt][nb] = mfma16_f16(a1[slot], b[nb][kb][0], am[mt][nb]);
-            ax[mt][nb] = mfma16_f16(a2[slot], b[nb][kb][0], ax[mt][nb]);
-            am[mt][nb] = mfma16_f16(a1[slot], b[nb][kb][1], am[mt][nb]);
-        }
-    }
-    __builtin_amdgcn_sched_group_barrier(0x100, 2, 0);
-#pragma unroll
-    for (int st = ST0; st < ST1; ++st) {
-        if (st + 1 < ST1) __builtin_amdgcn_sched_group_barrier(0x100, 2, 0);
-        __builtin_amdgcn_sched_group_barrier(0x008, 3 * NB, 0);
+    u32x4 a[2][G][2];
+    auto load = [&](int slot, int st) {
+#pragma unroll
+        for (int j = 0; j < G; ++j) {
+            a[slot][j][0] = f[(size_t)(st + j) * 128];
+            a[slot][j][1] = f[(size_t)(st + j) * 128 + 64];
+        }
+    };
+    load((ST0 / G) & 1, ST0);
+#pragma unroll
+    for (int st = ST0; st < ST1; st += G) {
+        const int slot = (st / G) & 1, nslot = slot ^ 1;
+        if (st + G < ST1) load(nslot, st + G);
+#pragma unroll
+        for (int p = 0; p < 3; ++p)
+#pragma unroll
+            for (int j = 0; j < G; ++j)
+#pragma unroll
+                for (int nb = 0; nb < NB; ++nb) {
+                    const int kb = (st + j) >> 1, mt = (st + j) & 1;
+                    acc[mt][nb] = mfma16_f16(a[slot][j][p == 1 ? 1 : 0], b[nb][kb][p == 2 ? 1 : 0], acc[mt][nb]);
+                }
+    }
+    __builtin_amdgcn_sched_group_barrier(0x100, 2 * G, 0);
+#pragma unroll
+    for (int st = ST0; st < ST1; st += G) {
+        if (st + G < ST1) __builtin_amdgcn_sched_group_barrier(0x100, 2 * G, 0);
+        __builtin_amdgcn_sched_group_barrier(0x008, 3 * G * NB, 0);
     }
 }
 
diff --git a/arreau_amd/csrc/internal.h b/arreau_amd/csrc/internal.h
--- a/arreau_amd/csrc/internal.h
+++ b/arreau_amd/csrc/internal.h
@@ -114,6 +114,8 @@
     int train_full_range;
     int calibrating;
     float edge_act_bound, node_act_bound;
+    int mlp_s1[16], mlp_s2[16];
+    float node_act_bound_scaled;
     int edge_variant, mlp_variant, conv_variant, readout_variant;
     mutable int ran_edge, ran_mlp, ran_conv, ran_x8, ran_readout;
     const float *t_w1f, *t_w2, *t_wk, *t_lin1, *t_lin2, *t_ro_w;
diff --git a/arreau_amd/csrc/model.hip b/arreau_amd/csrc/model.hip
--- a/arreau_amd/csrc/model.hip
+++ b/arreau_amd/csrc/model.hip
@@ -124,7 +124,8 @@
     return wmax;
 }
 
-static float pack_linear_f16x3_m16(const float* W, int out_dim, int in_dim, int in_stride, uint16_t* Q, bool native = false) {
+static float pack_linear_f16x3_m16(const float* W, int out_dim, int in_dim, int in_stride, uint16_t* Q, bool native = false,
+                                   const int* scale_log2 = nullptr) {
     const int U = out_dim / 32, KB = in_dim / 32;
     float wmax = 0.f;
     for (int u = 0; u < U; ++u)
@@ -138,8 +139,9 @@
                                               : 32 * kb + 16 * (g & 1) + 8 * (e >> 2) + 4 * (g >> 1) + (e & 3);
                         const float w = W[(size_t)out * in_stride + in];
                         wmax = fabsf(w) > wmax ? fabsf(w) : wmax;
-                        const uint16_t h1 = f32_to_f16_rne(w);
-                        const uint16_t h2 = f32_to_f16_rne((w - f16_to_f32(h1)) * 2048.0f);
+                        const float ws = scale_log2 ? ldexpf(w, *scale_log2) : w;
+                        const uint16_t h1 = f32_to_f16_rne(ws);
+                        const uint16_t h2 = f32_to_f16_rne(scale_log2 ? ws - f16_to_f32(h1) : (w - f16_to_f32(h1)) * 2048.0f);
                         const size_t base = (((size_t)u * KB + kb) * 2 + mt) * 2 * 512 + (size_t)lane * 8 + e;
                         Q[base] = h1;
                         Q[base + 512] = h2;
@@ -358,7 +360,17 @@
                            sd->vp_alpha_bars, sd->vp_betas, sd->q_one_step_transposed, sd->q_mats};
     for (const float* p : need) ARREAU_REQUIRE(p != nullptr, "arreau_model_create: missing state_dict entry");
 
-    float edge_bound = 0.f, node_bound = 0.f;
+    float edge_bound = 0.f, node_bound = 0.f, node_bound_scaled = 0.f;
+    int mlp_s1[16] = {0}, mlp_s2[16] = {0};
+    ARREAU_REQUIRE(L <= 16, "arreau_model_create: at most 16 layers");
+    auto plane_scale = [](const float* w, size_t n) {
+        float wmax = 0.f;
+        for (size_t i = 0; i < n; ++i) wmax = fmaxf(wmax, fabsf(w[i]));
+        if (!(wmax > 0.f) || !std::isfinite(wmax)) return 0;
+        int e;
+        frexpf(wmax, &e);
+        return std::min(std::max(2 - e, 0), 8);
+    };
     {
         std::vector<float> w1f_b;
         fold_poly_weight(sd->basis_w1, C, w1f_b);
@@ -383,19 +395,26 @@
             basis_max = std::max(basis_max, a);
         }
         edge_bound = (float)std::max(mono_max, std::max(h1_max, basis_max));
-        double nb = 0.0;
+        double nb = 0.0, nbs = 0.0;
         for (int l = 0; l < L; ++l) {
             const float* g = sd->norm_w + (size_t)l * C;
             const float* be = sd->norm_b + (size_t)l * C;
             for (int i = 0; i < C; ++i) nb = std::max(nb, sqrt((double)C - 1.0) * fabs((double)g[i]) + fabs((double)be[i]));
+            double hb = 0.0;
             for (int j = 0; j < H; ++j) {
                 const float* w = sd->linear1_w + ((size_t)l * H + j) * C;
                 double n2 = 0.0, dot = 0.0;
                 for (int i = 0; i < C; ++i) { n2 += (double)w[i] * g[i] * (double)w[i] * g[i]; dot += (double)w[i] * be[i]; }
-                nb = std::max(nb, sqrt((double)C) * sqrt(n2) + fabs(dot) + fabs((double)sd->linear1_b[(size_t)l * H + j]));
+                hb = std::max(hb, sqrt((double)C) * sqrt(n2) + fabs(dot) + fabs((double)sd->linear1_b[(size_t)l * H + j]));
             }
+            nb = std::max(nb, hb);
+            mlp_s1[l] = plane_scale(sd->linear1_w + (size_t)l * H * C, (size_t)H * C);
+            mlp_s2[l] = plane_scale(sd->linear2_w + (size_t)l * C * H, (size_t)C * H);
+            while (mlp_s1[l] > 0 && !(ldexp(hb, mlp_s1[l]) <= 65504.0)) --mlp_s1[l];
+            nbs = std::max(nbs, ldexp(hb, mlp_s1[l]));
         }
         node_bound = (float)nb;
+        node_bound_scaled = (float)std::max(nb, nbs);
     }
 
     BlobBuilder bb;
@@ -488,8 +507,8 @@
     for (int l = 0; l < L && fused; ++l)
         for (int w = 0; w < 4; ++w) {
             uint16_t* dst = reinterpret_cast<uint16_t*>(bb.data.data() + off_mlpf16m) + ((size_t)l * 4 + w) * (fq1 + fq2);
-            pack_linear_f16x3_m16(sd->linear1_w + ((size_t)l * H + (size_t)w * HQ) * C, HQ, C, C, dst, true);
-            pack_linear_f16x3_m16(sd->linear2_w + (size_t)l * C * H + (size_t)w * HQ, C, HQ, H, dst + fq1, true);
+            pack_linear_f16x3_m16(sd->linear1_w + ((size_t)l * H + (size_t)w * HQ) * C, HQ, C, C, dst, true, &mlp_s1[l]);
+            pack_linear_f16x3_m16(sd->linear2_w + (size_t)l * C * H + (size_t)w * HQ, C, HQ, H, dst + fq1, true, &mlp_s2[l]);
         }
     const size_t off_mb1 = bb.put(sd->linear1_b, (size_t)L * H);
     const size_t off_mb2 = bb.put(sd->linear2_b, (size_t)L * C);
@@ -589,10 +608,13 @@
     auto env_int = [](const char* name, int dflt) { const char* e = getenv(name); return e ? atoi(e) : dflt; };
     m->edge_act_bound = edge_bound;
     m->node_act_bound = node_bound;
+    m->node_act_bound_scaled = node_bound_scaled;
+    memcpy(m->mlp_s1, mlp_s1, sizeof(mlp_s1));
+    memcpy(m->mlp_s2, mlp_s2, sizeof(mlp_s2));
     const float f16_slack = 64.0f * 65504.0f;
     m->edge_variant = env_int("ARREAU_EDGE_VARIANT", edge_bound <= f16_slack ? 4 : 3);
-    m->mlp_variant = env_int("ARREAU_MLP_VARIANT", node_bound <= f16_slack ? 3 : 1);
-    m->train_full_range = edge_bound > f16_slack || node_bound > f16_slack ? 1 : 0;
+    m->mlp_variant = env_int("ARREAU_MLP_VARIANT", node_bound_scaled <= f16_slack ? 3 : 1);
+    m->train_full_range = edge_bound > f16_slack || node_bound_scaled > f16_slack ? 1 : 0;
     m->conv_variant = env_int("ARREAU_CONV_VARIANT", 2);
     m->readout_variant = env_int("ARREAU_READOUT_VARIANT", 1);
     m->ran_edge = m->ran_mlp = m->ran_conv = m->ran_readout = -1;
@@ -616,6 +638,18 @@
         return rc;
     }
     *out_model = m;
+    return ARREAU_OK;
+}
+
+extern "C" int arreau_model_read_mlp_planes(const arreau_model* model, int32_t layer, uint16_t* host_out, size_t count, void* stream) {
+    ARREAU_REQUIRE(model && host_out, "arreau_model_read_mlp_planes: null argument");
+    ARREAU_REQUIRE(model->fused && model->mlp_f16m, "arreau_model_read_mlp_planes: this model's shape has no fp16x3 ConvNext planes");
+    const size_t per_layer = (size_t)2 * model->H * model->C * 2;
+    ARREAU_REQUIRE(layer >= 0 && layer < model->L && count == per_layer, "arreau_model_read_mlp_planes: bad layer or count");
+    hipStream_t s = (hipStream_t)stream;
+    ARREAU_CHECK_HIP(hipMemcpyAsync(host_out, reinterpret_cast<const uint16_t*>(model->mlp_f16m) + (size_t)layer * per_layer,
+                                    per_layer * sizeof(uint16_t), hipMemcpyDeviceToHost, s));
+    ARREAU_CHECK_HIP(hipStreamSynchronize(s));
     return ARREAU_OK;
 }
 
@@ -688,6 +722,11 @@
     out->conv_cross_fp8 = model->ran_conv == 2 ? model->ran_x8 : 0;
     out->edge_activation_bound = model->edge_act_bound;
     out->node_activation_bound = model->node_act_bound;
+    out->node_activation_bound_scaled = model->node_act_bound_scaled;
+    for (int l = 0; l < 16; ++l) {
+        out->mlp_scale_linear1[l] = l < model->L ? model->mlp_s1[l] : 0;
+        out->mlp_scale_linear2[l] = l < model->L ? model->mlp_s2[l] : 0;
+    }
     out->basis_fp8_share = model->calib_fp8;
     out->cross_fp8_share = model->calib_x8;
     return ARREAU_OK;
diff --git a/arreau_amd/csrc/node_f16m.hip b/arreau_amd/csrc/node_f16m.hip
--- a/arreau_amd/csrc/node_f16m.hip
+++ b/arreau_amd/csrc/node_f16m.hip
@@ -32,6 +32,12 @@
 }
 }
 
+struct MlpScales { GeluScaled g; float b1, b2, ls; };
+static MlpScales mlp_scales(const arreau_model* m, int layer) {
+    const int s1 = m->mlp_s1[layer], s2 = m->mlp_s2[layer];
+    return MlpScales{gelu_scaled_make(s1), ldexpf(1.0f, s1), ldexpf(1.0f, s1 + s2), ldexpf(1.0f, -(s1 + s2))};
+}
+
 template <int C, int H, int NW, int NB, int NSLOT>
 __global__ __launch_bounds__(64 * NW, 2) void mlp_kernel_f16x3_m16(
     const float* __restrict__ x_conv,
@@ -42,7 +48,8 @@
     const float* __restrict__ wv,
     float bv, int n0, int N , int first_layer,
     float* __restrict__ xbar,
-    float* __restrict__ vsum)
+    float* __restrict__ vsum,
+    const MlpScales sc)
 {
     static_assert(C == 128 && H == 512, "chunking below assumes C = 128, H = 512");
     constexpr int KC = C / 32;
@@ -78,10 +85,10 @@
         dma_chunk<NF, NW>(dma_src, lds[2], wave, lane);
         dma_src += (size_t)NF * 64;
     }
-    for (int i = threadIdx.x; i < H; i += 64 * NW) bias_s[i] = mb1[i];
+    for (int i = threadIdx.x; i < H; i += 64 * NW) bias_s[i] = mb1[i] * sc.b1;
     for (int i = threadIdx.x; i < C; i += 64 * NW) {
-        ep_s[0][i] = mb2[i];
-        ep_s[1][i] = ls[i];
+        ep_s[0][i] = mb2[i] * sc.b2;
+        ep_s[1][i] = ls[i] * sc.ls;
         ep_s[2][i] = wv[i];
     }
 
@@ -154,20 +161,17 @@
         u32x4 hid[NB][KH][2];
 #pragma unroll
         for (int u = 0; u < KH; ++u) {
-            struct { f32x4v m[2][NB], x[2][NB]; } acc;
+            f32x4v acc[2][NB];
 #pragma unroll
             for (int mt = 0; mt < 2; ++mt) {
                 const f32x4 b = *reinterpret_cast<const f32x4*>(bias_s + w * HQ + 32 * u + 16 * mt + 4 * gp);
 #pragma unroll
-                for (int nb = 0; nb < NB; ++nb) {
-                    acc.m[mt][nb] = f32x4v{b[0], b[1], b[2], b[3]};
-                    acc.x[mt][nb] = f32x4v{0.f, 0.f, 0.f, 0.f};
-                }
-            }
-            if (active) mma16_range<KC, 0, ST, NB>(acc.m, acc.x, lds[sl], xn, lane);
+                for (int nb = 0; nb < NB; ++nb) acc[mt][nb] = f32x4v{b[0], b[1], b[2], b[3]};
+            }
+            if (active) mma16_range<KC, 0, ST, NB>(acc, lds[sl], xn, lane);
             sync();
             if (active) {
-                mma16_range<KC, ST, 2 * KC, NB>(acc.m, acc.x, lds[sl], xn, lane);
+                mma16_range<KC, ST, 2 * KC, NB>(acc, lds[sl], xn, lane);
 #pragma unroll
                 for (int nb = 0; nb < NB; ++nb) {
                     float v[8];
@@ -175,9 +179,7 @@
                     for (int mt = 0; mt < 2; ++mt)
 #pragma unroll
                         for (int pr = 0; pr < 2; ++pr) {
-                            const f32x2 pre = fma2(f32x2{acc.x[mt][nb][2 * pr], acc.x[mt][nb][2 * pr + 1]}, splat2(F16X3_INV_SCALE),
-                                                   f32x2{acc.m[mt][nb][2 * pr], acc.m[mt][nb][2 * pr + 1]});
-                            const f32x2 act = gelu_fast2(pre);
+                            const f32x2 act = gelu_fast2_scaled(f32x2{acc[mt][nb][2 * pr], acc[mt][nb][2 * pr + 1]}, sc.g);
                             v[4 * mt + 2 * pr] = act.x;
                             v[4 * mt + 2 * pr + 1] = act.y;
                         }
@@ -188,22 +190,9 @@
         }
 #pragma unroll
         for (int u = 0; u < KC; ++u) {
-            f32x4v cross[2][NB];
-#pragma unroll
-            for (int mt = 0; mt < 2; ++mt)
-#pragma unroll
-                for (int nb = 0; nb < NB; ++nb) cross[mt][nb] = f32x4v{0.f, 0.f, 0.f, 0.f};
-            if (active) mma16_range<KH, 0, ST, NB>(acc_o[u], cross, lds[sl], hid, lane);
+            if (active) mma16_range<KH, 0, ST, NB>(acc_o[u], lds[sl], hid, lane);
             sync();
-            if (active) {
-                mma16_range<KH, ST, 2 * KH, NB>(acc_o[u], cross, lds[sl], hid, lane);
-#pragma unroll
-                for (int mt = 0; mt < 2; ++mt)
-#pragma unroll
-                    for (int nb = 0; nb < NB; ++nb)
-#pragma unroll
-                        for (int r = 0; r < 4; ++r) acc_o[u][mt][nb][r] = fmaf(cross[mt][nb][r], F16X3_INV_SCALE, acc_o[u][mt][nb][r]);
-            }
+            if (active) mma16_range<KH, ST, 2 * KH, NB>(acc_o[u], lds[sl], hid, lane);
             sl = sl == NSLOT - 1 ? 0 : sl + 1;
         }
     }
@@ -278,7 +267,7 @@
     const float* __restrict__ wv, float bv, int n0, int first_layer, float* __restrict__ xbar, float* __restrict__ vsum,
     const float* __restrict__ kl , const int32_t* __restrict__ deg,
     const int32_t* __restrict__ src, const float* __restrict__ fk , const float* __restrict__ conv_bias,
-    MlpTrainSave save) {
+    MlpTrainSave save, const MlpScales sc) {
     static_assert(C == 128 && H == 512, "chunking below assumes C = 128, H = 512");
     constexpr int KC = C / 32, HQ = H / 4;
     constexpr int TS = 132;
@@ -299,8 +288,13 @@
     const int ou = wave >> 1, omt = wave & 1;
     const int ep_c0 = 32 * ou + 16 * omt + 4 * gp;
     const size_t ep_off = ((size_t)n * 16 + cp) * C + ep_c0;
-    const f32x4 ep_b2 = *reinterpret_cast<const f32x4*>(mb2 + ep_c0);
-    const f32x4 ep_ls = *reinterpret_cast<const f32x4*>(ls + ep_c0);
+    f32x4 ep_b2 = *reinterpret_cast<const f32x4*>(mb2 + ep_c0);
+    f32x4 ep_ls = *reinterpret_cast<const f32x4*>(ls + ep_c0);
+#pragma unroll
+    for (int r = 0; r < 4; ++r) {
+        ep_b2[r] *= sc.b2;
+        ep_ls[r] *= sc.ls;
+    }
     const f32x4 ep_xi = *reinterpret_cast<const f32x4*>(x_in + ep_off);
 
     if constexpr (FUSE) {
@@ -399,45 +393,44 @@
 #pragma unroll
                 for (int r = 0; r < 4; ++r) x[kb][4 * hf + r] = x[kb][4 * hf + r] * rstd * gw[r] + gb[r];
             }
-            split8<true, FUSE && TRAIN>(x[kb], xn[kb][0], xn[kb][1]);
+            split8<true, FUSE >(x[kb], xn[kb][0], xn[kb][1]);
         }
     }
 
     auto hidden_chunk = [&](const u32x4 (&w)[16], int j) {
         const int u = 2 * e + j;
-        f32x4v am[2], ax[2];
+        f32x4v am[2];
 #pragma unroll
         for (int mt = 0; mt < 2; ++mt) {
             const f32x4 b = *reinterpret_cast<const f32x4*>(mb1 + q * HQ + 32 * u + 16 * mt + 4 * gp);
-            am[mt] = f32x4v{b[0], b[1], b[2], b[3]};
-            ax[mt] = f32x4v{0.f, 0.f, 0.f, 0.f};
-        }
-#pragma unroll
-        for (int st = 0; st < 2 * KC; ++st) {
-            const int kb = st >> 1, mt = st & 1;
-            am[mt] = mfma16_f16(w[2 * st], xn[kb][0], am[mt]);
-            ax[mt] = mfma16_f16(w[2 * st + 1], xn[kb][0], ax[mt]);
-            am[mt] = mfma16_f16(w[2 * st], xn[kb][1], am[mt]);
-        }
+            am[mt] = f32x4v{b[0] * sc.b1, b[1] * sc.b1, b[2] * sc.b1, b[3] * sc.b1};
+        }
+#pragma unroll
+        for (int kb = 0; kb < KC; ++kb)
+#pragma unroll
+            for (int p = 0; p < 3; ++p)
+#pragma unroll
+                for (int mt = 0; mt < 2; ++mt)
+                    am[mt] = mfma16_f16(w[2 * (2 * kb + mt) + (p == 1 ? 1 : 0)], xn[kb][p == 2 ? 1 : 0], am[mt]);
         float v[8];
 #pragma unroll
         for (int mt = 0; mt < 2; ++mt)
 #pragma unroll
             for (int pr = 0; pr < 2; ++pr) {
-                const f32x2 pre = fma2(f32x2{ax[mt][2 * pr], ax[mt][2 * pr + 1]}, splat2(F16X3_INV_SCALE),
-                                       f32x2{am[mt][2 * pr], am[mt][2 * pr + 1]});
-                const f32x2 act = gelu_fast2(pre);
+                const f32x2 pre = f32x2{am[mt][2 * pr], am[mt][2 * pr + 1]};
+                const f32x2 act = gelu_fast2_scaled(pre, sc.g);
                 v[4 * mt + 2 * pr] = act.x;
                 v[4 * mt + 2 * pr + 1] = act.y;
                 if constexpr (TRAIN) {
                     const size_t o = ((size_t)n * 16 + cp) * H + q * HQ + 32 * u + 16 * mt + 4 * gp + 2 * pr;
                     typedef float f2v __attribute__((ext_vector_type(2)));
-                    *reinterpret_cast<f2v*>(save.hpre + o) = f2v{pre.x, pre.y};
-                    *reinterpret_cast<f2v*>(save.h + o) = f2v{act.x, act.y};
+                    const float t1 = 1.0f / sc.b1;
+                    *reinterpret_cast<f2v*>(save.hpre + o) = f2v{pre.x * t1, pre.y * t1};
+                    *reinterpret_cast<f2v*>(save.h + o) = f2v{act.x * t1, act.y * t1};
                 }
             }
         u32x4 hi, lo;
-        split8<false, FUSE && TRAIN>(v, hi, lo);
+        split8<false, FUSE >(v, hi, lo);
         hidx[4 * q + u][0][lane] = hi;
         hidx[4 * q + u][1][lane] = lo;
     };
@@ -460,16 +453,13 @@
     f32x4v acc = f32x4v{0.f, 0.f, 0.f, 0.f};
     auto quarter = [&](const u32x4 (&w)[16], auto w0c, int w2) {
         constexpr int w0 = decltype(w0c)::value;
-        f32x4v cross = f32x4v{0.f, 0.f, 0.f, 0.f};
 #pragma unroll
         for (int kb = 0; kb < 4; ++kb) {
             const u32x4 bh = hidx[4 * w2 + kb][0][lane], bl = hidx[4 * w2 + kb][1][lane];
             acc = mfma16_f16(w[w0 + 2 * kb], bh, acc);
-            cross = mfma16_f16(w[w0 + 2 * kb + 1], bh, cross);
+            acc = mfma16_f16(w[w0 + 2 * kb + 1], bh, acc);
             acc = mfma16_f16(w[w0 + 2 * kb], bl, acc);
         }
-#pragma unroll
-        for (int r = 0; r < 4; ++r) acc[r] = fmaf(cross[r], F16X3_INV_SCALE, acc[r]);
     };
     quarter(wa, std::integral_constant<int, 0>{}, 0);
     quarter(wa, std::integral_constant<int, 8>{}, 1);
@@ -482,7 +472,8 @@
         for (int r = 0; r < 4; ++r) xo[r] = (acc[r] + ep_b2[r]) * ep_ls[r] + ep_xi[r];
         *reinterpret_cast<f32x4*>(x_out + ep_off) = xo;
         if constexpr (TRAIN) {
-            *reinterpret_cast<f32x4*>(save.out + ep_off) = f32x4{acc[0] + ep_b2[0], acc[1] + ep_b2[1], acc[2] + ep_b2[2], acc[3] + ep_b2[3]};
+            *reinterpret_cast<f32x4*>(save.out + ep_off) = f32x4{(acc[0] + ep_b2[0]) * sc.ls, (acc[1] + ep_b2[1]) * sc.ls,
+                                                                 (acc[2] + ep_b2[2]) * sc.ls, (acc[3] + ep_b2[3]) * sc.ls};
             return;
         }
         f32x4 sum;
@@ -529,7 +520,7 @@
                        m->ln_w + (size_t)layer * C, m->ln_b + (size_t)layer * C, stream, m->mb1 + (size_t)layer * H,
                        m->mb2 + (size_t)layer * C, m->ls + (size_t)layer * C, m->ro_wv + (size_t)layer * C, m->ro_bv_host[layer],
                        0, layer == 0 ? 1 : 0, xbar + (size_t)layer * N * C, vsum, (const float*)nullptr, (const int32_t*)nullptr,
-                       (const int32_t*)nullptr, (const float*)nullptr, (const float*)nullptr, MlpTrainSave{});
+                       (const int32_t*)nullptr, (const float*)nullptr, (const float*)nullptr, MlpTrainSave{}, mlp_scales(m, layer));
     ARREAU_CHECK_HIP(hipGetLastError());
     return ARREAU_OK;
 }
@@ -552,7 +543,7 @@
                        m->ln_w + (size_t)layer * C, m->ln_b + (size_t)layer * C, stream, m->mb1 + (size_t)layer * H,
                        m->mb2 + (size_t)layer * C, m->ls + (size_t)layer * C, m->ro_wv + (size_t)layer * C, m->ro_bv_host[layer],
                        0, layer == 0 ? 1 : 0, xbar + (size_t)layer * Ntot * C, vsum, kbuf + layer_stride * layer, deg, src,
-                       m->fk + (size_t)layer * 16 * 16 * C, m->conv_bias + (size_t)layer * C, MlpTrainSave{});
+                       m->fk + (size_t)layer * 16 * 16 * C, m->conv_bias + (size_t)layer * C, MlpTrainSave{}, mlp_scales(m, layer));
     ARREAU_CHECK_HIP(hipGetLastError());
     return ARREAU_OK;
 }
@@ -575,7 +566,7 @@
         ARREAU_LAUNCH((mlp_kernel_f16x3_m16_split<128, 512, true, true>), dim3((unsigned)N), dim3(512), 0, s, (const float*)nullptr, x_in, x_out,
                       m->ln_w + (size_t)layer * C, m->ln_b + (size_t)layer * C, stream, m->mb1 + (size_t)layer * H, m->mb2 + (size_t)layer * C,
                       m->ls + (size_t)layer * C, (const float*)nullptr, 0.0f, 0, 0, (float*)nullptr, (float*)nullptr, kl, deg, src, fk,
-                      m->conv_bias + (size_t)layer * C, sv);
+                      m->conv_bias + (size_t)layer * C, sv, mlp_scales(m, layer));
         ARREAU_CHECK_HIP(hipGetLastError());
         return ARREAU_OK;
     }
@@ -583,14 +574,15 @@
                   m->ln_w + (size_t)layer * C, m->ln_b + (size_t)layer * C, stream, m->mb1 + (size_t)layer * H, m->mb2 + (size_t)layer * C,
                   m->ls + (size_t)layer * C, (const float*)nullptr, 0.0f, 0, 0, (float*)nullptr, (float*)nullptr, (const float*)nullptr,
                   (const int32_t*)nullptr, (const int32_t*)nullptr, (const float*)nullptr, (const float*)nullptr,
-                  MlpTrainSave{xhat, rstd, xn, hpre, h, out});
+                  MlpTrainSave{xhat, rstd, xn, hpre, h, out}, mlp_scales(m, layer));
     ARREAU_CHECK_HIP(hipGetLastError());
     return ARREAU_OK;
 }
 
 namespace {
+struct MlpPlaneScales { float f[2][16]; };
 __global__ __launch_bounds__(256) void repack_mlp_f16x3_m16_kernel(const float* __restrict__ lin1 , const float* __restrict__ lin2 ,
-                                                                    int L, unsigned short* __restrict__ q) {
+                                                                    int L, unsigned short* __restrict__ q, MlpPlaneScales sc) {
     constexpr int C = 128, H = 512, HQ = 128;
     const long i = (long)blockIdx.x * 256 + threadIdx.x;
     const long per_mat = 4L * 4 * 2 * 64 * 8;
@@ -601,8 +593,9 @@
     const int o = 32 * u + 16 * mt + (lane & 15);
     const int k = 32 * kb + 16 * (e >> 2) + 4 * g + (e & 3);
     const float v = mat == 0 ? lin1[((size_t)l * H + (size_t)w * HQ + o) * C + k] : lin2[((size_t)l * C + o) * H + (size_t)w * HQ + k];
-    const _Float16 h1 = (_Float16)v;
-    const _Float16 h2 = (_Float16)((v - (float)h1) * 2048.0f);
+    const float vs = v * sc.f[mat][l];
+    const _Float16 h1 = (_Float16)vs;
+    const _Float16 h2 = (_Float16)(vs - (float)h1);
     const size_t base = (((size_t)l * 4 + w) * 2 + mat) * (size_t)(2 * per_mat) + (((size_t)u * 4 + kb) * 2 + mt) * 2 * 512 + (size_t)lane * 8 + e;
     q[base] = __builtin_bit_cast(unsigned short, h1);
     q[base + 512] = __builtin_bit_cast(unsigned short, h2);
@@ -611,8 +604,13 @@
 int arreau_repack_mlp_f16x3_m16(arreau_model* m, hipStream_t s) {
     if (!(m->C == 128 && m->H == 512 && m->mlp_f16m)) return ARREAU_OK;
     const long n = (long)m->L * 4 * 2 * 16384;
+    MlpPlaneScales sc{};
+    for (int l = 0; l < m->L && l < 16; ++l) {
+        sc.f[0][l] = ldexpf(1.0f, m->mlp_s1[l]);
+        sc.f[1][l] = ldexpf(1.0f, m->mlp_s2[l]);
+    }
     ARREAU_LAUNCH(repack_mlp_f16x3_m16_kernel, dim3((unsigned)((n + 255) / 256)), dim3(256), 0, s, m->t_lin1, m->t_lin2, m->L,
-                  reinterpret_cast<unsigned short*>(const_cast<float*>(m->mlp_f16m)));
+                  reinterpret_cast<unsigned short*>(const_cast<float*>(m->mlp_f16m)), sc);
     ARREAU_CHECK_HIP(hipGetLastError());
     return ARREAU_OK;
 }
@@ -644,7 +642,7 @@
     auto launch = [&](auto kernel) {
         ARREAU_LAUNCH(kernel, grid, block, 0, s, x_conv, x_in, x_out, lnw, lnb, stream, m->mb1 + (size_t)layer * H,
                            m->mb2 + (size_t)layer * C, m->ls + (size_t)layer * C, m->ro_wv + (size_t)layer * C,
-                           m->ro_bv_host[layer], 0, N, layer == 0 ? 1 : 0, xbar + (size_t)layer * N * C, vsum);
+                           m->ro_bv_host[layer], 0, N, layer == 0 ? 1 : 0, xbar + (size_t)layer * N * C, vsum, mlp_scales(m, layer));
     };
     if (nb == 1 && slots == 4) launch(mlp_kernel_f16x3_m16<128, 512, NW, 1, 4>);
     else if (nb == 1) launch(mlp_kernel_f16x3_m16<128, 512, NW, 1, 3>);
diff --git a/arreau_amd/engine.py b/arreau_amd/engine.py
--- a/arreau_amd/engine.py
+++ b/arreau_amd/engine.py
@@ -107,7 +107,17 @@
                 "basis_row_bytes": int(st.basis_row_bytes), "conv_cross_fp8": int(st.conv_cross_fp8), "edge_activation_bound": float(st.edge_activation_bound),
                 "node_activation_bound": float(st.node_activation_bound),
                 "basis_fp8_share": float(st.basis_fp8_share), "cross_fp8_share": float(st.cross_fp8_share),
-                "readout_kernel": int(st.readout_kernel)}
+                "readout_kernel": int(st.readout_kernel),
+                "mlp_scale_linear1": [int(v) for v in st.mlp_scale_linear1][:self.cfg.num_layers],
+                "mlp_scale_linear2": [int(v) for v in st.mlp_scale_linear2][:self.cfg.num_layers],
+                "node_activation_bound_scaled": float(st.node_activation_bound_scaled)}
+
+    def mlp_planes(self, layer):
+        import numpy as np
+        out = np.empty(4 * self.cfg.hidden_dim * self.cfg.hidden_dim * self.cfg.widening_factor, dtype=np.uint16)
+        _hip.check(_hip.lib().arreau_model_read_mlp_planes(self._handle, int(layer), out.ctypes.data_as(ctypes.c_void_p), out.size,
+                                                           _hip.stream_ptr(self.device)), "arreau_model_read_mlp_planes")
+        return out
 
     def check_status(self, reset=True):
         st = self.status(reset=reset)
diff --git a/include/arreau_hip.h b/include/arreau_hip.h
--- a/include/arreau_hip.h
+++ b/include/arreau_hip.h
@@ -89,7 +89,11 @@
     float basis_fp8_share;
     float cross_fp8_share;
     int32_t readout_kernel;
+    int32_t mlp_scale_linear1[16];
+    int32_t mlp_scale_linear2[16];
+    float node_activation_bound_scaled;
 } arreau_status;
+int arreau_model_read_mlp_planes(const arreau_model* model, int32_t layer, uint16_t* host_out, size_t count, void* stream);
 int arreau_model_status(const arreau_model* model, arreau_status* out, int32_t reset, void* stream);
 int arreau_model_set_formats(arreau_model* model, int32_t basis_fp8, int32_t cross_fp8);
 int arreau_model_set_variant(arreau_model* model, int32_t edge_variant, int32_t mlp_variant);
```
